# uos/radarays_ros

Hardware: AMD Instinct MI355X
Metric: polar images/sec (400 az x 3424 bins) (higher is better)
Workload: dtype f32 rays / f64 energy+time; 1 GPU; target_10M_400x200_4pass; triangles=10248350, azimuths=400, range_bins=3424, rays_per_beam=200, passes=4, ambient_noise=2, frames_per_batch=8

## Files before the change

### include/radarays_mi355.h

```cpp
#ifndef RADARAYS_MI355_H
#define RADARAYS_MI355_H

#include <stddef.h>
#include <stdint.h>

#ifdef __cplusplus
extern "C" {
#endif

#define RR_ABI_VERSION 7
#define RR_MAX_BATCH 64

typedef struct rr_ctx rr_ctx;

typedef struct rr_material {
    float velocity;
    float ambient;
    float diffuse;
    float specular;
} rr_material;

typedef struct rr_config {
    int32_t n_cells;
    int32_t n_angles;
    int32_t n_reflections;
    int32_t signal_denoising;
    int32_t signal_denoising_triangular_width;
    int32_t signal_denoising_gaussian_width;
    int32_t signal_denoising_mb_width;
    int32_t ambient_noise;
    int32_t scroll_image;
    int32_t record_multi_reflection;
    int32_t record_multi_path;
    int32_t max_waves_per_azimuth;
    int32_t brdf_model;
    int32_t reserved_;
    double  resolution;
    double  energy_max;
    double  signal_max;
    double  signal_denoising_triangular_mode;
    double  signal_denoising_gaussian_mode;
    double  signal_denoising_mb_mode;
    double  ambient_noise_at_signal_0;
    double  ambient_noise_at_signal_1;
    double  ambient_noise_energy_max;
    double  ambient_noise_energy_min;
    double  ambient_noise_energy_loss;
    double  multipath_threshold;
    float   wave_energy_threshold;
    float   theta_min;
    float   theta_inc;
    float   range_max;
} rr_config;

typedef struct rr_stats {
    uint64_t wave_passes;
    uint64_t hits;
    uint64_t signals;
    uint64_t nodes_visited;
    uint64_t tris_tested;
    uint32_t overflow;
    uint32_t pad_;
} rr_stats;

void rr_default_config(rr_config* cfg);

rr_ctx* rr_create(int device);
void    rr_destroy(rr_ctx* ctx);
const char* rr_last_error(const rr_ctx* ctx);
int     rr_abi_version(void);

int rr_set_mesh(rr_ctx* ctx, const float* verts , size_t nv,
                const uint32_t* faces , size_t nf,
                const uint32_t* face_object_id );

int rr_set_mesh_gpu(rr_ctx* ctx, const float* verts , size_t nv,
                    const uint32_t* faces , size_t nf,
                    const uint32_t* face_object_id );

int rr_copy_mesh(rr_ctx* ctx, rr_ctx* src);

int rr_set_object_poses(rr_ctx* ctx, const float* poses , size_t n);
int rr_update_vertices(rr_ctx* ctx, const float* verts , size_t nv);
int rr_get_tree_cost(rr_ctx* ctx, double* cost_now, double* cost_at_build);
int rr_rebuild_tree(rr_ctx* ctx, int builder);

int rr_set_materials(rr_ctx* ctx, const rr_material* materials, size_t n_materials,
                     const int32_t* object_materials, size_t n_objects,
                     int32_t material_id_air);

int rr_set_config(rr_ctx* ctx, const rr_config* cfg);

int rr_set_beam_samples(rr_ctx* ctx, const float* dirs , size_t n);

int rr_set_noise_offsets(rr_ctx* ctx, const float* rnd, size_t n);

int rr_set_motion_poses(rr_ctx* ctx, const float* poses, size_t n);

int rr_simulate(rr_ctx* ctx, const float pose_qxyzw_t[7], int az_begin, int az_end,
                uint8_t* out_u8, float* out_f32, rr_stats* stats);

int rr_simulate_columns_device(rr_ctx* ctx, const float pose_qxyzw_t[7], int az_begin, int az_end,
                               uint8_t* d_cols_u8, float* d_cols_f32, void* stream);

int rr_simulate_batch_columns_device(rr_ctx* ctx, const float* poses, int n_frames, int az_begin, int az_end,
                                     uint8_t* d_cols_u8, void* stream);

int rr_simulate_batch_device(rr_ctx* ctx, const float* poses, int n_frames, uint8_t* d_imgs_u8, void* stream);

int rr_simulate_batch_host_async(rr_ctx* ctx, const float* poses, int n_frames, uint8_t* h_imgs_u8, void* stream);
int rr_wait_host(rr_ctx* ctx, const void* h_imgs_u8);
void* rr_host_alloc(size_t bytes);
void  rr_host_free(void* p);

int rr_copy_to_host_async(rr_ctx* ctx, const void* d_src, void* h_dst, size_t bytes, void* stream);
int rr_deliver_to_host_async(rr_ctx* ctx, const void* d_src, void* h_dst, size_t bytes, void* stream);
int rr_host_delivery_route(rr_ctx* ctx);

int rr_assemble_image_device(rr_ctx* ctx, const uint8_t* d_cols_u8 ,
                             uint8_t* d_img_u8 , void* stream);

int rr_assemble_blocks_device(rr_ctx* ctx, const uint8_t* d_cols_u8, int n_loc, size_t block_stride,
                              uint8_t* d_img_u8, void* stream);

int rr_simulate_material_sets_device(rr_ctx* ctx, const float pose[7], const rr_material* sets, int n_sets,
                                     size_t n_materials ,
                                     uint8_t* d_imgs_u8, void* stream);
int rr_simulate_material_sets(rr_ctx* ctx, const float pose[7], const rr_material* sets, int n_sets,
                              size_t n_materials, uint8_t* out_imgs_u8);

typedef struct rr_param_set {
    const rr_material* materials;
    const float* beam_dirs;
    int32_t n_reflections;
    int32_t reserved_;
} rr_param_set;
int rr_simulate_param_sets_device(rr_ctx* ctx, const float pose[7], const rr_param_set* sets, int n_sets, size_t n_materials,
                                  uint8_t* d_imgs_u8 , void* stream);
int rr_score_images_device(rr_ctx* ctx, const uint8_t* d_imgs_u8, int n_images, const uint8_t* d_ref_u8,
                           double* out_psnr , uint64_t* out_sse , void* stream);
int rr_simulate_param_sets(rr_ctx* ctx, const float pose[7], const rr_param_set* sets, int n_sets, size_t n_materials,
                           uint8_t* out_imgs_u8, const uint8_t* ref_img_u8, double* out_psnr);

int rr_assemble_frames_device(rr_ctx* ctx, const uint8_t* d_cols_u8, int n_loc, size_t block_stride,
                              int n_frames, size_t frame_stride, uint8_t* d_imgs_u8, void* stream);

int rr_simulate_device(rr_ctx* ctx, const float pose_qxyzw_t[7], uint8_t* d_img_u8, void* stream);

int rr_synchronize(rr_ctx* ctx, void* stream);

int rr_peek_error_bits_async(rr_ctx* ctx, uint32_t* h_bits, void* stream);

int rr_get_stats(rr_ctx* ctx, rr_stats* stats);

int rr_set_stats_mode(rr_ctx* ctx, int enable);
int rr_get_traversal_shape(rr_ctx* ctx, uint64_t out[8]);

int rr_debug_trace(rr_ctx* ctx, const float* origs , const float* dirs , size_t n,
                   float* out_t , uint32_t* out_face );
int rr_debug_fresnel(rr_ctx* ctx, size_t n, const float* normals , const float* dirs , const double* energy ,
                     const double* v1 , const float* v2 ,
                     float* out_refl_dir , double* out_refl_energy , float* out_refr_dir , double* out_refr_energy );
int rr_debug_brdf(rr_ctx* ctx, size_t n, const float* in5 , int brdf_model, float* out );
int rr_get_bvh_info(rr_ctx* ctx, uint64_t* n_nodes, uint64_t* n_tris, uint32_t* depth, uint32_t* stack_need);
int rr_get_trace_grid(rr_ctx* ctx, uint32_t out_rows[24], uint32_t out_hist[24], uint64_t* repaired_groups);
int rr_get_graph_stats(rr_ctx* ctx, uint64_t* captures, uint64_t* replays);
int rr_set_timing_mode(rr_ctx* ctx, int enable );
int rr_get_kernel_time(rr_ctx* ctx, const char* kernel ,
                       double* total_ms, uint64_t* launches, int reset);

int rr_get_kernel_samples(rr_ctx* ctx, const char* kernel, float* out_ms, size_t capacity, size_t* n_out);
int rr_reserve_timing_events(rr_ctx* ctx, size_t n);

typedef struct rr_detect_config {
    int32_t method;
    int32_t guard_cells;
    int32_t train_cells;
    int32_t k;
    int32_t min_intensity;
    int32_t min_bin;
    float   cfar_scale;
    int32_t reserved_;
} rr_detect_config;

typedef struct rr_radar_point {
    float    x, y, z;
    float    intensity;
    uint32_t column;
    uint32_t bin;
} rr_radar_point;

typedef struct rr_cartesian_config {
    int32_t width;
    int32_t interpolation;
    float   pixel_size;
    int32_t reserved_;
} rr_cartesian_config;

void rr_default_detect_config(rr_detect_config* cfg);

int rr_detect_device(rr_ctx* ctx, const uint8_t* d_imgs_u8 , int n_frames,
                     const rr_detect_config* cfg, rr_radar_point* d_points ,
                     int max_points, uint32_t* d_offsets , void* stream);
int rr_detect(rr_ctx* ctx, const uint8_t* imgs_u8, int n_frames, const rr_detect_config* cfg,
              rr_radar_point* points, int max_points, uint32_t* offsets);
int rr_polar_to_cartesian_device(rr_ctx* ctx, const uint8_t* d_imgs_u8, int n_frames, const rr_cartesian_config* cfg,
                                 uint8_t* d_cart_u8 , void* stream);
int rr_polar_to_cartesian(rr_ctx* ctx, const uint8_t* imgs_u8, int n_frames, const rr_cartesian_config* cfg,
                          uint8_t* cart_u8);

typedef struct rr_multi rr_multi;
rr_multi* rr_create_multi(const int* devices, int n_devices);
void rr_destroy_multi(rr_multi* m);
const char* rr_multi_last_error(const rr_multi* m);
int rr_multi_device_count(const rr_multi* m);
int rr_multi_rccl_version(const rr_multi* m);
rr_ctx* rr_multi_ctx(rr_multi* m, int i);
void rr_partition(int n_angles, int world, int rank, int* begin, int* end);
int rr_multi_plan(int n_angles, int n_cells, int n_devices, int n_frames, int* equal_blocks, size_t* bytes_per_device,
                  size_t* send_off, size_t* recv_off, size_t* piece_bytes);
int rr_multi_set_mesh(rr_multi* m, const float* verts, size_t nv, const uint32_t* faces, size_t nf, const uint32_t* face_object_id);
int rr_multi_set_mesh_gpu(rr_multi* m, const float* verts, size_t nv, const uint32_t* faces, size_t nf, const uint32_t* face_object_id);
int rr_multi_set_object_poses(rr_multi* m, const float* poses, size_t n);
int rr_multi_update_vertices(rr_multi* m, const float* verts, size_t nv);
int rr_multi_rebuild_tree(rr_multi* m, int builder);
int rr_multi_set_materials(rr_multi* m, const rr_material* materials, size_t n_materials,
                           const int32_t* object_materials, size_t n_objects, int32_t material_id_air);
int rr_multi_set_config(rr_multi* m, const rr_config* cfg);
int rr_multi_set_beam_samples(rr_multi* m, const float* dirs, size_t n);
int rr_multi_set_noise_offsets(rr_multi* m, const float* rnd, size_t n);
int rr_multi_set_motion_poses(rr_multi* m, const float* poses, size_t n);
int rr_multi_simulate(rr_multi* m, const float pose_qxyzw_t[7], uint8_t* out_u8);
int rr_multi_simulate_batch(rr_multi* m, const float* poses, int n_frames, uint8_t* out_imgs_u8);
int rr_multi_simulate_batch_async(rr_multi* m, const float* poses, int n_frames, uint8_t* h_imgs_u8);
int rr_multi_wait(rr_multi* m, const void* h_imgs_u8);

int rr_cone_dirs(float width_rad, int sample_dist, float p_in_cone, const float* u_angle, const float* r_variate, size_t n,
                 float* out_dirs);
int rr_sample_cone_local(uint32_t seed, float width_rad, size_t n, int sample_dist, float p_in_cone, float* out_dirs);

typedef struct rr_mesh {
    float* verts;
    size_t n_verts;
    uint32_t* faces;
    size_t n_faces;
    uint32_t* face_object_id;
    size_t n_objects;
    char** object_names;
} rr_mesh;
int rr_load_mesh_file(const char* path, rr_mesh* out, char* err, size_t err_len);
int rr_mesh_reorder_objects(rr_mesh* m, const char* const* order, size_t n_order, char* err, size_t err_len);
void rr_free_mesh(rr_mesh* m);


#ifdef __cplusplus
}
#endif
#endif
```

### radarays_ros_amd/csrc/rr_api.hip

```cpp
#include "rr_ctx.h"
#include <algorithm>
#include <cmath>
#include <cstring>
#include <cstdlib>
#include <dlfcn.h>

namespace rr {
namespace {

std::string g_create_error;

bool roctx_load()
{
    static int state = 0;
    if (state == 0) {
        state = -1;
        for (const char* n : { "librocprofiler-sdk-roctx.so.1", "librocprofiler-sdk-roctx.so", "libroctx64.so.4", "libroctx64.so" }) {
            void* h = dlopen(n, RTLD_NOW | RTLD_GLOBAL);
            if (!h) continue;
            g_roctx_push = (roctx_push_fn)dlsym(h, "roctxRangePushA");
            g_roctx_pop = (roctx_pop_fn)dlsym(h, "roctxRangePop");
            if (g_roctx_push && g_roctx_pop) { state = 1; break; }
        }
    }
// ... 118 lines not shown
    }
    }

    if (dirty & rr_ctx::D_MAT) {
    std::vector<float4> m4(c->materials.size());
    for (size_t i = 0; i < m4.size(); i++)
        m4[i] = make_float4(c->materials[i].velocity, c->materials[i].ambient, c->materials[i].diffuse, c->materials[i].specular);
    RR_HIP(c, c->d_materials.ensure(m4.size()));
    if (!m4.empty()) RR_HIP(c, upload_table(c, c->d_materials.p, m4.data(), m4.size() * sizeof(float4)));
    RR_HIP(c, c->d_mat_limits.ensure(m4.size()));
    launch_mat_limits(c->d_materials.p, m4.size(), c->d_mat_limits.p, nullptr);
    RR_HIP(c, hipGetLastError());
    RR_HIP(c, hipStreamSynchronize(nullptr));
    RR_HIP(c, c->d_objmat.ensure(c->object_materials.size()));
    if (!c->object_materials.empty())
        RR_HIP(c, upload_table(c, c->d_objmat.p, c->object_materials.data(), c->object_materials.size() * sizeof(int32_t)));
    }

    if (dirty & rr_ctx::D_CFG) {
    make_smear(g, c->smear, c->smear_mode);
    RR_HIP(c, c->d_smear.ensure(c->smear.size()));
    if (!c->smear.empty()) RR_HIP(c, upload_table(c, c->d_smear.p, c->smear.data(), c->smear.size() * sizeof(float)));

    RR_HIP(c, c->d_decay.ensure((size_t)std::max(1, g.n_cells)));
    launch_decay_table(c->d_decay.p, g.n_cells, g.resolution, g.ambient_noise_energy_loss, nullptr);
    RR_HIP(c, hipGetLastError());
    RR_HIP(c, hipDeviceSynchronize());
    }

    if (dirty & (rr_ctx::D_NOISE | rr_ctx::D_CFG)) {
    const size_t A = (size_t)g.n_angles;
    if (!c->noise.empty() && c->noise.size() % A != 0)
        return fail(c, -3, "rr_set_noise_offsets: the number of offsets must be a multiple of n_angles (one row per frame of a batch)");
    c->noise_rows = c->noise.size() >= 2 * A ? (int)(c->noise.size() / A) : 1;
    std::vector<float> nz((size_t)c->noise_rows * A, 0.0f);
    for (size_t i = 0; i < nz.size() && i < c->noise.size(); i++) nz[i] = c->noise[i];
    RR_HIP(c, c->d_noise.ensure(nz.size()));
    RR_HIP(c, upload_table(c, c->d_noise.p, nz.data(), nz.size() * sizeof(float)));
    }
    if ((dirty & (rr_ctx::D_MOTION | rr_ctx::D_CFG)) && !c->motion.empty()) {
        if (c->motion.size() % (7 * (size_t)g.n_angles) != 0)
            return fail(c, -3, "rr_set_motion_poses: the number of poses must be a multiple of n_angles (one table per frame of a batch)");
        c->motion_rows = (int)(c->motion.size() / (7 * (size_t)g.n_angles));
        RR_HIP(c, c->d_motion.ensure(c->motion.size()));
        RR_HIP(c, upload_table(c, c->d_motion.p, c->motion.data(), c->motion.size() * sizeof(float)));
    }
    c->motion_live = !c->motion.empty();
    const void* motion_after = c->motion_live ? (const void*)c->d_motion.p : nullptr;
    if (regen || noise_before != (const void*)c->d_noise.p || noise_rows_before != c->noise_rows ||
        motion_before != motion_after || motion_rows_before != c->motion_rows) c->graph_gen++;
    c->tables_dirty = 0;
    return 0;
}

int read_back(rr_ctx* c, void* dst, const void* d_src, size_t bytes)
{
    if (bytes == 0) return 0;
    if (bytes % 16 != 0 || (uintptr_t)d_src % 16 != 0) { RR_HIP(c, hipMemcpy(dst, d_src, bytes, hipMemcpyDeviceToHost)); return 0; }
    if (c->h_rb_bytes < bytes) {
        if (c->h_rb) (void)hipHostFree(c->h_rb);
        c->h_rb = nullptr; c->h_rb_bytes = 0;
        RR_HIP(c, hipHostMalloc(&c->h_rb, bytes + 4096, hipHostMallocDefault));
        c->h_rb_bytes = bytes + 4096;
    }
    launch_copy_host(d_src, c->h_rb, bytes, 4, -1, c->stream);
    RR_HIP(c, hipGetLastError());
    RR_HIP(c, hipStreamSynchronize(c->stream));
    std::memcpy(dst, c->h_rb, bytes);
    return 0;
}

int overflow_error(rr_ctx* c, uint32_t bits, bool since_sync)
{
    if (bits & 1u)
        return fail(c, -7, std::string("wave/signal queue capacity exceeded") + (since_sync ? " in a frame since the last rr_synchronize" : "") +
                               "; raise rr_config.max_waves_per_azimuth");
    if (bits & 2u)
        return fail(c, -8, std::string("object id or material id out of range of the tables given to rr_set_materials") +
                               (since_sync ? " (a frame since the last rr_synchronize)" : ""));
    return 0;
}

int check_ready(rr_ctx* c)
{
    if (!c) return -1;
    if (!c->have_mesh) return fail(c, -2, "rr_set_mesh has not been called");
    if (!c->have_cfg) return fail(c, -2, "rr_set_config has not been called");
    if (!c->have_materials) return fail(c, -2, "rr_set_materials has not been called");
    if (c->beams.empty() && c->cfg.n_reflections > 0) return fail(c, -2, "rr_set_beam_samples has not been called");
    return 0;
}

}

extern "C" {

int rr_abi_version(void) { return RR_ABI_VERSION; }

void rr_partition(int n_angles, int world, int rank, int* begin, int* end)
{
    if (world < 1) world = 1;
    const int base = n_angles / world, rem = n_angles % world;
    const int b = rank * base + (rank < rem ? rank : rem);
    if (begin) *begin = b;
    if (end) *end = b + base + (rank < rem ? 1 : 0);
}

void rr_default_config(rr_config* cfg)
{
    if (!cfg) return;
    std::memset(cfg, 0, sizeof(*cfg));
    cfg->n_cells = 3424; cfg->n_angles = 400; cfg->n_reflections = 4;
    cfg->signal_denoising = 1;
    cfg->signal_denoising_triangular_width = 50; cfg->signal_denoising_triangular_mode = 0.35;
    cfg->signal_denoising_gaussian_width = 50; cfg->signal_denoising_gaussian_mode = 0.5;
    cfg->signal_denoising_mb_width = 50; cfg->signal_denoising_mb_mode = 0.4;
    cfg->ambient_noise = 2; cfg->scroll_image = 0;
    cfg->record_multi_reflection = 1; cfg->record_multi_path = 0;
    cfg->max_waves_per_azimuth = 0;
    cfg->resolution = 0.0438; cfg->energy_max = 0.5; cfg->signal_max = 120.0;
    cfg->ambient_noise_at_signal_0 = 0.3; cfg->ambient_noise_at_signal_1 = 0.03;
    cfg->ambient_noise_energy_max = 0.5; cfg->ambient_noise_energy_min = 0.1;
    cfg->ambient_noise_energy_loss = 0.05; cfg->multipath_threshold = 0.5;
    cfg->wave_energy_threshold = 0.001f;
    cfg->theta_min = 0.0f; cfg->theta_inc = (float)(-(2 * M_PI) / 400);
    cfg->range_max = 1000.0f;
}

rr_ctx* rr_create(int device)
{
    int n = 0;
    hipError_t e = hipGetDeviceCount(&n);
    if (e != hipSuccess || n <= 0) {
        g_create_error = std::string("rr_create: no HIP device (") + (e != hipSuccess ? hipGetErrorString(e) : "count 0") +
                         "); this library has no CPU fallback";
        return nullptr;
    }
    if (device < 0 || device >= n) { g_create_error = "rr_create: device index out of range"; return nullptr; }
    if (hipSetDevice(device) != hipSuccess) { g_create_error = "rr_create: hipSetDevice failed"; return nullptr; }
    rr_ctx* c = new rr_ctx();
    c->device = device;
    if (hipStreamCreateWithFlags(&c->stream, hipStreamNonBlocking) != hipSuccess) {
        g_create_error = "rr_create: hipStreamCreate failed"; delete c; return nullptr;
    }
    rr_default_config(&c->cfg);
    int n_lanes = getenv("RR_LANES") ? atoi(getenv("RR_LANES")) : 4;
    n_lanes = std::max(1, std::min(n_lanes, 8));
    c->stream_lanes = getenv("RR_STREAM_LANES") ? std::max(1, std::min(atoi(getenv("RR_STREAM_LANES")), n_lanes))
                                                : std::min(3, n_lanes);
    if (getenv("RR_PASS0_AZ")) { const int a = atoi(getenv("RR_PASS0_AZ")); if (a == 1 || a == 2 || a == 4 || a == 8 || a == 16) c->pass0_az = a; }
    if (getenv("RR_STACK_LDS")) c->stack_lds_max = std::max(1, std::min(64, atoi(getenv("RR_STACK_LDS"))));
    if (getenv("RR_ROCTX") && atoi(getenv("RR_ROCTX")) != 0) c->roctx = roctx_load();
    if (getenv("RR_CULL_POP")) c->cull_pop = atoi(getenv("RR_CULL_POP")) != 0;
    if (getenv("RR_STACKLESS")) c->stackless = atoi(getenv("RR_STACKLESS")) != 0;
    if (getenv("RR_TRACE_CHUNK")) c->seg_chunk = std::max(0, std::min(1024, atoi(getenv("RR_TRACE_CHUNK"))));
    if (getenv("RR_GRAPHS")) c->use_graphs = atoi(getenv("RR_GRAPHS")) != 0;
    if (getenv("RR_HOST_SDMA")) c->host_sdma = atoi(getenv("RR_HOST_SDMA")) != 0;
    if (getenv("RR_TIGHT_GRID")) c->tight_grid = atoi(getenv("RR_TIGHT_GRID")) != 0;
    if (getenv("RR_TIGHT_FORCE")) c->tight_force = std::max(0, atoi(getenv("RR_TIGHT_FORCE")));
    {
        const float4 same = make_float4(0.3f, 0.f, 0.f, 0.f);
        DevBuf<float4> m1; DevBuf<double> l1;
        bool ok = m1.ensure(1) == hipSuccess && l1.ensure(2) == hipSuccess &&
                  upload_table(c, m1.p, &same, sizeof(same)) == hipSuccess;
        if (ok) {
            launch_mat_limits(m1.p, 1, l1.p, nullptr);
            double two[2] = {0.0, 0.0};
            ok = hipStreamSynchronize(nullptr) == hipSuccess && read_back(c, two, l1.p, sizeof(two)) == 0;
            c->limit_same = two[0];
        }
        m1.release(); l1.release();
        if (!ok) { g_create_error = "rr_create: device set-up failed"; rr_destroy(c); return nullptr; }
    }
    c->lanes.resize((size_t)n_lanes);
    for (Lane& L : c->lanes) {
        if (hipStreamCreateWithFlags(&L.stream, hipStreamNonBlocking) != hipSuccess ||
            hipEventCreateWithFlags(&L.ev_ready, hipEventDisableTiming) != hipSuccess ||
            hipEventCreateWithFlags(&L.ev_consumed, hipEventDisableTiming) != hipSuccess ||
            hipEventCreateWithFlags(&L.slot[0].ev, hipEventDisableTiming) != hipSuccess ||
            hipEventCreateWithFlags(&L.slot[1].ev, hipEventDisableTiming) != hipSuccess) {
            g_create_error = "rr_create: lane stream/event creation failed"; rr_destroy(c); return nullptr;
        }
    }
    return c;
}

void rr_destroy(rr_ctx* c)
{
    if (!c) return;
    (void)hipSetDevice(c->device);
    (void)hipDeviceSynchronize();
    if (c->sdma) { sdma_destroy(c->sdma); c->sdma = nullptr; }
    for (Delivery& d : c->deliveries) (void)hipEventDestroy(d.ev);
    for (hipEvent_t e : c->delivery_events) (void)hipEventDestroy(e);
    for (auto& kv : c->timers) for (auto& p : kv.second.pending) { (void)hipEventDestroy(p.first); (void)hipEventDestroy(p.second); }
    for (hipEvent_t e : c->event_pool) (void)hipEventDestroy(e);
    c->d_rest_v.release(); c->d_stage_v.release(); c->d_rest_f.release(); c->d_poses.release(); c->d_stage_poses.release();
    c->d_levels.release(); c->d_red.release(); c->d_cost.release(); c->d_built.release(); c->d_moved.release();
    c->d_bvh.release(); c->d_qas.release(); c->d_beams.release(); c->d_materials.release(); c->d_mat_limits.release();
    c->d_objmat.release(); c->d_smear.release(); c->d_noise.release(); c->d_decay.release(); c->d_param_imgs.release(); c->d_sse.release(); c->d_ref_img.release(); c->d_conv_in.release(); c->d_conv_cart.release(); c->d_conv_points.release(); c->d_conv_offs.release(); c->d_beam_order.release(); c->d_beam_order2.release(); c->d_motion.release();
    for (Lane& L : c->lanes) {
        if (L.stream) (void)hipStreamSynchronize(L.stream);
        for (int k = 0; k < 2; k++) { L.d_wA[k].release(); L.d_wB[k].release(); L.d_wC[k].release(); L.d_idx[k].release(); L.d_count[k].release(); L.d_torder[k].release(); }
        L.d_refpos.release();
        L.d_hit.release(); L.d_sig_count.release(); L.d_spill.release(); L.d_cflag.release(); L.d_cols_u8.release();
        L.d_sigtmp.release(); L.d_sig.release(); L.d_cols_f32.release(); L.d_counters.release(); L.d_sticky.release(); L.d_seg_stats.release(); L.d_matsets.release(); L.d_matset_limits.release(); L.d_set_beams.release(); L.d_set_order.release(); L.d_set_order2.release(); L.d_img_f32.release();
        L.d_hint.release(); L.d_ovf_list.release(); if (L.h_hist) { (void)hipHostFree(L.h_hist); L.h_hist = nullptr; }
        drop_graphs(L); L.d_poses.release();
        if (L.ev_ready) (void)hipEventDestroy(L.ev_ready);
        if (L.ev_consumed) (void)hipEventDestroy(L.ev_consumed);
        for (Delivery& d : L.slot) { d.img.release(); if (d.ev) (void)hipEventDestroy(d.ev); }
        if (L.stream) (void)hipStreamDestroy(L.stream);
    }
    if (c->stream) (void)hipStreamDestroy(c->stream);
    if (c->h_frame) (void)hipHostFree(c->h_frame);
    if (c->h_rb) (void)hipHostFree(c->h_rb);
    delete c;
}

const char* rr_last_error(const rr_ctx* c) { return c ? c->err.c_str() : g_create_error.c_str(); }

int rr_set_materials(rr_ctx* c, const rr_material* materials, size_t n_materials,
                     const int32_t* object_materials, size_t n_objects, int32_t material_id_air)
{
    if (!c) return -1;
    if (!materials || n_materials == 0) return fail(c, -3, "rr_set_materials: empty material table");
    if (n_objects && !object_materials) return fail(c, -3, "rr_set_materials: null object_materials");
    if (material_id_air < 0 || (size_t)material_id_air >= n_materials) return fail(c, -3, "rr_set_materials: material_id_air out of range");
    for (size_t i = 0; i < n_objects; i++)
        if (object_materials[i] < 0 || (size_t)object_materials[i] >= n_materials)
            return fail(c, -3, "rr_set_materials: object_materials entry out of range");
    if (c->have_materials && c->materials.size() == n_materials && c->object_materials.size() == n_objects &&
        c->material_id_air == material_id_air &&
        std::memcmp(c->materials.data(), materials, n_materials * sizeof(rr_material)) == 0 &&
        (n_objects == 0 || std::memcmp(c->object_materials.data(), object_materials, n_objects * sizeof(int32_t)) == 0))
        return 0;
    c->materials.assign(materials, materials + n_materials);
    c->object_materials.assign(object_materials, object_materials + n_objects);
    c->material_id_air = material_id_air;
    c->have_materials = true; c->tables_dirty |= rr_ctx::D_MAT;
    return 0;
}

int rr_set_config(rr_ctx* c, const rr_config* cfg)
{
    if (!c) return -1;
    if (!cfg) return fail(c, -3, "rr_set_config: null config");
    if (cfg->n_cells < 1 || cfg->n_cells > 8192) return fail(c, -3, "rr_set_config: n_cells must be in [1, 8192]");
    if (cfg->n_angles < 1 || cfg->n_angles > 65536) return fail(c, -3, "rr_set_config: n_angles must be in [1, 65536]");
    if (cfg->n_reflections < 0 || cfg->n_reflections > 16) return fail(c, -3, "rr_set_config: n_reflections must be in [0, 16]");
    if (cfg->signal_denoising < 0 || cfg->signal_denoising > 3) return fail(c, -3, "rr_set_config: signal_denoising must be 0..3");
    const int w = cfg->signal_denoising == 1 ? cfg->signal_denoising_triangular_width
                : cfg->signal_denoising == 2 ? cfg->signal_denoising_gaussian_width
                : cfg->signal_denoising == 3 ? cfg->signal_denoising_mb_width : 0;
    if (w < 0 || w > 256) return fail(c, -3, "rr_set_config: smear width must be in [0, 256]");
    if (cfg->ambient_noise < 0 || cfg->ambient_noise > 2) return fail(c, -3, "rr_set_config: ambient_noise must be 0..2");
    if (cfg->brdf_model < 0 || cfg->brdf_model > 1) return fail(c, -3, "rr_set_config: brdf_model must be 0 (A + B cos^C) or 1 (Cook-Torrance lobe)");
    if (!(cfg->resolution > 0.0)) return fail(c, -3, "rr_set_config: resolution must be > 0");
    const double mf = cfg->signal_denoising == 1 ? cfg->signal_denoising_triangular_mode
                    : cfg->signal_denoising == 2 ? cfg->signal_denoising_gaussian_mode
                    : cfg->signal_denoising == 3 ? cfg->signal_denoising_mb_mode : 0.0;
    if (!(mf >= 0.0 && mf < 1.0)) return fail(c, -3, "rr_set_config: denoising mode fraction must be in [0, 1)");
    if (!(cfg->range_max > 0.0f && cfg->range_max <= 1.0e30f)) return fail(c, -3, "rr_set_config: range_max must be in (0, 1e30]");
    if (!std::isfinite(cfg->wave_energy_threshold) || !std::isfinite(cfg->theta_min) || !std::isfinite(cfg->theta_inc))
        return fail(c, -3, "rr_set_config: non-finite wave_energy_threshold / theta_min / theta_inc");
    if (c->have_cfg && std::memcmp(&c->cfg, cfg, sizeof(rr_config)) == 0) return 0;
    c->cfg = *cfg;
    c->have_cfg = true; c->tables_dirty |= rr_ctx::D_CFG;
    return 0;
}

int rr_set_beam_samples(rr_ctx* c, const float* dirs, size_t n)
{
    if (!c) return -1;
    if (n && !dirs) return fail(c, -3, "rr_set_beam_samples: null dirs");
    if (n > 65536) return fail(c, -3, "rr_set_beam_samples: more than 65536 samples");
    for (size_t i = 0; i < 3 * n; i++) if (!std::isfinite(dirs[i])) return fail(c, -3, "rr_set_beam_samples: non-finite direction");
    if (c->beams.size() == 3 * n && (n == 0 || std::memcmp(c->beams.data(), dirs, 3 * n * sizeof(float)) == 0)) return 0;
    c->beams.assign(dirs, dirs + 3 * n);
    c->tables_dirty |= rr_ctx::D_BEAMS;
    return 0;
}

int rr_set_noise_offsets(rr_ctx* c, const float* rnd, size_t n)
{
    if (!c) return -1;
    if (n && !rnd) return fail(c, -3, "rr_set_noise_offsets: null pointer");
    for (size_t i = 0; i < n; i++) if (!std::isfinite(rnd[i])) return fail(c, -3, "rr_set_noise_offsets: non-finite offset");
    c->noise.assign(rnd, rnd + n);
    c->tables_dirty |= rr_ctx::D_NOISE;
    return 0;
}

int rr_set_motion_poses(rr_ctx* c, const float* poses, size_t n)
{
    if (!c) return -1;
    if (n && !poses) return fail(c, -3, "rr_set_motion_poses: null pointer");
    for (size_t i = 0; i < 7 * n; i++) if (!std::isfinite(poses[i])) return fail(c, -3, "rr_set_motion_poses: non-finite pose");
    c->motion.assign(poses, poses + 7 * n);
    c->tables_dirty |= rr_ctx::D_MOTION;
    return 0;
}

void* rr_host_alloc(size_t bytes)
{
    void* p = nullptr;
    if (hipHostMalloc(&p, bytes ? bytes : 1, hipHostMallocDefault) != hipSuccess) return nullptr;
    return p;
}

void rr_host_free(void* p) { if (p) (void)hipHostFree(p); }

int rr_score_images_device(rr_ctx* c, const uint8_t* d_imgs_u8, int n_images, const uint8_t* d_ref_u8, double* out_psnr,
                           uint64_t* out_sse, void* stream)
{
    if (!c) return -1;
    if (!c->have_cfg) return fail(c, -2, "rr_set_config has not been called");
    if (!d_imgs_u8 || !d_ref_u8 || (!out_psnr && !out_sse)) return fail(c, -3, "rr_score_images_device: null buffer");
    if (n_images < 1 || n_images > 65535) return fail(c, -3, "rr_score_images_device: n_images must be 1..65535");
    RR_HIP(c, hipSetDevice(c->device));
    hipStream_t s = stream_of(c, stream);
    const size_t npx = (size_t)c->cfg.n_cells * c->cfg.n_angles;
    static_assert(sizeof(unsigned long long) == sizeof(uint64_t), "sse words");
    if (c->d_sse.n < (size_t)n_images) { RR_HIP(c, hipStreamSynchronize(s)); RR_HIP(c, c->d_sse.ensure((size_t)n_images)); }
    RR_HIP(c, hipMemsetAsync(c->d_sse.p, 0, (size_t)n_images * sizeof(uint64_t), s));
    launch_score(d_imgs_u8, d_ref_u8, npx, n_images, c->d_sse.p, s);
    RR_HIP(c, hipGetLastError());
    std::vector<uint64_t> sse((size_t)n_images);
    RR_HIP(c, hipMemcpyAsync(sse.data(), c->d_sse.p, (size_t)n_images * sizeof(uint64_t), hipMemcpyDeviceToHost, s));
    RR_HIP(c, hipStreamSynchronize(s));
    for (int k = 0; k < n_images; k++) {
        if (out_sse) out_sse[k] = sse[(size_t)k];
        if (out_psnr) {
            const double err = (double)sse[(size_t)k] / (double)npx;
            out_psnr[k] = err > 0.0 ? 10.0 * std::log10((255.0 * 255.0) / err) : INFINITY;
        }
    }
    return 0;
}

void rr_default_detect_config(rr_detect_config* cfg)
{
    if (!cfg) return;
    std::memset(cfg, 0, sizeof(*cfg));
    cfg->method = 0; cfg->guard_cells = 2; cfg->train_cells = 16; cfg->k = 12;
    cfg->min_intensity = 1; cfg->min_bin = 0; cfg->cfar_scale = 3.0f;
}

namespace {

int check_frames(rr_ctx* c, const char* who, const void* imgs, int n_frames)
{
    if (!c) return -1;
    if (!c->have_cfg) return fail(c, -2, "rr_set_config has not been called");
    if (!imgs) return fail(c, -3, std::string(who) + ": null images");
    if (n_frames < 1 || n_frames > 65535) return fail(c, -3, std::string(who) + ": n_frames must be 1..65535");
// ... 135 lines not shown
```

### radarays_ros_amd/csrc/rr_ctx.h

```cpp
#pragma once
#include "rr_launch.h"
#include "rr_sdma.h"
#include <map>
#include <string>
#include <vector>

namespace rr {
template <typename T>
struct DevBuf {
    T* p = nullptr;
    size_t n = 0;
    hipError_t ensure(size_t count) {
        if (count <= n && p) return hipSuccess;
        if (p) { (void)hipFree(p); p = nullptr; n = 0; }
        if (count == 0) count = 1;
        hipError_t e = hipMalloc((void**)&p, count * sizeof(T));
        if (e == hipSuccess) n = count;
        return e;
    }
    void release() { if (p) (void)hipFree(p); p = nullptr; n = 0; }
};

struct KernelTimer {
    std::vector<std::pair<hipEvent_t, hipEvent_t>> pending;
    double total_ms = 0.0;
    uint64_t launches = 0;
    std::vector<float> samples_ms;
};

struct Delivery {
    DevBuf<uint8_t> img;
    hipEvent_t ev = nullptr;
    const void* dst = nullptr;
    uint64_t job = 0;
};

struct Lane {
    int buf_seg = 0, buf_cap = 0, buf_sigcap = 0, buf_cells = 0, buf_passes = 0;
    DevBuf<float4> d_wA[2], d_wB[2];
    DevBuf<double2> d_wC[2];
    DevBuf<uint32_t> d_idx[2], d_count[2], d_refpos, d_sig_count, d_spill;
    DevBuf<uint2> d_torder[2];
    DevBuf<uint2> d_hit;
    DevBuf<uint8_t> d_cflag, d_cols_u8;
    DevBuf<SigRec> d_sigtmp, d_sig;
    DevBuf<float> d_cols_f32;
    DevBuf<Counters> d_counters;
    DevBuf<uint32_t> d_sticky;
    DevBuf<float> d_img_f32;
    DevBuf<SegStats> d_seg_stats;
    DevBuf<float4> d_matsets;
    DevBuf<double> d_matset_limits;
    DevBuf<float4> d_set_beams; DevBuf<uint32_t> d_set_order, d_set_order2;
    std::vector<float4> h_set_beams, h_matsets; std::vector<uint32_t> h_set_order, h_set_order2;
    int last_n_seg = 0, last_n_passes = 0;
    int spill_stride = 0, stack_lds = 1;
    DevBuf<GridHint> d_hint; DevBuf<uint32_t> d_ovf_list; int ovf_stride = 0;
    uint32_t* h_hist = nullptr; int hist_gen = 0;
    struct FrameGraph {
        int az_begin = 0, az_end = 0, n_frames = 0; const void* cols = nullptr; unsigned short rows[kMaxPasses] = {};
        hipGraph_t g = nullptr; hipGraphExec_t ge = nullptr; hipGraphNode_t pose_node = nullptr; uint64_t last_use = 0; int hits = 0;
        hipGraphExec_t ge2 = nullptr; hipEvent_t ev[2] = { nullptr, nullptr }; bool ev_pending[2] = { false, false }; int flip = 0;
        hipKernelNodeParams pose_kp{};
        Params pose_P;
    };
    std::vector<FrameGraph> graphs; int graph_gen = 0;
    DevBuf<float> d_poses;
    unsigned short last_rows[kMaxPasses] = {};

    hipStream_t stream = nullptr;
    hipEvent_t ev_ready = nullptr, ev_consumed = nullptr;
    bool pending_consume = false;
    Delivery slot[2]; int next_slot = 0;
};

}
using namespace rr;

struct rr_ctx {
    int device = 0;
    hipStream_t stream = nullptr;
    std::string err;

    bool have_mesh = false;
    DevBuf<float4> d_bvh;
    uint32_t tri_base4 = 0;
    uint64_t n_nodes = 0, n_tris = 0;
    uint32_t depth = 0, stack_need = 0;
    float hit_pad = 0.f;

    DevBuf<float> d_rest_v, d_stage_v;
    DevBuf<uint32_t> d_rest_f;
    size_t rest_nv = 0, rest_nf = 0;
    uint32_t n_objects = 1;
    std::vector<float> poses;
    DevBuf<float> d_poses, d_stage_poses;
    bool dyn_ready = false;
    bool rebuilding = false;
    DevBuf<uint32_t> d_levels;
    std::vector<uint32_t> level_off;
    bool cost_known = false; double cost_at_build = 0.0;
    DevBuf<float4> d_built; bool have_built = false; float built_hit_pad = 0.f;
    std::vector<float> build_poses; bool verts_dirty = false;
    DevBuf<uint8_t> d_moved;
    DevBuf<float> d_red; DevBuf<double> d_cost;

    rr_config cfg;
    bool have_cfg = false;
    std::vector<rr_material> materials;
    std::vector<int32_t> object_materials;
    int32_t material_id_air = 0;
    bool have_materials = false;
    std::vector<float> beams;
    std::vector<float> noise;
    int noise_rows = 1;
    int motion_rows = 1;
    bool motion_live = false;
    std::vector<float> motion;
    std::vector<float> smear;
    int smear_mode = 0;

    DevBuf<float4> d_qas, d_beams, d_materials;
    DevBuf<double> d_mat_limits;
    double limit_same = 0.0;
    DevBuf<uint32_t> d_beam_order, d_beam_order2;
    DevBuf<int32_t> d_objmat;
    DevBuf<float> d_smear, d_noise, d_motion, d_decay;
    DevBuf<uint8_t> d_param_imgs;
    enum : unsigned { D_CFG = 1, D_BEAMS = 2, D_MAT = 4, D_NOISE = 8, D_MOTION = 16, D_ALL = 31 };
    unsigned tables_dirty = D_ALL;

    std::vector<Lane> lanes;
    size_t next_lane = 0, last_lane = 0;
    size_t next_stream_lane = 0;
    int stream_lanes = 3;

    bool stats_mode = false;
    int pass0_az = 16;
    int stack_lds_max = 64;
    int timing = 0;
    std::map<std::string, KernelTimer> timers;
    std::vector<hipEvent_t> event_pool;
    hipEvent_t take_event() {
        if (!event_pool.empty()) { hipEvent_t e = event_pool.back(); event_pool.pop_back(); return e; }
        hipEvent_t e = nullptr; (void)hipEventCreate(&e); return e;
    }

    int passes_override = -1;
    DevBuf<unsigned long long> d_sse; DevBuf<uint8_t> d_ref_img;
    DevBuf<uint8_t> d_conv_in, d_conv_cart; DevBuf<rr_radar_point> d_conv_points; DevBuf<uint32_t> d_conv_offs;
    void* h_rb = nullptr; size_t h_rb_bytes = 0;
    void* h_frame = nullptr; size_t h_frame_bytes = 0;

    bool roctx = false;
    int seg_chunk = 16;
    int stackless = 0;
    int cull_pop = 1;
    int host_sdma = 1; SdmaCopier* sdma = nullptr; bool sdma_tried = false;
    std::vector<Delivery> deliveries;
    std::vector<hipEvent_t> delivery_events;
    int tight_grid = 1;
    int tight_force = 0;
    int hist_gen = 1;
    int use_graphs = 1;
    int graph_gen = 1;
    uint64_t graph_clock = 0, graph_replays = 0, graph_captures = 0;
};

namespace rr {
typedef int (*roctx_push_fn)(const char*);
typedef int (*roctx_pop_fn)(void);
inline roctx_push_fn g_roctx_push = nullptr; inline roctx_pop_fn g_roctx_pop = nullptr;
inline void roctx_push(const char* name) { if (g_roctx_push) g_roctx_push(name); }
inline void roctx_pop() { if (g_roctx_pop) g_roctx_pop(); }
int fail(rr_ctx* c, int code, const std::string& msg);

inline hipStream_t stream_of(const rr_ctx* c, void* stream) { return stream ? (hipStream_t)stream : c->stream; }

#define RR_HIP(c, expr)                                                                        \
    do {                                                                                       \
        hipError_t e_ = (expr);                                                                \
        if (e_ != hipSuccess)                                                                  \
            return fail((c), -100, std::string(#expr) + ": " + hipGetErrorString(e_));         \
    } while (0)

struct TimedScope {
    rr_ctx* c; hipStream_t s; const char* name; hipEvent_t a = nullptr, b = nullptr;
    bool on;
    TimedScope(rr_ctx* c_, hipStream_t s_, const char* n_) : c(c_), s(s_), name(n_) {
        on = c->timing == 1;
        if (on) { a = c->take_event(); b = c->take_event(); (void)hipEventRecord(a, s); }
        if (c->roctx) roctx_push(name);
    }
    ~TimedScope() {
        if (on) { (void)hipEventRecord(b, s); c->timers[name].pending.emplace_back(a, b); }
        if (c->roctx) roctx_pop();
    }
};

struct KernelEvents {
    rr_ctx* c; const char* name; hipEvent_t a = nullptr, b = nullptr;
    KernelEvents(rr_ctx* c_, const char* n_) : c(c_), name(n_) {
        if (c->timing == 1) { a = c->take_event(); b = c->take_event(); }
        if (c->roctx) roctx_push(name);
    }
    ~KernelEvents() {
        if (a) c->timers[name].pending.emplace_back(a, b);
        if (c->roctx) roctx_pop();
    }
};

struct SetPlan {
    int n_groups = 1;
    unsigned char frame_passes[64], frame_beam[64], group_frame[64];
    const float4* d_beams = nullptr; const uint32_t* d_order = nullptr; const uint32_t* d_order2 = nullptr;
};

int check_ready(rr_ctx* c);
int upload_tables(rr_ctx* c);
void beam_trace_orders(const float* beams, size_t nb, std::vector<uint32_t>& order, std::vector<uint32_t>& order2);
int read_back(rr_ctx* c, void* dst, const void* d_src, size_t bytes);
int overflow_error(rr_ctx* c, uint32_t bits, bool since_sync = false);
inline int read_counters(rr_ctx* c, Counters& h) { return read_back(c, &h, c->lanes[c->last_lane].d_counters.p, sizeof(h)); }

void drop_graphs(Lane& L);
int prepare_lane(rr_ctx* c, Lane& L, int n_seg, bool want_f32 = false);
bool host_visible(const void* p);
int settle_lane(rr_ctx* c, Lane& L, int slot = -1, const void* only_dst = nullptr);
int take_lane(rr_ctx* c, size_t li, hipStream_t s, int slot = -1);
hipError_t give_lane(Lane& L, hipStream_t s);
int run_frame(rr_ctx* c, Lane& L, const float* pose, int az_begin, int az_end, uint8_t* d_cols_u8 , float* d_cols_f32,
              hipStream_t s, int n_frames = 1, const float4* d_matsets = nullptr, int mat_stride = 0, bool lane_f32 = false, const SetPlan* plan = nullptr);
int assemble_frames(rr_ctx* c, const Lane& L, uint8_t* dst, int n_frames, hipStream_t s);

}
```

### radarays_ros_amd/csrc/rr_device.h

```cpp
#pragma once
#include <hip/hip_runtime.h>
#include <stdint.h>

#include "rr_bvh.h"

namespace rr {

struct V3 { float x, y, z; };
struct Quat { float x, y, z, w; };

__host__ __device__ inline V3 v_add(V3 a, V3 b) { return { a.x + b.x, a.y + b.y, a.z + b.z }; }
__host__ __device__ inline V3 v_sub(V3 a, V3 b) { return { a.x - b.x, a.y - b.y, a.z - b.z }; }
__host__ __device__ inline V3 v_neg(V3 a) { return { -a.x, -a.y, -a.z }; }
__host__ __device__ inline V3 v_scale(V3 a, float s) { return { a.x * s, a.y * s, a.z * s }; }
__host__ __device__ inline float v_dot(V3 a, V3 b) { return a.x * b.x + a.y * b.y + a.z * b.z; }
__host__ __device__ inline V3 v_cross(V3 a, V3 b)
{
    return { a.y * b.z - a.z * b.y, a.z * b.x - a.x * b.z, a.x * b.y - a.y * b.x };
}
__host__ __device__ inline V3 v_normalize(V3 a)
{
    const float d = sqrtf(a.x * a.x + a.y * a.y + a.z * a.z);
    return { a.x / d, a.y / d, a.z / d };
}
__host__ __device__ inline Quat q_mul(Quat a, Quat b)
{
    Quat r;
    r.x = a.w * b.x + a.x * b.w + a.y * b.z - a.z * b.y;
    r.y = a.w * b.y - a.x * b.z + a.y * b.w + a.z * b.x;
    r.z = a.w * b.z + a.x * b.y - a.y * b.x + a.z * b.w;
    r.w = a.w * b.w - a.x * b.x - a.y * b.y - a.z * b.z;
    return r;
}
__host__ __device__ inline Quat q_conj(Quat a) { return { -a.x, -a.y, -a.z, a.w }; }
__host__ __device__ inline V3 q_rot(Quat q, V3 v)
{
    Quat t;
    t.x = q.w * v.x + q.y * v.z - q.z * v.y;
    t.y = q.w * v.y - q.x * v.z + q.z * v.x;
    t.z = q.w * v.z + q.x * v.y - q.y * v.x;
    t.w = 0.0f - q.x * v.x - q.y * v.y - q.z * v.z;
    const Quat c = q_conj(q);
    V3 r;
    r.x = t.w * c.x + t.x * c.w + t.y * c.z - t.z * c.y;
    r.y = t.w * c.y - t.x * c.z + t.y * c.w + t.z * c.x;
    r.z = t.w * c.z + t.x * c.y - t.y * c.x + t.z * c.w;
    return r;
}

struct WaveBuf {
    float4* A;
    float4* B;
    double2* C;
};

struct SigRec { int32_t cell; float strength; };

struct Counters {
    unsigned long long nodes, tris;
    unsigned long long wave_iters;
    unsigned int max_iters, n_waves;
    unsigned int overflow, pad;
    unsigned long long it_all, it_node, it_leaf, quad_steps;
    unsigned long long pad2;
};

constexpr int kMaxPasses = 24;
struct GridHint { uint32_t hist[kMaxPasses]; uint32_t ovf_n[kMaxPasses]; unsigned long long repaired;  };

struct SegStats { uint32_t wave_passes, hits, signals, pad; };

struct Params {
    const Node4* nodes;
    const TriRec* tris;
    uint32_t tri_base4;
    const float4* q_as;
    const float4* beams;
    const uint32_t* beam_order;
    const uint32_t* beam_order2;
    const float4* materials;
    const double* mat_limits;
    double limit_same;
    const int32_t* object_materials;
    const float* smear;
    const float* noise_rnd;
    int noise_rows;
    int mat_stride;
    int set_mode;
    int n_groups;
    unsigned char frame_passes[64];
    unsigned char frame_beam[64];
    unsigned char group_frame[64];
    const float* decay;
    const float* motion_poses;
    int motion_rows;
    WaveBuf waves[2];
    uint32_t* idx[2];
    uint32_t* count[2];
    uint2* torder[2];
    uint32_t* refpos;
    uint8_t* cflag;
    SigRec* sigtmp;
    uint2* hit;
    SigRec* sig;
    uint32_t* sig_count;
    uint32_t* spill;
    Counters* counters;
    uint32_t* sticky;
    SegStats* seg_stats;
    uint8_t* cols_u8;
    float* cols_f32;
    int az_begin, n_seg;
    int n_loc, n_frames;
    float4* pose_table;
    int n_beam, cap, sigcap;
    int n_cells, n_angles, n_materials, n_objects, material_id_air;
    int n_passes, record_multi_reflection, record_multi_path;
    int brdf_model;
    int signal_denoising, smear_w, smear_mode, ambient_noise, scroll;
    float thr, range_max;
    float hit_pad;
    double resolution, multipath_threshold;
    float energy_max_f;
    double signal_max;
    double noise_at_0, noise_at_1, noise_e_max, noise_e_min, noise_e_loss;
    int spill_stride, stack_lds, spill_depth;
    int pass0_az;
    int trace_row;
    int seg_chunk;
    int stackless;
    int cull_pop;
    GridHint* grid_hint;
    uint32_t* hist_host;
    uint32_t* ovf_list;
    int ovf_stride;
    unsigned short tight_groups[kMaxPasses];
};

struct PoseArgs { float p[64][7]; int n; };
struct NoPoses {};
template <bool FIRST> struct PosesOf { using type = NoPoses; };
template <> struct PosesOf<true> { using type = PoseArgs; };

__host__ __device__ inline int passes_of(const Params& P, int frame) { return P.set_mode ? (int)P.frame_passes[frame] : P.n_passes; }
__host__ __device__ inline int beam_base(const Params& P, int frame) { return P.set_mode ? (int)P.frame_beam[frame] * P.n_beam : 0; }

static_assert(sizeof(Params) <= 4096, "Params is passed by value: HIP kernel arguments are limited to 4 KB");

}
```

### radarays_ros_amd/csrc/rr_frame.hip

```cpp
#include "rr_ctx.h"
#include "rr_hostprof.h"
#include <algorithm>
#include <cmath>
#include <cstdio>
#include <cstring>
#include <cstdlib>

namespace rr {
namespace {

inline int eff_passes(const rr_ctx* c) { return c->passes_override >= 0 ? c->passes_override : c->cfg.n_reflections; }
inline rr_config eff_config(const rr_ctx* c) { rr_config g = c->cfg; g.n_reflections = eff_passes(c); return g; }

int wave_capacity(const rr_config& cfg, int n_beam)
{
    long cap = cfg.max_waves_per_azimuth;
    if (cap <= 0) {
        cap = n_beam;
        for (int p = 1; p < cfg.n_reflections && cap < 65536; p++) cap *= 2;
        cap = std::min<long>(cap, 65536);
    }
    cap = std::max<long>(cap, n_beam);
    return (int)cap;
}

int signal_capacity(const rr_config& cfg, int n_beam, int cap)
{
    long tot = 0, w = n_beam;
    for (int p = 0; p < cfg.n_reflections; p++) { tot += std::min<long>(w, cap); w = std::min<long>(2 * w, cap); }
    if (cfg.record_multi_path) tot *= 2;
    return (int)std::max<long>(tot, 1);
}

void drop_graph(Lane::FrameGraph& fg)
{
    for (int k = 0; k < 2; k++) {
        if (fg.ev[k]) { if (fg.ev_pending[k]) (void)hipEventSynchronize(fg.ev[k]); (void)hipEventDestroy(fg.ev[k]); fg.ev[k] = nullptr; fg.ev_pending[k] = false; }
    }
    if (fg.ge) (void)hipGraphExecDestroy(fg.ge);
    if (fg.ge2) (void)hipGraphExecDestroy(fg.ge2);
    if (fg.g) (void)hipGraphDestroy(fg.g);
    fg.ge = fg.ge2 = nullptr; fg.g = nullptr;
}
int ensure_frame_buffers(rr_ctx* c, Lane& L, int n_seg, bool want_f32)
{
    const rr_config g = eff_config(c);
    const int n_beam = (int)(c->beams.size() / 3);
    const int cap = wave_capacity(g, n_beam);
    const int sigcap = signal_capacity(g, n_beam, cap);
    const size_t S = (size_t)n_seg;
    const size_t per_seg = (size_t)cap * (2 * 2 * 48 + 2 * 4 + 2 * 9 + 8) + (size_t)sigcap * 8 + (size_t)g.n_cells * 5;
    size_t free_b = 0, total_b = 0;
    RR_HIP(c, hipMemGetInfo(&free_b, &total_b));
    if (S * per_seg > total_b / 2)
        return fail(c, -6, "wave queue capacity needs more than half of device memory; lower max_waves_per_azimuth");
    for (int k = 0; k < 2; k++) {
        RR_HIP(c, L.d_wA[k].ensure(S * 2 * cap));
        RR_HIP(c, L.d_wB[k].ensure(S * 2 * cap));
        RR_HIP(c, L.d_wC[k].ensure(S * 2 * cap));
        RR_HIP(c, L.d_idx[k].ensure(S * cap));
        RR_HIP(c, L.d_torder[k].ensure(S * cap));
        RR_HIP(c, L.d_count[k].ensure(S));
    }
    RR_HIP(c, L.d_cflag.ensure(S * 2 * cap));
    RR_HIP(c, L.d_refpos.ensure(S * 2 * cap));
    RR_HIP(c, L.d_sigtmp.ensure(S * 2 * cap));
    RR_HIP(c, L.d_hit.ensure(S * cap));
    RR_HIP(c, L.d_sig.ensure(S * sigcap));
    RR_HIP(c, L.d_sig_count.ensure(S));
    if (!L.d_counters.p) { RR_HIP(c, L.d_counters.ensure(1)); RR_HIP(c, hipMemset(L.d_counters.p, 0, sizeof(Counters))); }
    if (!L.d_sticky.p) { RR_HIP(c, L.d_sticky.ensure(1)); RR_HIP(c, hipMemset(L.d_sticky.p, 0, sizeof(uint32_t))); }
    RR_HIP(c, L.d_seg_stats.ensure(S * (size_t)std::max(1, g.n_reflections)));
    if (!L.d_hint.p) { RR_HIP(c, L.d_hint.ensure(1)); RR_HIP(c, hipMemset(L.d_hint.p, 0, sizeof(GridHint))); L.hist_gen = 0; }
    if (!L.h_hist) { RR_HIP(c, hipHostMalloc((void**)&L.h_hist, kMaxPasses * sizeof(uint32_t), hipHostMallocDefault)); std::memset(L.h_hist, 0, kMaxPasses * sizeof(uint32_t)); }
    RR_HIP(c, L.d_ovf_list.ensure(S * (size_t)kMaxPasses)); L.ovf_stride = (int)S;
    RR_HIP(c, L.d_cols_u8.ensure(S * g.n_cells));
    if (want_f32) RR_HIP(c, L.d_cols_f32.ensure(S * g.n_cells));
    L.stack_lds = (int)std::max<uint32_t>(1, std::min<uint32_t>(c->stack_need, (uint32_t)c->stack_lds_max));
    const int spill_depth = (int)c->stack_need - L.stack_lds;
    const size_t A0 = (size_t)c->pass0_az, Sw0 = 16 / A0;
    const size_t slots0 = ((((S + A0 - 1) / A0) * (((size_t)n_beam + Sw0 - 1) / Sw0) + 1) / 2) * 32;
    const size_t threads = std::max(S * (size_t)((cap + 63) / 64) * 64, slots0);
    L.spill_stride = (int)threads;
    if (spill_depth > 0) RR_HIP(c, L.d_spill.ensure((size_t)spill_depth * threads));
    else RR_HIP(c, L.d_spill.ensure(1));
    L.buf_seg = n_seg; L.buf_cap = cap; L.buf_sigcap = sigcap; L.buf_cells = g.n_cells; L.buf_passes = std::max(1, g.n_reflections);
    RR_HIP(c, L.d_poses.ensure((size_t)RR_MAX_BATCH * 8));
    L.graph_gen = 0;
    return 0;
}

void fill_params(rr_ctx* c, Lane& L, Params& P, const float pose[7], int az_begin, int n_seg,
                 uint8_t* d_cols_u8, float* d_cols_f32)
{
    const rr_config g = eff_config(c);
    std::memset(&P, 0, sizeof(P));
    P.nodes = reinterpret_cast<const Node4*>(c->d_bvh.p); P.tris = reinterpret_cast<const TriRec*>(c->d_bvh.p + c->tri_base4);
    P.tri_base4 = c->tri_base4;
    P.q_as = c->d_qas.p; P.beams = c->d_beams.p; P.beam_order = c->d_beam_order.p; P.beam_order2 = c->d_beam_order2.p; P.materials = c->d_materials.p;
    P.mat_limits = c->d_mat_limits.p; P.limit_same = c->limit_same;
    P.object_materials = c->d_objmat.p; P.smear = c->d_smear.p;
    P.noise_rnd = g.ambient_noise ? c->d_noise.p : nullptr; P.noise_rows = c->noise_rows;
    P.decay = c->d_decay.p;
    P.motion_poses = c->motion.empty() ? nullptr : c->d_motion.p; P.motion_rows = c->motion_rows;
    for (int k = 0; k < 2; k++) {
        P.waves[k].A = L.d_wA[k].p; P.waves[k].B = L.d_wB[k].p; P.waves[k].C = L.d_wC[k].p;
        P.idx[k] = L.d_idx[k].p; P.count[k] = L.d_count[k].p; P.torder[k] = L.d_torder[k].p;
    }
    P.refpos = L.d_refpos.p;
    P.cflag = L.d_cflag.p; P.sigtmp = L.d_sigtmp.p; P.hit = L.d_hit.p;
    P.sig = L.d_sig.p; P.sig_count = L.d_sig_count.p; P.spill = L.d_spill.p; P.counters = L.d_counters.p; P.sticky = L.d_sticky.p; P.seg_stats = L.d_seg_stats.p;
    P.cols_u8 = d_cols_u8; P.cols_f32 = d_cols_f32;
    P.az_begin = az_begin; P.n_seg = n_seg;
    P.n_beam = (int)(c->beams.size() / 3); P.cap = L.buf_cap; P.sigcap = L.buf_sigcap;
    P.n_cells = g.n_cells; P.n_angles = g.n_angles;
    P.n_materials = (int)c->materials.size(); P.n_objects = (int)c->object_materials.size();
    P.material_id_air = c->material_id_air;
    P.n_passes = g.n_reflections;
    P.record_multi_reflection = g.record_multi_reflection; P.record_multi_path = g.record_multi_path;
    P.brdf_model = g.brdf_model;
    P.signal_denoising = c->smear.empty() ? 0 : g.signal_denoising;
    P.smear_w = (int)c->smear.size(); P.smear_mode = c->smear_mode;
    P.ambient_noise = g.ambient_noise; P.scroll = g.scroll_image;
    P.thr = g.wave_energy_threshold; P.range_max = g.range_max; P.hit_pad = c->hit_pad;
    P.resolution = g.resolution; P.multipath_threshold = g.multipath_threshold;
    P.energy_max_f = (float)g.energy_max; P.signal_max = g.signal_max;
    P.noise_at_0 = g.ambient_noise_at_signal_0; P.noise_at_1 = g.ambient_noise_at_signal_1;
    P.noise_e_max = g.ambient_noise_energy_max; P.noise_e_min = g.ambient_noise_energy_min;
    P.noise_e_loss = g.ambient_noise_energy_loss;
    P.spill_stride = L.spill_stride; P.stack_lds = L.stack_lds;
    P.spill_depth = std::max(0, (int)c->stack_need - L.stack_lds);
    P.pass0_az = c->pass0_az;
    P.cull_pop = c->cull_pop; P.seg_chunk = c->seg_chunk; P.stackless = c->stackless;
    P.grid_hint = L.d_hint.p; P.ovf_list = L.d_ovf_list.p; P.ovf_stride = L.ovf_stride;
    P.hist_host = (c->tight_grid && g.n_reflections > 1) ? L.h_hist : nullptr;
}

int copy_out(rr_ctx* c, const void* d_src, void* h_dst, size_t bytes, bool visible, hipStream_t s)
{
    if (bytes == 0) return 0;
    if (visible && bytes % 16 == 0 && ((uintptr_t)h_dst | (uintptr_t)d_src) % 16 == 0) {
        launch_copy_host(d_src, h_dst, bytes, 8, 0, s);
        RR_HIP(c, hipGetLastError());
    } else RR_HIP(c, hipMemcpyAsync(h_dst, d_src, bytes, hipMemcpyDeviceToHost, s));
    return 0;
}

int wait_delivery(rr_ctx* c, Delivery& d)
{
    if (!d.dst) return 0;
    if (d.job) sdma_wait(c->sdma, d.job);
    else RR_HIP(c, hipEventSynchronize(d.ev));
    d.dst = nullptr; d.job = 0;
    return 0;
}

SdmaCopier* sdma_of(rr_ctx* c, const void* any_device_ptr)
{
    if (!c->host_sdma) return nullptr;
    if (!c->sdma && !c->sdma_tried) {
        c->sdma_tried = true;
        std::string why;
        c->sdma = sdma_create(c->device, any_device_ptr, why);
        if (!c->sdma && getenv("RR_HOST_SDMA_VERBOSE")) fprintf(stderr, "[rr] SDMA delivery not available: %s\n", why.c_str());
    }
    if (c->sdma && sdma_failed(c->sdma, nullptr)) {
        if (getenv("RR_HOST_SDMA_VERBOSE")) { std::string why; (void)sdma_failed(c->sdma, &why); fprintf(stderr, "[rr] SDMA delivery switched off: %s\n", why.c_str()); }
        c->host_sdma = 0;
        return nullptr;
    }
    return c->sdma;
}

int choose_trace_rows(rr_ctx* c, Lane& L, Params& P, const rr_config& g, hipStream_t s)
{
    if (L.hist_gen != c->hist_gen) {
        RR_HIP(c, hipMemsetAsync(L.d_hint.p, 0, sizeof(GridHint), s));
        std::memset(L.h_hist, 0, kMaxPasses * sizeof(uint32_t));
        L.hist_gen = c->hist_gen;
    }
    const bool tight = c->tight_grid && !c->stats_mode && !P.set_mode && P.spill_depth == 0 && g.n_reflections <= kMaxPasses;
    if (tight) {
        for (int pass = 1; pass < g.n_reflections; pass++) {
            const long bound = std::min<long>((long)P.cap, pass < 20 ? (long)P.n_beam << pass : (long)P.cap);
            const long full = (bound + 15) / 16;
            uint32_t h = 0;
            for (const Lane& o : c->lanes) if (o.h_hist && o.hist_gen == c->hist_gen) h = std::max(h, o.h_hist[pass]);
            long row = h ? std::min<long>(full, ((long)h + (long)h / 16 + 32 + 15) / 16) : full;
            row |= 1;
            if (c->tight_force) row = std::min<long>(full, c->tight_force);
            P.tight_groups[pass] = (row < full && row < 65535) ? (unsigned short)row : 0;
        }
    }
    std::memcpy(L.last_rows, P.tight_groups, sizeof(L.last_rows));
    return 0;
}

int issue_chain(rr_ctx* c, const Params& Q, const PoseArgs& pa, const rr_config& g, hipStream_t s)
{
    for (int pass = 0; pass < g.n_reflections; pass++) {
        if (c->roctx) roctx_push(pass == 0 ? "trace pass 0" : "trace");
        if (c->timing) {
            hipEvent_t a = c->take_event(), b = c->take_event();
            const bool rep = pass > 0 && pass < kMaxPasses && Q.tight_groups[pass];
            hipEvent_t ra = rep ? c->take_event() : nullptr, rb = rep ? c->take_event() : nullptr;
            bool launched = false;
            launch_trace(Q, pass, &pa, c->stats_mode, s, a, b, ra, rb, &launched);
            c->timers[pass == 0 ? "trace0" : "trace"].pending.emplace_back(a, b);
            if (launched) c->timers["trace_repair"].pending.emplace_back(ra, rb);
            else if (rep) { c->event_pool.push_back(ra); c->event_pool.push_back(rb); }
        } else {
            launch_trace(Q, pass, &pa, c->stats_mode, s);
        }
        if (c->roctx) roctx_pop();
        { KernelEvents t(c, "shade"); launch_shade(Q, pass, s, t.a, t.b); }
        if (pass < g.n_reflections - 1) { KernelEvents t(c, "scan"); launch_scan(Q, pass, s, t.a, t.b); }
    }
    { KernelEvents t(c, "column"); launch_column(Q, s, t.a, t.b); }
    return 0;
}

Lane::FrameGraph* find_graph(Lane& L, int az_begin, int az_end, int n_frames, const uint8_t* d_cols_u8, const Params& P)
{
    Lane::FrameGraph* fg = nullptr;
    for (Lane::FrameGraph& x : L.graphs)
        if (x.az_begin == az_begin && x.az_end == az_end && x.n_frames == n_frames && x.cols == (const void*)d_cols_u8 &&
            std::memcmp(x.rows, P.tight_groups, sizeof(x.rows)) == 0) { fg = &x; break; }
    if (!fg) {
        if (L.graphs.size() >= 12) {
            size_t lru = 0;
            for (size_t k = 1; k < L.graphs.size(); k++) if (L.graphs[k].last_use < L.graphs[lru].last_use) lru = k;
            drop_graph(L.graphs[lru]);
            L.graphs.erase(L.graphs.begin() + (long)lru);
        }
        Lane::FrameGraph n;
        n.az_begin = az_begin; n.az_end = az_end; n.n_frames = n_frames; n.cols = d_cols_u8;
        std::memcpy(n.rows, P.tight_groups, sizeof(n.rows));
        L.graphs.push_back(n);
        fg = &L.graphs.back();
    }
    return fg;
}

void capture_graph(rr_ctx* c, Lane::FrameGraph* fg, const Params& P, const PoseArgs& pa, const rr_config& g, hipStream_t s)
{
    if (c->sdma) sdma_wait_all(c->sdma);
    hipError_t e = hipStreamBeginCapture(s, hipStreamCaptureModeThreadLocal);
    if (e == hipSuccess) {
        const int rcq = issue_chain(c, P, pa, g, s);
        hipGraph_t gph = nullptr;
        e = hipStreamEndCapture(s, &gph);
        if (rcq == 0 && e == hipSuccess && gph) {
            hipGraphExec_t ge = nullptr, ge2 = nullptr;
            if (hipGraphInstantiate(&ge, gph, nullptr, nullptr, 0) == hipSuccess && hipGraphInstantiate(&ge2, gph, nullptr, nullptr, 0) == hipSuccess &&
                hipEventCreateWithFlags(&fg->ev[0], hipEventDisableTiming) == hipSuccess && hipEventCreateWithFlags(&fg->ev[1], hipEventDisableTiming) == hipSuccess) {
                size_t nn = 0; (void)hipGraphGetNodes(gph, nullptr, &nn);
                std::vector<hipGraphNode_t> nodes(nn); (void)hipGraphGetNodes(gph, nodes.data(), &nn);
                for (hipGraphNode_t nd : nodes) {
                    hipGraphNodeType ty; hipKernelNodeParams kp{};
                    if (hipGraphNodeGetType(nd, &ty) == hipSuccess && ty == hipGraphNodeTypeKernel &&
                        hipGraphKernelNodeGetParams(nd, &kp) == hipSuccess && kp.func == trace0_kernel(P.spill_depth > 0, P.stackless != 0)) {
                        fg->pose_node = nd; fg->pose_kp = kp; fg->pose_P = P; break;
                    }
                }
                if (fg->pose_node) { fg->g = gph; fg->ge = ge; fg->ge2 = ge2; c->graph_captures++; }
                else { (void)hipGraphExecDestroy(ge); (void)hipGraphExecDestroy(ge2); (void)hipGraphDestroy(gph); }
            } else { if (ge) (void)hipGraphExecDestroy(ge); if (ge2) (void)hipGraphExecDestroy(ge2); (void)hipGraphDestroy(gph); }
            if (!fg->ge) for (int k = 0; k < 2; k++) if (fg->ev[k]) { (void)hipEventDestroy(fg->ev[k]); fg->ev[k] = nullptr; }
        } else if (gph) (void)hipGraphDestroy(gph);
    }
    (void)hipGetLastError();
    if (!fg->ge) fg->hits = -1000000;
}

int replay_graph(rr_ctx* c, Lane::FrameGraph* fg, const PoseArgs& pa, hipStream_t s)
{
    int pass0 = 0;
    void* args[3] = { (void*)&fg->pose_P, (void*)&pass0, (void*)&pa };
    hipKernelNodeParams kp = fg->pose_kp;
    kp.kernelParams = args; kp.extra = nullptr;
    hipError_t e = hipSuccess;
    const int w = fg->flip; fg->flip ^= 1;
    hipGraphExec_t ex = w ? fg->ge2 : fg->ge;
    if (fg->ev_pending[w]) { HostProfScope hp(6, "ctx:   graph: wait for the exec's previous launch"); e = hipEventSynchronize(fg->ev[w]); fg->ev_pending[w] = false; }
    { HostProfScope hp(3, "ctx:   graph: set the poses"); if (e == hipSuccess) e = hipGraphExecKernelNodeSetParams(ex, fg->pose_node, &kp); }
    { HostProfScope hp(4, "ctx:   graph: launch"); if (e == hipSuccess) e = hipGraphLaunch(ex, s); }
// ... 420 lines not shown
```

### radarays_ros_amd/csrc/rr_kernels.hip

```cpp
#include "rr_device.h"
#include "rr_launch.h"
#include <hip/hip_ext.h>

#include <algorithm>

namespace rr {

__device__ inline Quat ld_quat(const float4* p) { const float4 v = *p; return { v.x, v.y, v.z, v.w }; }

template <bool ARGS>
__device__ __forceinline__ void azimuth_frame(const Params& P, const PoseArgs* pa, int seg, Quat& q_am, V3& t_am)
{
    const int frame = seg / P.n_loc, az = P.az_begin + seg % P.n_loc;
    const Quat q_as = ld_quat(P.q_as + az);
    const int row = P.set_mode ? 0 : frame;
    Quat q_sm; V3 t_sm;
    if constexpr (ARGS) {
        const float* ps = pa->p[row];
        q_sm = { ps[0], ps[1], ps[2], ps[3] }; t_sm = { ps[4], ps[5], ps[6] };
    } else {
        const float4 a = P.pose_table[2 * row], b = P.pose_table[2 * row + 1];
        q_sm = { a.x, a.y, a.z, a.w }; t_sm = { b.x, b.y, b.z };
    }
    if (P.motion_poses) {
        const float* ps = P.motion_poses + 7 * ((size_t)(frame % P.motion_rows) * P.n_angles + az);
        q_sm = { ps[0], ps[1], ps[2], ps[3] }; t_sm = { ps[4], ps[5], ps[6] };
    }
    q_am = q_mul(q_sm, q_as);
    t_am = t_sm;
}

struct Hit { float t; uint32_t tri; uint32_t face; };

constexpr int kRaysPerWave = 16;
constexpr int kTraceThreads = 64;
constexpr int kRaysPerBlock = kTraceThreads / 4;
#ifndef RR_CULL_POP
#define RR_CULL_POP 1
#endif
constexpr bool kCullPop = RR_CULL_POP != 0;

#define RR_DPP_I(x, ctrl) __builtin_amdgcn_update_dpp(0, (int)(x), (ctrl), 0xF, 0xF, true)
#define RR_DPP_F(x, ctrl) __int_as_float(__builtin_amdgcn_update_dpp(0, __float_as_int(x), (ctrl), 0xF, 0xF, true))
#define RR_QBCAST0 0x00
#define RR_QBCAST1 0x55
#define RR_QBCAST2 0xAA
#define RR_QBCAST3 0xFF
#define RR_QROT1 0x39
#define RR_QROT2 0x4E
#define RR_QROT3 0x93
#define RR_QXOR1 0xB1
#define RR_QXOR2 0x4E

struct RaySetup { V3 o, d; float idx, idy, idz, oox, ooy, ooz; };
__device__ inline RaySetup ray_setup(V3 o, V3 d)
{
    RaySetup R; R.o = o; R.d = d;
    const float eps = 1e-20f;
    const float dx = fabsf(d.x) < eps ? copysignf(eps, d.x) : d.x;
    const float dy = fabsf(d.y) < eps ? copysignf(eps, d.y) : d.y;
    const float dz = fabsf(d.z) < eps ? copysignf(eps, d.z) : d.z;
    R.idx = __builtin_amdgcn_rcpf(dx); R.idy = __builtin_amdgcn_rcpf(dy); R.idz = __builtin_amdgcn_rcpf(dz);
    R.oox = -o.x * R.idx; R.ooy = -o.y * R.idy; R.ooz = -o.z * R.idz;
    return R;
}

template <bool STATS, bool SPILL, bool CULL>
__device__ inline Hit traverse(const float4* __restrict__ base4, const uint32_t tri_base4,
                               const RaySetup& R, float range_max, float hit_pad,
                               uint32_t* lds_stack, int stack_lds, uint32_t* spill, int spill_stride, int gray,
                               unsigned& n_nodes, unsigned& n_tris, unsigned* wstat = nullptr)
{
    const int q = threadIdx.x & 3;
    const int wave = threadIdx.x >> 6;
    const int rw = (threadIdx.x & 63) >> 2;
    uint32_t* my = lds_stack + (size_t)wave * stack_lds * kRaysPerWave + rw;
    uint16_t* myk = reinterpret_cast<uint16_t*>(lds_stack + (size_t)(kTraceThreads / 64) * stack_lds * kRaysPerWave) +
                    (size_t)wave * stack_lds * kRaysPerWave + rw;
    const V3 o = R.o, d = R.d;
    const float idx = R.idx, idy = R.idy, idz = R.idz, oox = R.oox, ooy = R.ooy, ooz = R.ooz;

    unsigned long long bestkey = 0x7F80000000000000ull;
    uint32_t best_first = 0;
    float tcull = range_max * 1.0001f + 1e-3f;
    int sp = 0;
    uint32_t cur = 0;

    const uint32_t q2 = 2u * (uint32_t)q, q3 = 3u * (uint32_t)q;
    const int qsh = (threadIdx.x & 63) & ~3;
    uint32_t misskey = 0x7F800000u | (uint32_t)q;
    asm volatile("" : "+v"(misskey));
    while (true) {
        const bool leaf = (cur & kLeafFlag) != 0;
        if (STATS) n_tris += 0x10000u;
        if (STATS && wstat) {
            wstat[0]++; wstat[1] += __ballot(!leaf) != 0ull; wstat[2] += __ballot(leaf) != 0ull;
            wstat[3] += (unsigned)__builtin_popcountll(__ballot(true)) >> 2;
        }
        const uint32_t first = cur & 0x0FFFFFFFu;
        const uint32_t cnt = ((cur >> 28) & 7u) + 1u;
        const float4* p = base4 + (first + (leaf ? q3 : q2));
        const float4 A = p[0], B = p[1];
        float4 C = make_float4(0.f, 0.f, 0.f, 0.f);
        if (leaf) C = p[2];
        if (!leaf) {
            if (STATS) { n_nodes += (q == 0); }
            const float ax = __builtin_fmaf(A.x, idx, oox), bx = __builtin_fmaf(A.w, idx, oox);
            const float ay = __builtin_fmaf(A.y, idy, ooy), by = __builtin_fmaf(B.x, idy, ooy);
            const float az = __builtin_fmaf(A.z, idz, ooz), bz = __builtin_fmaf(B.y, idz, ooz);
            const float tmin = fmaxf(fmaxf(fminf(ax, bx), fminf(ay, by)), fmaxf(fminf(az, bz), 0.0f));
            const float tmax = fminf(fminf(fmaxf(ax, bx), fmaxf(ay, by)), fmaxf(az, bz));
            const float lim = __int_as_float(min(__float_as_int(tmax), __float_as_int(tcull)));
            const bool h = tmin <= lim;
            const uint32_t mykey = h ? ((__float_as_uint(tmin) & ~3u) | (uint32_t)q) : misskey;
            const uint32_t myref = __float_as_uint(B.z);
            const uint32_t d1 = (uint32_t)RR_DPP_I(mykey, RR_QROT1) - mykey;
            const uint32_t d2 = (uint32_t)RR_DPP_I(mykey, RR_QROT2) - mykey;
            const uint32_t d3 = (uint32_t)RR_DPP_I(mykey, RR_QROT3) - mykey;
            const int rank = (int)((d1 >> 31) + (d2 >> 31) + (d3 >> 31));
            const int nhit = __builtin_popcount((unsigned)(__builtin_amdgcn_ballot_w64(h) >> qsh) & 0xFu);
            uint32_t nxt = (h && rank == 0) ? myref : 0u;
            nxt |= (uint32_t)RR_DPP_I(nxt, RR_QXOR1);
            nxt |= (uint32_t)RR_DPP_I(nxt, RR_QXOR2);
            if (h && rank > 0) {
                const int e = sp + (nhit - 1 - rank);
                if (SPILL && e >= stack_lds) spill[(size_t)(e - stack_lds) * spill_stride + gray] = myref;
                else { my[e * kRaysPerWave] = myref; if (CULL) myk[e * kRaysPerWave] = (uint16_t)(__float_as_uint(tmin) >> 16); }
            }
            if (nhit > 0) { sp += nhit - 1; cur = nxt; continue; }
        } else {
            if (STATS) n_tris += ((uint32_t)q < cnt);
            const V3 v0 = { A.x, A.y, A.z }, e1 = { B.x, B.y, B.z }, e2 = { C.x, C.y, C.z };
            const V3 pvec = v_cross(d, e2);
            const float det = v_dot(e1, pvec);
            const float inv = 1.0f / det;
            const V3 tvec = v_sub(o, v0);
            const float u = v_dot(tvec, pvec) * inv;
            const V3 qvec = v_cross(tvec, e1);
            const float v = v_dot(d, qvec) * inv;
            const float tt = v_dot(e2, qvec) * inv;
            bool ok = ((uint32_t)q < cnt) && (det != 0.0f) && (u >= 0.0f && u <= 1.0f) && (v >= 0.0f && u + v <= 1.0f) &&
                      (tt > 0.0f && tt <= range_max);
            const bool graze = ok && (det * det < C.w);
            if (__builtin_amdgcn_ballot_w64(graze) != 0ull) {
                const V3 ph = v_add(o, v_scale(d, tt));
                const V3 v1 = v_add(v0, e1), v2 = v_add(v0, e2);
                const bool inside =
                    ph.x >= fminf(v0.x, fminf(v1.x, v2.x)) - hit_pad && ph.x <= fmaxf(v0.x, fmaxf(v1.x, v2.x)) + hit_pad &&
                    ph.y >= fminf(v0.y, fminf(v1.y, v2.y)) - hit_pad && ph.y <= fmaxf(v0.y, fmaxf(v1.y, v2.y)) + hit_pad &&
                    ph.z >= fminf(v0.z, fminf(v1.z, v2.z)) - hit_pad && ph.z <= fmaxf(v0.z, fmaxf(v1.z, v2.z)) + hit_pad;
                if (graze && !inside) ok = false;
            }
            const uint32_t tb = ok ? __float_as_uint(tt) : 0x7F800000u;
            uint32_t tm = min(tb, (uint32_t)RR_DPP_I(tb, RR_QXOR1));
            tm = min(tm, (uint32_t)RR_DPP_I(tm, RR_QXOR2));
            const uint32_t fk = (tb == tm) ? ((__float_as_uint(A.w) << 2) | (uint32_t)q) : 0xFFFFFFFFu;
            uint32_t fm = min(fk, (uint32_t)RR_DPP_I(fk, RR_QXOR1));
            fm = min(fm, (uint32_t)RR_DPP_I(fm, RR_QXOR2));
            const unsigned long long key = ((unsigned long long)tm << 32) | fm;
            if (key < bestkey) {
                bestkey = key; best_first = first;
                tcull = __builtin_fmaf(__uint_as_float(tm), 1.0001f, 1e-3f);
            }
        }
        if (!CULL) {
            if (sp == 0) break;
            sp--;
            cur = (SPILL && sp >= stack_lds) ? spill[(size_t)(sp - stack_lds) * spill_stride + gray] : my[sp * kRaysPerWave];
        } else {
            const uint32_t ck = __float_as_uint(tcull) >> 16;
            bool more = false;
            while (sp > 0) {
                sp--;
                uint32_t k = 0;
                if (SPILL && sp >= stack_lds) cur = spill[(size_t)(sp - stack_lds) * spill_stride + gray];
                else { cur = my[sp * kRaysPerWave]; k = myk[sp * kRaysPerWave]; }
                asm volatile("" : "+v"(cur), "+v"(k));
                if (k <= ck) { more = true; break; }
            }
            if (!more) break;
        }
    }
    Hit best;
    best.t = __uint_as_float((uint32_t)(bestkey >> 32));
    const bool hit = (uint32_t)(bestkey >> 32) < 0x7F800000u;
    best.face = hit ? ((uint32_t)bestkey >> 2) : 0xFFFFFFFFu;
    best.tri = hit ? (best_first - tri_base4) / 3u + ((uint32_t)bestkey & 3u) : 0xFFFFFFFFu;
    return best;
}

__device__ inline Hit traverse_stackless(const float4* __restrict__ base4, const uint32_t tri_base4,
                                         const RaySetup& R, float range_max, float hit_pad)
{
    const int q = threadIdx.x & 3;
    const V3 o = R.o, d = R.d;
    const float idx = R.idx, idy = R.idy, idz = R.idz, oox = R.oox, ooy = R.ooy, ooz = R.ooz;
    unsigned long long bestkey = 0x7F80000000000000ull;
    uint32_t best_first = 0;
    float tcull = range_max * 1.0001f + 1e-3f;
    const uint32_t q2 = 2u * (uint32_t)q, q3 = 3u * (uint32_t)q;
    uint32_t cur = 0;
    int from = -1;
    float tmin = 0.0f, tmax = -1.0f;
    uint32_t mykey = 0x7FFFFFFFu, myref = 0u, plink = 0xFFFFFFFFu, leafkey = 0u;
    while (true) {
        const bool leaf = (cur & kLeafFlag) != 0;
        const uint32_t first = cur & 0x0FFFFFFFu;
        const uint32_t cnt = ((cur >> 28) & 7u) + 1u;
        const float4* p = base4 + (first + (leaf ? q3 : q2));
        const float4 A = p[0], B = p[1];
        float4 C = make_float4(0.f, 0.f, 0.f, 0.f);
        if (leaf) C = p[2];
        int prev;
        if (!leaf) {
            const float ax = __builtin_fmaf(A.x, idx, oox), bx = __builtin_fmaf(A.w, idx, oox);
            const float ay = __builtin_fmaf(A.y, idy, ooy), by = __builtin_fmaf(B.x, idy, ooy);
            const float az = __builtin_fmaf(A.z, idz, ooz), bz = __builtin_fmaf(B.y, idz, ooz);
            tmin = fmaxf(fmaxf(fminf(ax, bx), fminf(ay, by)), fmaxf(fminf(az, bz), 0.0f));
            tmax = fminf(fminf(fmaxf(ax, bx), fmaxf(ay, by)), fmaxf(az, bz));
            mykey = (__float_as_uint(tmin) & ~3u) | (uint32_t)q;
            myref = __float_as_uint(B.z);
            plink = (uint32_t)RR_DPP_I(__float_as_uint(B.w), RR_QBCAST0);
            uint32_t pk = (q == from) ? mykey : 0u;
            pk |= (uint32_t)RR_DPP_I(pk, RR_QXOR1);
            pk |= (uint32_t)RR_DPP_I(pk, RR_QXOR2);
            prev = from >= 0 ? (int)pk : -1;
        } else {
            const V3 v0 = { A.x, A.y, A.z }, e1 = { B.x, B.y, B.z }, e2 = { C.x, C.y, C.z };
            const V3 pvec = v_cross(d, e2);
            const float det = v_dot(e1, pvec);
            const float inv = 1.0f / det;
            const V3 tvec = v_sub(o, v0);
            const float u = v_dot(tvec, pvec) * inv;
            const V3 qvec = v_cross(tvec, e1);
            const float v = v_dot(d, qvec) * inv;
            const float tt = v_dot(e2, qvec) * inv;
            bool ok = ((uint32_t)q < cnt) && (det != 0.0f) && (u >= 0.0f && u <= 1.0f) && (v >= 0.0f && u + v <= 1.0f) &&
                      (tt > 0.0f && tt <= range_max);
            const bool graze = ok && (det * det < C.w);
            if (__builtin_amdgcn_ballot_w64(graze) != 0ull) {
                const V3 ph = v_add(o, v_scale(d, tt));
                const V3 v1 = v_add(v0, e1), v2 = v_add(v0, e2);
                const bool inside =
                    ph.x >= fminf(v0.x, fminf(v1.x, v2.x)) - hit_pad && ph.x <= fmaxf(v0.x, fmaxf(v1.x, v2.x)) + hit_pad &&
                    ph.y >= fminf(v0.y, fminf(v1.y, v2.y)) - hit_pad && ph.y <= fmaxf(v0.y, fmaxf(v1.y, v2.y)) + hit_pad &&
                    ph.z >= fminf(v0.z, fminf(v1.z, v2.z)) - hit_pad && ph.z <= fmaxf(v0.z, fmaxf(v1.z, v2.z)) + hit_pad;
                if (graze && !inside) ok = false;
            }
            const uint32_t tb = ok ? __float_as_uint(tt) : 0x7F800000u;
            uint32_t tm = min(tb, (uint32_t)RR_DPP_I(tb, RR_QXOR1));
            tm = min(tm, (uint32_t)RR_DPP_I(tm, RR_QXOR2));
            const uint32_t fk = (tb == tm) ? ((__float_as_uint(A.w) << 2) | (uint32_t)q) : 0xFFFFFFFFu;
            uint32_t fm = min(fk, (uint32_t)RR_DPP_I(fk, RR_QXOR1));
            fm = min(fm, (uint32_t)RR_DPP_I(fm, RR_QXOR2));
            const unsigned long long key = ((unsigned long long)tm << 32) | fm;
            if (key < bestkey) {
                bestkey = key; best_first = first;
                tcull = __builtin_fmaf(__uint_as_float(tm), 1.0001f, 1e-3f);
            }
            prev = (int)leafkey;
        }
        const float lim = __int_as_float(min(__float_as_int(tmax), __float_as_int(tcull)));
        const bool h = (tmin <= lim) && ((int)mykey > prev);
        const uint32_t cand = h ? mykey : 0x7FFFFFFFu;
        uint32_t m = min(cand, (uint32_t)RR_DPP_I(cand, RR_QXOR1));
        m = min(m, (uint32_t)RR_DPP_I(m, RR_QXOR2));
        if (m != 0x7FFFFFFFu) {
            uint32_t nxt = (cand == m) ? myref : 0u;
            nxt |= (uint32_t)RR_DPP_I(nxt, RR_QXOR1);
            nxt |= (uint32_t)RR_DPP_I(nxt, RR_QXOR2);
            cur = nxt; leafkey = m; from = -1;
        } else {
            if (plink == 0xFFFFFFFFu) break;
            cur = plink & ~7u; from = (int)(plink & 7u);
        }
    }
    Hit best;
    best.t = __uint_as_float((uint32_t)(bestkey >> 32));
    const bool hit = (uint32_t)(bestkey >> 32) < 0x7F800000u;
    best.face = hit ? ((uint32_t)bestkey >> 2) : 0xFFFFFFFFu;
    best.tri = hit ? (best_first - tri_base4) / 3u + ((uint32_t)bestkey & 3u) : 0xFFFFFFFFu;
    return best;
}

template <bool FIRST, bool STATS, bool SPILL, bool CULL, bool SL = false>
__device__ __forceinline__ void trace_group(const Params& P, const int pass, const int seg_y, const int gx, const int count,
                                            uint32_t* lds_stack, const int gdim_x, const PoseArgs* poses = nullptr)
{
    const int r = threadIdx.x >> 2, q = threadIdx.x & 3;
    const int cur = pass & 1;
    RaySetup R; int j, seg;
    {
        const int rr = r;
        int k = gx * kRaysPerBlock + rr;
        seg = seg_y;
        bool live = k < count;
        if (FIRST) {
            const int ns = P.set_mode ? P.n_groups * P.n_loc : P.n_seg;
            const int A = P.pass0_az, lgA = 31 - __builtin_clz(A), Sw = kRaysPerWave >> lgA;
            const int n_ab = (ns + A - 1) >> lgA;
            const int w = gx * (kRaysPerBlock / kRaysPerWave) + (rr >> 4), r16 = rr & 15;
            const int sb = w / n_ab, ab = w - sb * n_ab;
            k = sb * Sw + (r16 >> lgA); seg = (ab << lgA) + (r16 & (A - 1));
            live = k < P.n_beam && seg < ns;
            if (!live) { seg = 0; k = 0; }
            else if (P.set_mode) { const int g = seg / P.n_loc; seg = (int)P.group_frame[g] * P.n_loc + (seg - g * P.n_loc); }
        }
        j = -1;
        V3 orig = { 0.0f, 0.0f, 0.0f }, dir = { 1.0f, 0.0f, 0.0f };
        if (live) {
            const int bb = FIRST ? beam_base(P, seg / P.n_loc) : 0;
            uint2 tj = make_uint2(0u, 0u);
            if (!FIRST) tj = P.torder[cur][(size_t)seg * P.cap + k];
            j = FIRST ? (int)P.beam_order[bb + k] : (int)tj.x;
            if (FIRST) {
                const float4 b = P.beams[bb + j];
                dir = { b.x, b.y, b.z };
            } else {
                const uint32_t slot = tj.y;
                const size_t w = (size_t)seg * 2 * P.cap + slot;
                const float4 A = P.waves[cur].A[w], B = P.waves[cur].B[w];
                orig = { A.x, A.y, A.z };
                dir = { A.w, B.x, B.y };
            }
        }
        Quat q_am; V3 t_am;
        azimuth_frame<FIRST>(P, poses, seg, q_am, t_am);
        R = ray_setup(FIRST ? t_am : v_add(q_rot(q_am, orig), t_am), q_rot(q_am, dir));
    }
    const bool active = j >= 0;

    unsigned nn = 0, nt = 0;
    unsigned ws[4] = { 0, 0, 0, 0 };
    if (active) {
        const int gray = ((FIRST ? 0 : seg_y) * gdim_x + (int)gx) * kRaysPerBlock + r;
        Hit h;
        if constexpr (SL) h = traverse_stackless(reinterpret_cast<const float4*>(P.nodes), P.tri_base4, R, P.range_max, P.hit_pad);
        else h = traverse<STATS, SPILL, CULL>(reinterpret_cast<const float4*>(P.nodes), P.tri_base4, R, P.range_max, P.hit_pad, lds_stack, P.stack_lds,
                                              P.spill, P.spill_stride, gray, nn, nt, STATS ? ws : nullptr);
        if (q == 0) {
            const size_t hk = (size_t)seg * P.cap + j;
            P.hit[hk] = make_uint2(__float_as_uint((h.tri != 0xFFFFFFFFu) ? h.t : -1.0f), h.tri);
        }
    }
    if (STATS) {
        unsigned it = nt >> 16; nt &= 0xFFFFu;
        for (int off = 32; off > 0; off >>= 1) { nn += __shfl_down(nn, off); nt += __shfl_down(nt, off); it = max(it, (unsigned)__shfl_down(it, off)); }
        if ((threadIdx.x & 63) == 0) {
            atomicAdd(&P.counters->nodes, (unsigned long long)nn);
            atomicAdd(&P.counters->tris, (unsigned long long)nt);
            atomicAdd(&P.counters->wave_iters, (unsigned long long)it);
            atomicMax(&P.counters->max_iters, it);
            atomicAdd(&P.counters->n_waves, 1u);
        }
        unsigned a = ws[0], b = ws[1], c2 = ws[2], d2 = ws[3];
        for (int off = 32; off > 0; off >>= 1) {
            const unsigned a2 = __shfl_down(a, off), b2 = __shfl_down(b, off), c3 = __shfl_down(c2, off), d3 = __shfl_down(d2, off);
            if (a2 > a) { a = a2; b = b2; c2 = c3; d2 = d3; }
        }
        if ((threadIdx.x & 63) == 0) {
            atomicAdd(&P.counters->it_all, (unsigned long long)a);
            atomicAdd(&P.counters->it_node, (unsigned long long)b);
            atomicAdd(&P.counters->it_leaf, (unsigned long long)c2);
            atomicAdd(&P.counters->quad_steps, (unsigned long long)d2);
        }
    }
}

template <bool FIRST, bool STATS, bool SPILL, bool CULL, bool SL = false>
__global__ __launch_bounds__(kTraceThreads) void k_trace(const Params P, const int pass, const typename PosesOf<FIRST>::type poses)
{
    __builtin_amdgcn_s_setprio(2);
    extern __shared__ uint32_t lds_stack[];
    const int cur = pass & 1;
    if (FIRST && blockIdx.x == 0 && blockIdx.y == 0) {
        if (threadIdx.x == 0) P.counters->overflow = 0;
        if (P.grid_hint && threadIdx.x < kMaxPasses) P.grid_hint->ovf_n[threadIdx.x] = 0;
        if constexpr (FIRST) {
            float* table = reinterpret_cast<float*>(P.pose_table);
            for (int i = threadIdx.x; i < 8 * poses.n; i += kTraceThreads) table[i] = (i & 7) < 7 ? poses.p[i >> 3][i & 7] : 0.0f;
        }
    }
    int seg_y = (int)blockIdx.y, gx = (int)blockIdx.x, gdim = (int)gridDim.x;
    if (!FIRST && P.seg_chunk > 0) {
        gdim = P.trace_row;
        const int yy = (int)blockIdx.y, ch = yy / gdim;
        gx = yy - ch * gdim;
        seg_y = ch * P.seg_chunk + (int)blockIdx.x;
        if (seg_y >= P.n_seg) return;
    }
    const int count = FIRST ? 0 : (int)P.count[cur][seg_y];
    if (!FIRST && gx * kRaysPerBlock >= count) return;
    const PoseArgs* pa = nullptr;
    if constexpr (FIRST) pa = &poses;
    trace_group<FIRST, STATS, SPILL, CULL, SL>(P, pass, seg_y, gx, count, lds_stack, gdim, pa);
}

template <bool CULL>
__global__ __launch_bounds__(kTraceThreads) void k_trace_repair(const Params P, const int pass)
{
    extern __shared__ uint32_t lds_stack[];
    const uint32_t n = P.grid_hint->ovf_n[pass];
    if (n == 0) return;
    __builtin_amdgcn_s_setprio(2);
    const int tight = (int)P.tight_groups[pass];
    for (uint32_t i = 0; i < n; i++) {
        const int seg = (int)P.ovf_list[(size_t)pass * P.ovf_stride + i];
        const int count = (int)P.count[pass & 1][seg];
        for (int g = tight + (int)blockIdx.x; g * kRaysPerBlock < count; g += (int)gridDim.x) {
            trace_group<false, false, false, CULL>(P, pass, seg, g, count, lds_stack, 0);
            if (threadIdx.x == 0) atomicAdd(&P.grid_hint->repaired, 1ull);
        }
    }
}

template <bool CULL, bool STATS>
__global__ __launch_bounds__(kTraceThreads) void k_debug_trace(const Params P, const float* origs, const float* dirs, int n,
                                                               float* out_t, uint32_t* out_face, unsigned long long* steps)
{
    extern __shared__ uint32_t lds_stack[];
    const int i = blockIdx.x * kRaysPerBlock + (threadIdx.x >> 2);
    if (i >= n) return;
    const V3 o = { origs[3 * i], origs[3 * i + 1], origs[3 * i + 2] };
    const V3 d = { dirs[3 * i], dirs[3 * i + 1], dirs[3 * i + 2] };
    unsigned nn = 0, nt = 0;
    const RaySetup R = ray_setup(o, d);
    const Hit h = traverse<STATS, true, CULL>(reinterpret_cast<const float4*>(P.nodes), P.tri_base4, R, P.range_max, P.hit_pad, lds_stack, P.stack_lds,
                                  P.spill, P.spill_stride, i, nn, nt);
    if ((threadIdx.x & 3) == 0) {
        if (out_t) out_t[i] = (h.tri != 0xFFFFFFFFu) ? h.t : -1.0f;
        if (out_face) out_face[i] = h.face;
        if (STATS) atomicAdd(steps, (unsigned long long)(nt >> 16));
    }
}

__device__ inline float acosf_ref(float x) { return (float)acos((double)x); }

__device__ inline double fresnel_angle_limit(double v1, double v2)
{
    const double n1 = v2, n2 = v1;
    double angle_limit = 100.0;
    if (n1 > 0.0) { const double n21 = n2 / n1; if (fabs(n21) <= 1.0) angle_limit = asin(n21); }
    return angle_limit;
}
__global__ void k_mat_limits(const float4* materials, size_t n, double* limits)
{
    const size_t i = (size_t)blockIdx.x * blockDim.x + threadIdx.x;
    if (i < n) limits[i] = fresnel_angle_limit(0.3, (double)materials[i].x);
}
void launch_mat_limits(const float4* materials, size_t n, double* limits, hipStream_t s)
{
    if (n) hipLaunchKernelGGL(k_mat_limits, dim3((unsigned)((n + 63) / 64)), dim3(64), 0, s, materials, n, limits);
}

__device__ inline void fresnel_split(V3 n, const V3 d, const float incidence_f, const double energy, const double v1, const double v2,
                                     const double angle_limit, V3& rdir, double& renergy, V3& tdir, double& tenergy)
{
    const double polarization = 0.5;
    const double n1 = v2, n2 = v1;
    const double incidence_angle = (double)incidence_f;
    rdir = v_add(d, v_scale(v_scale(n, 2.0f), v_dot(v_neg(n), d)));
    tdir = { 0.0f, 0.0f, 0.0f };
    bool transmitted = false;
    if (n1 > 0.0) {
        if (incidence_angle <= angle_limit) {
            if (v_dot(n, d) > 0.0f) n = v_neg(n);
            if (n2 > 0.0) {
                const double n12 = n1 / n2;
                const double c = cos(incidence_angle);
                tdir = v_add(v_scale(d, (float)n12),
                             v_scale(n, (float)(n12 * c - sqrt(1 - n12 * n12 * (1 - c * c)))));
                transmitted = true;
            }
        }
    }
    double rs, rp;
    const double eps = 0.0001;
    if (!transmitted) {
        const double h = (double)1.57079637050628662109375f;
        const double ch = -0x1.777a5cf72ceccp-25, sh = 0x1.ffffffffffff7p-1;
        const double s = incidence_angle + h;
        if (s > M_PI - eps) { rs = 1.0; rp = 1.0; }
        else {
            double si, ci;
            sincos(incidence_angle, &si, &ci);
            const double a = si * ch, b = ci * sh, e = ci * ch, f = si * sh;
            const double sd = a - b, ss = a + b, cd = e + f, cs = e - f;
            rs = -sd / ss;
            rp = (sd / cd) / (ss / cs);
        }
    } else {
        const double refraction_angle = (double)acosf_ref(v_dot(tdir, v_neg(n)));
        const double s = incidence_angle + refraction_angle;
        if (s < eps) {
            rs = (n1 - n2) / (n1 + n2);
            rp = rs;
        } else if (s > M_PI - eps) {
            rs = 1.0; rp = 1.0;
        } else {
            const double df = incidence_angle - refraction_angle;
            double sd, cd, ss, cs;
            sincos(df, &sd, &cd);
            sincos(s, &ss, &cs);
            rs = -sd / ss;
            rp = (sd / cd) / (ss / cs);
        }
    }
    const double Rs = rs * rs, Rp = rp * rp;
    const double Reff = polarization * Rs + (1.0 - polarization) * Rp;
    const double Teff = 1.0 - Reff;
    renergy = Reff * energy;
    tenergy = Teff * energy;
}

__global__ void k_debug_fresnel(size_t n, const float* normals, const float* dirs, const double* energy, const double* v1, const float* v2,
                                float* out_rdir, double* out_re, float* out_tdir, double* out_te)
{
    const size_t i = (size_t)blockIdx.x * blockDim.x + threadIdx.x;
    if (i >= n) return;
    const V3 nrm = { normals[3 * i], normals[3 * i + 1], normals[3 * i + 2] }, d = { dirs[3 * i], dirs[3 * i + 1], dirs[3 * i + 2] };
    const float inc = acosf_ref(v_dot(v_neg(d), nrm));
    const double v2d = (double)v2[i];
    V3 rdir, tdir; double re, te;
    fresnel_split(nrm, d, inc, energy[i], v1[i], v2d, fresnel_angle_limit(v1[i], v2d), rdir, re, tdir, te);
    out_rdir[3 * i] = rdir.x; out_rdir[3 * i + 1] = rdir.y; out_rdir[3 * i + 2] = rdir.z;
    out_tdir[3 * i] = tdir.x; out_tdir[3 * i + 1] = tdir.y; out_tdir[3 * i + 2] = tdir.z;
    out_re[i] = re; out_te[i] = te;
}
void launch_debug_fresnel(size_t n, const float* normals, const float* dirs, const double* energy, const double* v1, const float* v2,
                          float* out_rdir, double* out_re, float* out_tdir, double* out_te, hipStream_t s)
{
    if (n) hipLaunchKernelGGL(k_debug_fresnel, dim3((unsigned)((n + 63) / 64)), dim3(64), 0, s, n, normals, dirs, energy, v1, v2, out_rdir, out_re, out_tdir, out_te);
}

__device__ inline float ct_lobe(float angle, float specular_exp)
{
    float sn, c;
    sincosf(angle, &sn, &c);
    if (!(c > 0.0f)) return 0.0f;
    float a2 = 2.0f / (specular_exp + 2.0f);
    a2 = fminf(fmaxf(a2, 1e-4f), 1.0f);
    const float cc = c * c;
    const float d = a2 * cc + sn * sn;
    const float D = a2 / (d * d);
    const float g1 = (2.0f * c) / (c + sqrtf(a2 + (1.0f - a2) * cc));
    return a2 * D * (g1 * g1);
}

__device__ inline float back_reflection_shader(float incidence_angle, float energy,
                                               float diffuse, float specular_fac, float specular_exp, int model)
{
    float I_specular;
    if (model == 1) I_specular = ct_lobe(incidence_angle, specular_exp);
    else {
        const float IdotR = cosf(incidence_angle);
        I_specular = powf(IdotR, specular_exp);
    }
    const float I_total = diffuse * 1.0f + specular_fac * I_specular;
    return I_total * energy;
}

__global__ void k_debug_brdf(size_t n, const float* __restrict__ in, int model, float* __restrict__ out)
{
    const size_t i = (size_t)blockIdx.x * blockDim.x + threadIdx.x;
    if (i < n) out[i] = back_reflection_shader(in[5 * i], in[5 * i + 1], in[5 * i + 2], in[5 * i + 3], in[5 * i + 4], model);
}
void launch_debug_brdf(size_t n, const float* in, int model, float* out, hipStream_t s)
{
    if (n) hipLaunchKernelGGL(k_debug_brdf, dim3((unsigned)((n + 63) / 64)), dim3(64), 0, s, n, in, model, out);
}

__device__ inline int signal_cell(double time, double resolution)
{
    const float half_time = (float)(time / 2.0);
    const float signal_dist = (float)(0.3 * (double)half_time);
    return (int)((double)signal_dist / resolution);
}

template <bool FIRST>
__global__ __launch_bounds__(64) void k_shade(const Params P, const int pass)
{
    const int seg = blockIdx.y;
    const int j = blockIdx.x * 64 + threadIdx.x;
    const int cur = pass & 1, nxt = cur ^ 1;
    const int count = FIRST ? P.n_beam : (int)P.count[cur][seg];
    if (j >= count) return;
    const int frame = seg / P.n_loc;
    const int np_f = passes_of(P, frame);
    const bool last = (pass == np_f - 1);

    const size_t base2 = (size_t)seg * 2 * P.cap;
    const size_t s0 = base2 + 2 * (size_t)j, s1 = s0 + 1;
    if (FIRST && pass >= np_f) {
        P.cflag[s0] = 0; P.cflag[s1] = 0;
        const SigRec none = { -1, 0.0f };
        P.sigtmp[s0] = none; P.sigtmp[s1] = none;
        return;
    }

    V3 orig = { 0.0f, 0.0f, 0.0f }, dir;
    double energy = 1.0, time = 0.0;
    uint32_t mat = 0;
    if (FIRST) {
        const float4 b = P.beams[beam_base(P, frame) + j];
        dir = { b.x, b.y, b.z };
    } else {
        const uint32_t slot = P.idx[cur][(size_t)seg * P.cap + j];
        const size_t w = base2 + slot;
        const float4 A = P.waves[cur].A[w], B = P.waves[cur].B[w];
        const double2 C = P.waves[cur].C[w];
        orig = { A.x, A.y, A.z };
        dir = { A.w, B.x, B.y };
        mat = __float_as_uint(B.z);
        energy = C.x; time = C.y;
    }

    uint8_t f0 = 0, f1 = 0;
    SigRec sg0 = { -1, 0.0f }, sg1 = { -1, 0.0f };

    const size_t hk = (size_t)((FIRST && P.set_mode) ? (int)P.group_frame[P.frame_beam[frame]] * P.n_loc + (seg - frame * P.n_loc) : seg) * P.cap + j;
    const uint2 hitrec = P.hit[hk];
    const float range = __uint_as_float(hitrec.x);
    if (range >= 0.0f)
    {
        f0 |= 4;
        const uint32_t tri = hitrec.y;
        const float4* tp = reinterpret_cast<const float4*>(P.tris + tri);
        const float4 tb = tp[1], tc = tp[2];
        const uint32_t obj_id = __float_as_uint(tb.w);
        const V3 e1 = { tb.x, tb.y, tb.z }, e2 = { tc.x, tc.y, tc.z };

        Quat q_am; V3 t_am;
        azimuth_frame<false>(P, nullptr, seg, q_am, t_am);
        V3 nint = v_normalize(v_cross(e1, e2));
        nint = q_rot(q_conj(q_am), nint);
        if (v_dot(dir, nint) > 0.0f) nint = v_neg(nint);
        const V3 normal = v_normalize(nint);

        const V3 dir_in = dir;
        orig = v_add(orig, v_scale(dir, range));
        time += (double)range / 0.3;

        bool ok = true;
        uint32_t mat_refr;
        if ((int)mat == P.material_id_air) {
            if (obj_id >= (uint32_t)P.n_objects) { ok = false; mat_refr = 0; }
            else mat_refr = (uint32_t)P.object_materials[obj_id];
        } else {
            mat_refr = (uint32_t)P.material_id_air;
        }
        if (ok && mat_refr >= (uint32_t)P.n_materials) ok = false;
        if (!ok) {
            atomicOr(&P.counters->overflow, 2u); atomicOr(P.sticky, 2u);
        } else {
            const float4 m = P.materials[(size_t)frame * P.mat_stride + mat_refr];
            const float v_refraction = (mat != mat_refr) ? m.x : (float)0.3;
            const double angle_limit = (mat != mat_refr) ? P.mat_limits[(size_t)frame * P.mat_stride + mat_refr] : P.limit_same;

            V3 rdir, tdir; double renergy, tenergy;
            const float incidence_angle = acosf_ref(v_dot(v_neg(dir_in), normal));
            fresnel_split(normal, dir_in, incidence_angle, energy, 0.3, (double)v_refraction, angle_limit, rdir, renergy, tdir, tenergy);

            const float skip_dist = 0.001f;
            if (renergy > (double)P.thr)
            {
                if (!last) {
                    f0 |= 1;
                    const V3 o2 = v_add(orig, v_scale(rdir, skip_dist));
                    const double t2 = time + (double)skip_dist / 0.3;
                    P.waves[nxt].A[s0] = make_float4(o2.x, o2.y, o2.z, rdir.x);
                    P.waves[nxt].B[s0] = make_float4(rdir.y, rdir.z, __uint_as_float(mat), 0.0f);
                    P.waves[nxt].C[s0] = make_double2(renergy, t2);
                }
                if ((int)mat == P.material_id_air)
                {
                    const float ret = back_reflection_shader(incidence_angle, (float)renergy, m.y, m.z, m.w, P.brdf_model);
                    if (pass == 0 || P.record_multi_reflection) {
                        const float time_back = (float)(time * 2.0);
                        sg0.cell = signal_cell((double)time_back, P.resolution);
                        sg0.strength = ret;
                        if (sg0.cell < 0) sg0.cell = -1;
                    }
                    if (pass > 0 && P.record_multi_path) {
                        const float dist = sqrtf(orig.x * orig.x + orig.y * orig.y + orig.z * orig.z);
                        const V3 dsh = { orig.x / dist, orig.y / dist, orig.z / dist };
                        const double time_to_sensor = (double)dist / 0.3;
                        const double sensor_view_scalar = (double)v_dot(dir_in, dsh);
                        const float ang = acosf_ref(v_dot(v_neg(rdir), dsh));
                        if (sensor_view_scalar > P.multipath_threshold) {
                            sg1.strength = back_reflection_shader(ang, (float)renergy, m.y, m.z, m.w, P.brdf_model);
                            sg1.cell = signal_cell(time + time_to_sensor, P.resolution);
                            if (sg1.cell < 0) sg1.cell = -1;
                        }
                    }
                }
            }
            if (!last && tenergy > (double)P.thr)
            {
                f1 |= 1;
                const V3 o2 = v_add(orig, v_scale(tdir, skip_dist));
                const double t2 = time + (double)skip_dist / 0.3;
                P.waves[nxt].A[s1] = make_float4(o2.x, o2.y, o2.z, tdir.x);
                P.waves[nxt].B[s1] = make_float4(tdir.y, tdir.z, __uint_as_float(mat_refr), 0.0f);
                P.waves[nxt].C[s1] = make_double2(tenergy, t2);
            }
        }
    }
    P.cflag[s0] = f0; P.cflag[s1] = f1;
    P.sigtmp[s0] = sg0; P.sigtmp[s1] = sg1;
}

__device__ inline int block_excl_scan(int v, int& total, int* lds )
{
    const int lane = threadIdx.x & 63, wid = threadIdx.x >> 6;
    int x = v;
    for (int off = 1; off < 64; off <<= 1) { const int y = __shfl_up(x, off); if (lane >= off) x += y; }
    if (lane == 63) lds[wid] = x;
    __syncthreads();
    int pre = 0, tot = 0;
    for (int w = 0; w < 4; w++) { const int s = lds[w]; if (w < wid) pre += s; tot += s; }
    __syncthreads();
    total = tot;
    return pre + x - v;
}

template <bool FIRST>
__global__ __launch_bounds__(256) void k_scan(const Params P, const int pass)
{
    __shared__ int lds[8];
    const int seg = blockIdx.x;
    const int cur = pass & 1, nxt = cur ^ 1;
    const int count = FIRST ? P.n_beam : (int)P.count[cur][seg];
    const int n_slots = 2 * count;
    const size_t base2 = (size_t)seg * 2 * P.cap;

    int n_child = 0;
    int n_sig = FIRST ? 0 : (int)P.sig_count[seg];
    const int sig_before = n_sig;
    int n_hit = 0, n_refl = 0, my_hits = 0;
    unsigned ovf = 0;
    uint8_t f_nx = 0; SigRec sr_nx = { -1, 0.0f };
    if ((int)threadIdx.x < n_slots) { f_nx = P.cflag[base2 + threadIdx.x]; sr_nx = P.sigtmp[base2 + threadIdx.x]; }
    for (int b = 0; b < n_slots; b += 256) {
        const int s = b + threadIdx.x;
        const uint8_t f = f_nx; const SigRec sr = sr_nx;
        f_nx = 0; sr_nx = { -1, 0.0f };
        if (s + 256 < n_slots) { f_nx = P.cflag[base2 + s + 256]; sr_nx = P.sigtmp[base2 + s + 256]; }
        const int hit = (f >> 2) & 1;
        const int c = f & 1;
        const int g = sr.cell >= 0 ? 1 : 0;
        int tot;
        const int pre = block_excl_scan(((s & 1) ? (c << 10) : c) | (g << 20), tot, lds);
        const int pos = n_child + (pre & 1023) + ((pre >> 10) & 1023);
        if (c) { if (pos < P.cap) { P.idx[nxt][(size_t)seg * P.cap + pos] = (uint32_t)s; P.refpos[base2 + s] = (uint32_t)pos; } else { ovf = 1; P.refpos[base2 + s] = 0xFFFFFFFFu; } }
        n_child += (tot & 1023) + ((tot >> 10) & 1023);
        n_refl += tot & 1023;
        const int spos = n_sig + ((pre >> 20) & 1023);
        if (g) { if (spos < P.sigcap) P.sig[(size_t)seg * P.sigcap + spos] = sr; else ovf = 1; }
        n_sig += (tot >> 20) & 1023;
        my_hits += hit;
    }
    {
        int tot;
        block_excl_scan(my_hits, tot, lds);
        n_hit = tot;
    }
    __syncthreads();
    {
        int n_refl_placed = 0;
        {
            n_refl_placed = n_refl;
            if (n_child > P.cap) {
                int mine = 0;
                for (int k = threadIdx.x; k < count; k += 256) {
                    const size_t sl = base2 + 2 * (size_t)k;
                    if ((P.cflag[sl] & 1) && P.refpos[sl] != 0xFFFFFFFFu) mine++;
                }
                int tot; block_excl_scan(mine, tot, lds); n_refl_placed = tot;
            }
        }
        int placed0 = 0, placed1 = 0;
        auto fetch = [&](int k, int& c0, int& c1, uint32_t& rp0, uint32_t& rp1, uint32_t& jp) {
            c0 = c1 = 0; rp0 = rp1 = 0xFFFFFFFFu; jp = 0;
            if (k < count) {
                const uint32_t j = FIRST ? P.beam_order2[beam_base(P, seg / P.n_loc) + k] : P.torder[cur][(size_t)seg * P.cap + k].x;
                const size_t sl = base2 + 2 * (size_t)j;
                const uint2 rp = *reinterpret_cast<const uint2*>(P.refpos + sl);
                const uint8_t f0 = P.cflag[sl], f1 = P.cflag[sl + 1];
                if (f0 & 1) { rp0 = rp.x; c0 = rp0 != 0xFFFFFFFFu; }
                if (f1 & 1) { rp1 = rp.y; c1 = rp1 != 0xFFFFFFFFu; }
                jp = j;
            }
        };
        int c0n, c1n; uint32_t rp0n, rp1n, jpn;
        fetch((int)threadIdx.x, c0n, c1n, rp0n, rp1n, jpn);
        for (int b = 0; b < count; b += 256) {
            const int c0 = c0n, c1 = c1n; const uint32_t rp0 = rp0n, rp1 = rp1n, jp = jpn;
            fetch(b + 256 + (int)threadIdx.x, c0n, c1n, rp0n, rp1n, jpn);
            int tot;
            const int pre = block_excl_scan(c0 | (c1 << 10), tot, lds);
            if (c0) P.torder[nxt][(size_t)seg * P.cap + placed0 + (pre & 1023)] = make_uint2(rp0, 2u * jp);
            if (c1) P.torder[nxt][(size_t)seg * P.cap + n_refl_placed + placed1 + ((pre >> 10) & 1023)] = make_uint2(rp1, 2u * jp + 1u);
            placed0 += tot & 1023; placed1 += (tot >> 10) & 1023;
        }
    }
    if (__syncthreads_or((int)ovf) && threadIdx.x == 0) { atomicOr(&P.counters->overflow, 1u); atomicOr(P.sticky, 1u); }
    if (threadIdx.x == 0) {
        P.count[nxt][seg] = (uint32_t)min(n_child, P.cap);
        if (P.grid_hint && pass + 1 < kMaxPasses) {
            const uint32_t cn = (uint32_t)min(n_child, P.cap);
            if (cn > P.grid_hint->hist[pass + 1]) atomicMax(&P.grid_hint->hist[pass + 1], cn);
            const uint32_t tg = P.tight_groups[pass + 1];
            if (tg && cn > tg * (uint32_t)kRaysPerBlock) {
                const uint32_t at = atomicAdd(&P.grid_hint->ovf_n[pass + 1], 1u);
                P.ovf_list[(size_t)(pass + 1) * P.ovf_stride + at] = (uint32_t)seg;
            }
        }
        P.sig_count[seg] = (uint32_t)min(n_sig, P.sigcap);
        SegStats st; st.wave_passes = (uint32_t)count; st.hits = (uint32_t)n_hit;
        st.signals = (uint32_t)(n_sig - sig_before); st.pad = 0;
        P.seg_stats[(size_t)pass * P.n_seg + seg] = st;
    }
}

__constant__ unsigned char c_perm[256] = {
    151, 160, 137, 91, 90, 15, 131, 13, 201, 95, 96, 53, 194, 233, 7, 225, 140, 36, 103, 30,
    69, 142, 8, 99, 37, 240, 21, 10, 23, 190, 6, 148, 247, 120, 234, 75, 0, 26, 197, 62,
    94, 252, 219, 203, 117, 35, 11, 32, 57, 177, 33, 88, 237, 149, 56, 87, 174, 20, 125, 136,
    171, 168, 68, 175, 74, 165, 71, 134, 139, 48, 27, 166, 77, 146, 158, 231, 83, 111, 229, 122,
    60, 211, 133, 230, 220, 105, 92, 41, 55, 46, 245, 40, 244, 102, 143, 54, 65, 25, 63, 161,
    1, 216, 80, 73, 209, 76, 132, 187, 208, 89, 18, 169, 200, 196, 135, 130, 116, 188, 159, 86,
    164, 100, 109, 198, 173, 186, 3, 64, 52, 217, 226, 250, 124, 123, 5, 202, 38, 147, 118, 126,
    255, 82, 85, 212, 207, 206, 59, 227, 47, 16, 58, 17, 182, 189, 28, 42, 223, 183, 170, 213,
    119, 248, 152, 2, 44, 154, 163, 70, 221, 153, 101, 155, 167, 43, 172, 9, 129, 22, 39, 253,
    19, 98, 108, 110, 79, 113, 224, 232, 178, 185, 112, 104, 218, 246, 97, 228, 251, 34, 242, 193,
    238, 210, 144, 12, 191, 179, 162, 241, 81, 51, 145, 235, 249, 14, 239, 107, 49, 192, 214, 31,
    181, 199, 106, 157, 184, 84, 204, 176, 115, 121, 50, 45, 127, 4, 150, 254, 138, 236, 205, 93,
    222, 114, 67, 29, 24, 72, 243, 141, 128, 195, 78, 66, 215, 61, 156, 180
};
__device__ inline double p_fade(double t) { return t * t * t * (t * (t * 6 - 15) + 10); }
__device__ inline double p_lerp(double t, double a, double b) { return a + t * (b - a); }
__device__ inline double2 p_grad_coef(int hash)
{
    const int h = hash & 15;
    const double su = (h & 1) == 0 ? 1.0 : -1.0, sv = (h & 2) == 0 ? 1.0 : -1.0;
    double a = 0.0, b = 0.0;
    if (h < 8) a = su; else b = su;
    if (h < 4) b = sv;
    else if (h == 12 || h == 14) a = sv;
    return make_double2(a, b);
}
__device__ inline double p_grad2(const double2 g, double x, double y) { return g.x * x + g.y * y; }
constexpr int kPerlinRow = 257;
struct PerlinCol { double v; const double2* t0; const double2* t1; };
__device__ inline void perlin_col_table(const unsigned char* pt, double sy, double2* t0, double2* t1,
                                        int tid, int n_threads)
{
    const int Y = (int)floor(sy) & 255;
    const double y = sy - floor(sy);
    for (int e = tid; e < 2 * kPerlinRow; e += n_threads) {
        const int row = e >= kPerlinRow ? 1 : 0;
        const int X = (e - row * kPerlinRow) & 255;
        const double2 g = p_grad_coef(pt[pt[(pt[X] + Y + row) & 255]]);
        (row ? t1 : t0)[e - row * kPerlinRow] = make_double2(g.x, g.y * (row ? y - 1 : y));
    }
}
__device__ inline double perlin_col(const PerlinCol& pc, double sx)
{
    const double fl = floor(sx);
    const int X = (int)fl & 255;
    const double x = sx - fl, x1 = x - 1;
    const double u = p_fade(x);
    const double2 e00 = pc.t0[X], e10 = pc.t0[X + 1], e01 = pc.t1[X], e11 = pc.t1[X + 1];
    return p_lerp(pc.v, p_lerp(u, e00.x * x + e00.y, e10.x * x1 + e10.y),
                        p_lerp(u, e01.x * x + e01.y, e11.x * x1 + e11.y));
}

__device__ inline float uniform01(uint32_t seed, uint32_t col, uint32_t i)
{
    unsigned long long z = ((unsigned long long)seed << 40) ^ ((unsigned long long)col << 20) ^ (unsigned long long)i;
    z += 0x9E3779B97F4A7C15ull;
    z = (z ^ (z >> 30)) * 0xBF58476D1CE4E5B9ull;
    z = (z ^ (z >> 27)) * 0x94D049BB133111EBull;
    z = z ^ (z >> 31);
    return (float)(z >> 40) * (1.0f / 16777216.0f);
}

__device__ inline uint8_t saturate_u8(float x)
{
    const float r = __builtin_amdgcn_fmed3f(__builtin_rintf(x), 0.0f, 255.0f);
    return (__builtin_fabsf(x) < 2147483648.0f) ? (uint8_t)(int)r : (uint8_t)0;
}

__global__ void k_decay_table(float* decay, int n_cells, double resolution, double energy_loss_d)
{
    const int i = blockIdx.x * blockDim.x + threadIdx.x;
    if (i >= n_cells) return;
    const float energy_loss = (float)energy_loss_d;
    const float x = (float)(((double)(float)i + 0.5) * resolution);
    decay[i] = expf(-energy_loss * x);
}
void launch_decay_table(float* decay, int n_cells, double resolution, double energy_loss, hipStream_t s)
{
    hipLaunchKernelGGL(k_decay_table, dim3((n_cells + 255) / 256), dim3(256), 0, s, decay, n_cells, resolution, energy_loss);
}

#ifndef RR_SIG_CHUNK
#define RR_SIG_CHUNK 1024
#endif
constexpr int kSigChunk = RR_SIG_CHUNK;

template <int kColThreads>
__global__ __launch_bounds__(kColThreads) void k_column(const Params P)
{
    constexpr int kColWaves = kColThreads / 64;
    extern __shared__ float lds_col[];
    constexpr int kWPad = 64;
    constexpr size_t kReplayBytes = kSigChunk * sizeof(SigRec) + (256 + 2 * kWPad) * sizeof(double) + kColWaves * 64 * sizeof(int2);
    constexpr size_t kNoiseBytes = 4 * kPerlinRow * sizeof(double2) + 256;
    constexpr size_t kUnionBytes = kReplayBytes > kNoiseBytes ? kReplayBytes : kNoiseBytes;
    __shared__ __align__(16) unsigned char s_union[kUnionBytes];
    SigRec* s_sig = reinterpret_cast<SigRec*>(s_union);
    double* s_w = reinterpret_cast<double*>(s_union + kSigChunk * sizeof(SigRec));
    int2 (*s_list)[64] = reinterpret_cast<int2 (*)[64]>(s_union + kSigChunk * sizeof(SigRec) + (256 + 2 * kWPad) * sizeof(double));
    double2* s_tab = reinterpret_cast<double2*>(s_union);
    unsigned char* s_perm = reinterpret_cast<unsigned char*>(s_tab + 4 * kPerlinRow);
    __shared__ unsigned long long s_tiles[2];
    __shared__ int s_odd;
    __shared__ float s_red[kColWaves];
    __shared__ int s_wcnt[kColWaves];

    const int seg = blockIdx.x;
    const int tid = threadIdx.x, lane = tid & 63, wid = tid >> 6;
    const int n_cells = P.n_cells;
    const int W = P.signal_denoising > 0 ? P.smear_w : 1;
    const int mode = P.signal_denoising > 0 ? P.smear_mode : 0;
    const int n_tiles = (n_cells + 63) >> 6;

    const int n_list = (P.n_passes > 1) ? (int)P.sig_count[seg] : 0;
    int count_last = 0;
    if (P.n_passes == 1) count_last = P.n_beam;
    else if (P.n_passes > 1) count_last = (int)P.count[(P.n_passes - 1) & 1][seg];
    const int n_slots = 2 * count_last;
    const int S = n_list + n_slots;
    const size_t base2 = (size_t)seg * 2 * P.cap;

    for (int i = tid; i < n_cells; i += kColThreads) lds_col[i] = 0.0f;
    for (int i = tid; i < 256 + 2 * kWPad; i += kColThreads) {
        const int k = i - kWPad;
        s_w[i] = (P.signal_denoising > 0 && k >= 0 && k < W) ? (double)P.smear[k] : 0.0;
    }
    __syncthreads();

    int n_valid_last = 0, n_hit_last = 0;
    float rmax = 0.0f;
    for (int c0 = 0; c0 < S; c0 += kSigChunk) {
        const int n_in = min(kSigChunk, S - c0);
        if (tid < 2) s_tiles[tid] = 0ull;
        if (tid == 2) s_odd = 0;
        int n = 0;
        unsigned long long tm0 = 0ull, tm1 = 0ull;
        bool odd = false;
        for (int r0 = 0; r0 < n_in; r0 += kColThreads) {
// ... 217 lines not shown
        const int w = t & 15, c = c0 + 4 * w;
#pragma unroll
        for (int k = 0; k < 4; k++) {
            const int r = (t >> 4) + 16 * k, a = a0 + r;
            uint32_t v = 0;
            if (a < n_angles && c < n_cells) {
                const uint32_t blk = __umulhi((uint32_t)a, magic);
                const uint32_t loc = (uint32_t)a - blk * (uint32_t)n_loc;
                v = *reinterpret_cast<const uint32_t*>(cols + (size_t)blk * block_stride + (size_t)loc * n_cells + c);
            }
            tile[r][w] = v;
        }
    }
    __syncthreads();
    {
        const int g = t & 15, a = a0 + 4 * g;
        int col = scroll + a;
        if (col >= n_angles) col -= n_angles;
#pragma unroll
        for (int k = 0; k < 4; k++) {
            const int r = (t >> 4) + 16 * k, c = c0 + r;
            if (a < n_angles && c < n_cells) {
                const int w = r >> 2, sh = 8 * (r & 3);
                const uint32_t b0 = (tile[4 * g + 0][w] >> sh) & 0xFFu, b1 = (tile[4 * g + 1][w] >> sh) & 0xFFu;
                const uint32_t b2 = (tile[4 * g + 2][w] >> sh) & 0xFFu, b3 = (tile[4 * g + 3][w] >> sh) & 0xFFu;
                *reinterpret_cast<uint32_t*>(img + (size_t)c * n_angles + col) = b0 | (b1 << 8) | (b2 << 16) | (b3 << 24);
            }
        }
    }
}

__global__ __launch_bounds__(256) void k_score(const uint8_t* __restrict__ imgs, const uint8_t* __restrict__ ref, size_t npx,
                                               unsigned long long* sse)
{
    const uint8_t* img = imgs + (size_t)blockIdx.y * npx;
    unsigned long long acc = 0;
    const size_t n16 = npx / 16, stride = (size_t)gridDim.x * blockDim.x;
    const bool aligned = ((reinterpret_cast<uintptr_t>(img) | reinterpret_cast<uintptr_t>(ref)) & 15u) == 0;
    size_t done = 0;
    if (aligned) {
        for (size_t i = (size_t)blockIdx.x * blockDim.x + threadIdx.x; i < n16; i += stride) {
            const uint4 a = reinterpret_cast<const uint4*>(img)[i], b = reinterpret_cast<const uint4*>(ref)[i];
            const uint32_t aw[4] = { a.x, a.y, a.z, a.w }, bw[4] = { b.x, b.y, b.z, b.w };
            uint32_t part = 0;
#pragma unroll
            for (int w = 0; w < 4; w++)
#pragma unroll
                for (int k = 0; k < 4; k++) {
                    const int d = (int)((aw[w] >> (8 * k)) & 0xFFu) - (int)((bw[w] >> (8 * k)) & 0xFFu);
                    part += (uint32_t)(d * d);
                }
            acc += part;
        }
        done = n16 * 16;
    }
    for (size_t i = done + (size_t)blockIdx.x * blockDim.x + threadIdx.x; i < npx; i += stride) {
        const int d = (int)img[i] - (int)ref[i];
        acc += (unsigned long long)(d * d);
    }
    for (int off = 32; off > 0; off >>= 1) acc += __shfl_down(acc, off);
    __shared__ unsigned long long s_part[4];
    if ((threadIdx.x & 63) == 0) s_part[threadIdx.x >> 6] = acc;
    __syncthreads();
    if (threadIdx.x == 0) atomicAdd(&sse[blockIdx.y], s_part[0] + s_part[1] + s_part[2] + s_part[3]);
}
constexpr int kCopyThreads = 256;
__global__ __launch_bounds__(kCopyThreads) void k_copy_host(const uint4* __restrict__ src, uint4* __restrict__ dst, size_t n16, int xcd)
{
    unsigned b = blockIdx.x, nb = gridDim.x;
    if (xcd >= 0) {
        if ((int)(b & 7u) != xcd) return;
        b >>= 3; nb >>= 3;
    }
    const size_t nthreads = (size_t)nb * kCopyThreads;
    for (size_t i = (size_t)b * kCopyThreads + threadIdx.x; i < n16; i += nthreads) {
        const uint4 v = src[i];
        dst[i] = v;
    }
}
void launch_copy_host(const void* src, void* dst, size_t bytes, int blocks, int xcd, hipStream_t s)
{
    const size_t n16 = bytes / 16;
    if (n16 == 0) return;
    unsigned g = (unsigned)std::max<size_t>(1, std::min<size_t>((size_t)blocks, (n16 + kCopyThreads - 1) / kCopyThreads));
    if (xcd >= 0) g *= 8u;
    hipLaunchKernelGGL(k_copy_host, dim3(g), dim3(kCopyThreads), 0, s, reinterpret_cast<const uint4*>(src), reinterpret_cast<uint4*>(dst), n16, xcd);
}

__global__ void k_store_u32(const uint32_t* __restrict__ src, uint32_t* __restrict__ dst) { *dst = *src; }
void launch_store_u32(const uint32_t* src, uint32_t* h_dst, hipStream_t s) { hipLaunchKernelGGL(k_store_u32, dim3(1), dim3(1), 0, s, src, h_dst); }

__global__ __launch_bounds__(256) void k_copy_words(const uint32_t* __restrict__ src, uint32_t* __restrict__ dst, size_t n)
{
    for (size_t i = (size_t)blockIdx.x * blockDim.x + threadIdx.x; i < n; i += (size_t)gridDim.x * blockDim.x) dst[i] = src[i];
}
void launch_copy_words(const void* src, void* dst, size_t bytes, hipStream_t s)
{
    const size_t n = bytes / 4;
    if (!n) return;
    const int g = (int)std::min<size_t>(256, (n + 255) / 256);
    hipLaunchKernelGGL(k_copy_words, dim3(g), dim3(256), 0, s, reinterpret_cast<const uint32_t*>(src), reinterpret_cast<uint32_t*>(dst), n);
}

void launch_score(const uint8_t* imgs, const uint8_t* ref, size_t npx, int n_images, unsigned long long* sse, hipStream_t s)
{
    const unsigned blocks = (unsigned)std::max<size_t>(1, std::min<size_t>(64, (npx / 16 + 255) / 256));
    hipLaunchKernelGGL(k_score, dim3(blocks, (unsigned)n_images), dim3(256), 0, s, imgs, ref, npx, sse);
}

__global__ void k_encode_refs(Node4* nodes, size_t n_children, uint32_t tri_base4)
{
    const size_t i = (size_t)blockIdx.x * blockDim.x + threadIdx.x;
    if (i >= n_children) return;
    uint32_t& ref = nodes[i >> 2].c[i & 3].ref;
    const uint32_t r = ref;
    if (r == kEmptyRef) return;
    if (r & kLeafFlag) ref = (r & 0xF0000000u) | (tri_base4 + 3u * (r & 0x0FFFFFFFu));
    else ref = r * 8u;
}
__global__ void k_tri_graze(TriRec* tris, size_t n)
{
    const size_t i = (size_t)blockIdx.x * blockDim.x + threadIdx.x;
    if (i >= n) return;
    const V3 e1 = { tris[i].e1[0], tris[i].e1[1], tris[i].e1[2] }, e2 = { tris[i].e2[0], tris[i].e2[1], tris[i].e2[2] };
    const V3 c = v_cross(e1, e2);
    tris[i].pad = __float_as_uint(2.5e-5f * v_dot(c, c));
}
__global__ void k_parent_links(Node4* nodes, size_t n_children)
{
    const size_t i = (size_t)blockIdx.x * blockDim.x + threadIdx.x;
    if (i == 0) nodes[0].c[0].pad = 0xFFFFFFFFu;
    if (i >= n_children) return;
    const uint32_t r = nodes[i >> 2].c[i & 3].ref;
    if (r == kEmptyRef || (r & kLeafFlag)) return;
    nodes[r >> 3].c[0].pad = (uint32_t)((i >> 2) << 3) | (uint32_t)(i & 3);
}
void launch_encode_refs(Node4* nodes, size_t n_nodes, uint32_t tri_base4, hipStream_t s, size_t n_tris)
{
    const size_t n = n_nodes * 4;
    if (n == 0) return;
    hipLaunchKernelGGL(k_encode_refs, dim3((unsigned)((n + 255) / 256)), dim3(256), 0, s, nodes, n, tri_base4);
    hipLaunchKernelGGL(k_parent_links, dim3((unsigned)((n + 255) / 256)), dim3(256), 0, s, nodes, n);
    if (n_tris) hipLaunchKernelGGL(k_tri_graze, dim3((unsigned)((n_tris + 255) / 256)), dim3(256), 0, s,
                                   reinterpret_cast<TriRec*>(reinterpret_cast<float4*>(nodes) + tri_base4), n_tris);
}

void launch_trace(const Params& P, int pass, const PoseArgs* poses, bool stats, hipStream_t s, hipEvent_t ev_start, hipEvent_t ev_stop,
                  hipEvent_t ev_rep_start, hipEvent_t ev_rep_stop, bool* repair_launched)
{
    if (repair_launched) *repair_launched = false;
    const int n_seg = (pass == 0 && P.set_mode) ? P.n_groups * P.n_loc : P.n_seg;
    const int A0 = P.pass0_az, Sw0 = kRaysPerWave / A0;
    const size_t waves0 = (size_t)((n_seg + A0 - 1) / A0) * (size_t)((P.n_beam + Sw0 - 1) / Sw0);
    const long bound = std::min<long>((long)P.cap, pass < 20 ? (long)P.n_beam << pass : (long)P.cap);
    const unsigned row = (pass > 0 && pass < kMaxPasses && P.tight_groups[pass]) ? (unsigned)P.tight_groups[pass]
                                                                               : (unsigned)((bound + kRaysPerBlock - 1) / kRaysPerBlock);
    const bool tightened = pass > 0 && pass < kMaxPasses && P.tight_groups[pass];
    const unsigned row_odd = (pass > 0 && P.spill_depth == 0 && !tightened) ? (row | 1u) : row;
    dim3 grid = pass == 0 ? dim3((unsigned)((waves0 + (kTraceThreads / 64) - 1) / (kTraceThreads / 64)))
                          : dim3(row_odd, n_seg);
    Params Pl = P;
    if (pass > 0 && P.seg_chunk > 0) {
        const unsigned S = (unsigned)P.seg_chunk, n_chunks = ((unsigned)n_seg + S - 1) / S;
        if ((size_t)n_chunks * row < 65535) { grid = dim3(S, n_chunks * row); Pl.trace_row = (int)row; }
        else Pl.seg_chunk = 0;
    }
    dim3 block(kTraceThreads);
    const bool cull = kCullPop && P.cull_pop && pass > 0 && (size_t)P.stack_lds * kRaysPerBlock * 6 <= 10240 / (128 / kTraceThreads);
    const size_t lds = (size_t)P.stack_lds * kRaysPerBlock * (cull ? 6 : 4);
    const bool spill = P.spill_depth > 0;
#define RR_LAUNCH_TRACE0(S, X) hipExtLaunchKernelGGL((k_trace<true, S, X, false>), grid, block, lds, s, ev_start, ev_stop, 0, Pl, pass, *poses)
#define RR_LAUNCH_TRACE(F, S, X, C) hipExtLaunchKernelGGL((k_trace<F, S, X, C>), grid, block, lds, s, ev_start, ev_stop, 0, Pl, pass, NoPoses{})
    if (P.stackless && !stats) {
        if (pass == 0) hipExtLaunchKernelGGL((k_trace<true, false, false, false, true>), grid, block, 0, s, ev_start, ev_stop, 0, Pl, pass, *poses);
        else hipExtLaunchKernelGGL((k_trace<false, false, false, false, true>), grid, block, 0, s, ev_start, ev_stop, 0, Pl, pass, NoPoses{});
    } else if (pass == 0) {
        if (stats) { if (spill) RR_LAUNCH_TRACE0(true, true); else RR_LAUNCH_TRACE0(true, false); }
        else       { if (spill) RR_LAUNCH_TRACE0(false, true); else RR_LAUNCH_TRACE0(false, false); }
    } else if (cull) {
        if (stats) { if (spill) RR_LAUNCH_TRACE(false, true, true, true); else RR_LAUNCH_TRACE(false, true, false, true); }
        else       { if (spill) RR_LAUNCH_TRACE(false, false, true, true); else RR_LAUNCH_TRACE(false, false, false, true); }
    } else {
        if (stats) { if (spill) RR_LAUNCH_TRACE(false, true, true, false); else RR_LAUNCH_TRACE(false, true, false, false); }
        else       { if (spill) RR_LAUNCH_TRACE(false, false, true, false); else RR_LAUNCH_TRACE(false, false, false, false); }
    }
#undef RR_LAUNCH_TRACE
#undef RR_LAUNCH_TRACE0
    if (pass > 0 && pass < kMaxPasses && P.tight_groups[pass]) {
        const dim3 rgrid(128);
        if (!ev_rep_start) {
            if (cull) hipLaunchKernelGGL((k_trace_repair<true>), rgrid, block, lds, s, Pl, pass);
            else      hipLaunchKernelGGL((k_trace_repair<false>), rgrid, block, lds, s, Pl, pass);
        } else if (cull) hipExtLaunchKernelGGL((k_trace_repair<true>), rgrid, block, lds, s, ev_rep_start, ev_rep_stop, 0, Pl, pass);
        else             hipExtLaunchKernelGGL((k_trace_repair<false>), rgrid, block, lds, s, ev_rep_start, ev_rep_stop, 0, Pl, pass);
        if (repair_launched) *repair_launched = true;
    }
}

void* trace0_kernel(bool spill, bool stackless)
{
    if (stackless) return (void*)k_trace<true, false, false, false, true>;
    return spill ? (void*)k_trace<true, false, true, false> : (void*)k_trace<true, false, false, false>;
}

void launch_shade(const Params& P, int pass, hipStream_t s, hipEvent_t ev_start, hipEvent_t ev_stop)
{
    const int cap_p = (int)std::min<long>((long)P.cap, pass < 20 ? (long)P.n_beam << pass : (long)P.cap);
    dim3 grid((cap_p + 63) / 64, P.n_seg), block(64);
    if (!ev_start) {
        if (pass == 0) hipLaunchKernelGGL((k_shade<true>), grid, block, 0, s, P, pass);
        else           hipLaunchKernelGGL((k_shade<false>), grid, block, 0, s, P, pass);
    } else if (pass == 0) hipExtLaunchKernelGGL((k_shade<true>), grid, block, 0, s, ev_start, ev_stop, 0, P, pass);
    else                  hipExtLaunchKernelGGL((k_shade<false>), grid, block, 0, s, ev_start, ev_stop, 0, P, pass);
}

void launch_scan(const Params& P, int pass, hipStream_t s, hipEvent_t ev_start, hipEvent_t ev_stop)
{
    dim3 grid(P.n_seg), block(256);
    if (!ev_start) {
        if (pass == 0) hipLaunchKernelGGL((k_scan<true>), grid, block, 0, s, P, pass);
        else           hipLaunchKernelGGL((k_scan<false>), grid, block, 0, s, P, pass);
    } else if (pass == 0) hipExtLaunchKernelGGL((k_scan<true>), grid, block, 0, s, ev_start, ev_stop, 0, P, pass);
    else                  hipExtLaunchKernelGGL((k_scan<false>), grid, block, 0, s, ev_start, ev_stop, 0, P, pass);
}

void launch_column(const Params& P, hipStream_t s, hipEvent_t ev_start, hipEvent_t ev_stop)
{
    dim3 grid(P.n_seg);
    const size_t lds = (((size_t)P.n_cells * sizeof(float)) + 15) & ~(size_t)15;
    if (!ev_start) {
        if (P.n_seg >= 1024) hipLaunchKernelGGL(k_column<256>, grid, dim3(256), lds, s, P);
        else hipLaunchKernelGGL(k_column<512>, grid, dim3(512), lds, s, P);
    } else if (P.n_seg >= 1024) hipExtLaunchKernelGGL(k_column<256>, grid, dim3(256), lds, s, ev_start, ev_stop, 0, P);
    else hipExtLaunchKernelGGL(k_column<512>, grid, dim3(512), lds, s, ev_start, ev_stop, 0, P);
}

void launch_assemble_u8(const uint8_t* cols, uint8_t* img, int n_angles, int n_cells, int scroll, hipStream_t s,
                        int n_loc, size_t block_stride, int n_frames, size_t frame_stride)
{
    dim3 grid((n_cells + 63) / 64, (n_angles + 63) / 64, n_frames > 0 ? n_frames : 1), block(256);
    if (n_loc <= 0) { n_loc = n_angles; block_stride = (size_t)n_angles * n_cells; }
    const int sc = ((scroll % n_angles) + n_angles) % n_angles;
    const bool aligned = ((reinterpret_cast<uintptr_t>(cols) | reinterpret_cast<uintptr_t>(img) | block_stride | frame_stride) & 3u) == 0;
    if (aligned && n_cells % 4 == 0 && n_angles % 4 == 0 && sc % 4 == 0 && n_angles < 65536 && n_loc > 1) {
        const uint32_t magic = (uint32_t)((1ull << 32) / (uint32_t)n_loc) + 1u;
        hipLaunchKernelGGL(k_assemble_u8x4, grid, block, 0, s, cols, img, n_angles, n_cells, sc, n_loc, magic,
                           block_stride, frame_stride);
        return;
    }
    hipLaunchKernelGGL((k_assemble<uint8_t>), grid, block, 0, s, cols, img, n_angles, n_cells, scroll, n_loc, block_stride,
                       frame_stride);
}

void launch_assemble_f32(const float* cols, float* img, int n_angles, int n_cells, int scroll, hipStream_t s)
{
    dim3 grid((n_cells + 63) / 64, (n_angles + 63) / 64), block(256);
    hipLaunchKernelGGL((k_assemble<float>), grid, block, 0, s, cols, img, n_angles, n_cells, scroll, n_angles, (size_t)n_angles * n_cells, (size_t)0);
}

void launch_debug_trace(const Params& P, const float* origs, const float* dirs, int n,
                        float* out_t, uint32_t* out_face, hipStream_t s, unsigned long long* steps)
{
    dim3 grid((n + kRaysPerBlock - 1) / kRaysPerBlock), block(kTraceThreads);
    const bool cull = kCullPop && P.cull_pop;
    const size_t lds = (size_t)P.stack_lds * kRaysPerBlock * (cull ? 6 : 4);
    if (steps) {
        if (cull) hipLaunchKernelGGL((k_debug_trace<true, true>), grid, block, lds, s, P, origs, dirs, n, out_t, out_face, steps);
        else hipLaunchKernelGGL((k_debug_trace<false, true>), grid, block, lds, s, P, origs, dirs, n, out_t, out_face, steps);
    } else {
        if (cull) hipLaunchKernelGGL((k_debug_trace<true, false>), grid, block, lds, s, P, origs, dirs, n, out_t, out_face, steps);
        else hipLaunchKernelGGL((k_debug_trace<false, false>), grid, block, lds, s, P, origs, dirs, n, out_t, out_face, steps);
    }
}

}
```

### radarays_ros_amd/csrc/rr_probe.hip

```cpp
#include "rr_ctx.h"
#include <algorithm>
#include <cstdio>
#include <cstring>
#include <cstdlib>

extern "C" {

int rr_get_stats(rr_ctx* c, rr_stats* st)
{
    if (!c || !st) return -1;
    RR_HIP(c, hipSetDevice(c->device));
    RR_HIP(c, hipDeviceSynchronize());
    std::memset(st, 0, sizeof(*st));
    Lane& L = c->lanes[c->last_lane];
    if (!L.d_counters.p) return 0;
    Counters h;
    { const int rcb = read_counters(c, h); if (rcb) return rcb; }
    st->nodes_visited = h.nodes; st->tris_tested = h.tris; st->overflow = h.overflow;
    if (getenv("RR_TRACE_STATS")) fprintf(stderr, "[rr stats] waves %u wave_iters %llu (avg %.1f) max_iters %u\n", h.n_waves, h.wave_iters, h.n_waves ? (double)h.wave_iters / h.n_waves : 0.0, h.max_iters);
    if (getenv("RR_TRACE_STATS") && h.n_waves)
        fprintf(stderr, "[rr stats] per wave: iterations %.2f, issuing node path %.2f, leaf path %.2f, live quad-steps %.1f (of 16 x iterations = %.1f)\n",
                (double)h.it_all / h.n_waves, (double)h.it_node / h.n_waves, (double)h.it_leaf / h.n_waves,
                (double)h.quad_steps / h.n_waves, 16.0 * h.it_all / h.n_waves);
    const size_t n = (size_t)L.last_n_seg * (size_t)L.last_n_passes;
    if (n && L.d_seg_stats.p) {
        std::vector<SegStats> ss(n);
        { const int rcb = read_back(c, ss.data(), L.d_seg_stats.p, n * sizeof(SegStats)); if (rcb) return rcb; }
        for (const SegStats& x : ss) { st->wave_passes += x.wave_passes; st->hits += x.hits; st->signals += x.signals; }
    }
    return 0;
}

int rr_set_stats_mode(rr_ctx* c, int enable) { if (!c) return -1; c->stats_mode = enable != 0; return 0; }

int rr_get_traversal_shape(rr_ctx* c, uint64_t out[8])
{
    if (!c || !out) return -1;
    RR_HIP(c, hipSetDevice(c->device));
    RR_HIP(c, hipDeviceSynchronize());
    std::memset(out, 0, 8 * sizeof(uint64_t));
    Lane& L = c->lanes[c->last_lane];
    if (!L.d_counters.p) return 0;
    Counters h;
    { const int rcb = read_counters(c, h); if (rcb) return rcb; }
    out[0] = h.n_waves; out[1] = h.it_all; out[2] = h.it_node; out[3] = h.it_leaf; out[4] = h.quad_steps; out[5] = h.max_iters;
    out[6] = h.nodes; out[7] = h.quad_steps > h.nodes ? h.quad_steps - h.nodes : 0;
    return 0;
}
int rr_set_timing_mode(rr_ctx* c, int enable) { if (!c) return -1; c->timing = enable; return 0; }

int rr_get_kernel_time(rr_ctx* c, const char* kernel, double* total_ms, uint64_t* launches, int reset)
{
    if (!c || !kernel) return -1;
    RR_HIP(c, hipSetDevice(c->device));
    RR_HIP(c, hipDeviceSynchronize());
    KernelTimer& t = c->timers[kernel];
    for (auto& p : t.pending) {
        float ms = 0.0f;
        if (hipEventElapsedTime(&ms, p.first, p.second) == hipSuccess) { t.total_ms += ms; t.launches++; t.samples_ms.push_back(ms); }
        c->event_pool.push_back(p.first); c->event_pool.push_back(p.second);
    }
    t.pending.clear();
    if (total_ms) *total_ms = t.total_ms;
    if (launches) *launches = t.launches;
    if (reset) { t.total_ms = 0.0; t.launches = 0; t.samples_ms.clear(); }
    return 0;
}

int rr_get_kernel_samples(rr_ctx* c, const char* kernel, float* out_ms, size_t capacity, size_t* n_out)
{
    if (!c || !kernel || !n_out) return -1;
    int rc = rr_get_kernel_time(c, kernel, nullptr, nullptr, 0); if (rc) return rc;
    const KernelTimer& t = c->timers[kernel];
    *n_out = t.samples_ms.size();
    if (out_ms) for (size_t i = 0; i < t.samples_ms.size() && i < capacity; i++) out_ms[i] = t.samples_ms[i];
    return 0;
}

int rr_reserve_timing_events(rr_ctx* c, size_t n)
{
    if (!c) return -1;
    RR_HIP(c, hipSetDevice(c->device));
    while (c->event_pool.size() < n) { hipEvent_t e = nullptr; RR_HIP(c, hipEventCreate(&e)); c->event_pool.push_back(e); }
    return 0;
}

int rr_get_trace_grid(rr_ctx* c, uint32_t out_rows[24], uint32_t out_hist[24], uint64_t* repaired_groups)
{
    if (!c) return -1;
    static_assert(kMaxPasses == 24, "rr_get_trace_grid's arrays");
    RR_HIP(c, hipSetDevice(c->device));
    RR_HIP(c, hipDeviceSynchronize());
    const Lane& L = c->lanes[c->last_lane];
    uint64_t rep = 0;
    for (int k = 0; k < kMaxPasses; k++) { if (out_rows) out_rows[k] = L.last_rows[k]; if (out_hist) out_hist[k] = 0; }
    for (const Lane& o : c->lanes) {
        if (!o.d_hint.p || o.hist_gen != c->hist_gen) continue;
        GridHint h;
        RR_HIP(c, hipMemcpy(&h, o.d_hint.p, sizeof(h), hipMemcpyDeviceToHost));
        rep += h.repaired;
        for (int k = 0; k < kMaxPasses && out_hist; k++) out_hist[k] = std::max(out_hist[k], h.hist[k]);
    }
    if (repaired_groups) *repaired_groups = rep;
    return 0;
}

int rr_get_graph_stats(rr_ctx* c, uint64_t* captures, uint64_t* replays)
{
    if (!c) return -1;
    if (captures) *captures = c->graph_captures;
    if (replays) *replays = c->graph_replays;
    return 0;
}

int rr_debug_fresnel(rr_ctx* c, size_t n, const float* normals, const float* dirs, const double* energy, const double* v1, const float* v2,
                     float* out_refl_dir, double* out_refl_energy, float* out_refr_dir, double* out_refr_energy)
{
    if (!c) return -1;
    if (n == 0) return 0;
    if (!normals || !dirs || !energy || !v1 || !v2 || !out_refl_dir || !out_refl_energy || !out_refr_dir || !out_refr_energy)
        return fail(c, -3, "rr_debug_fresnel: null pointer");
    RR_HIP(c, hipSetDevice(c->device));
    DevBuf<float> d_n, d_d, d_v2, d_rd, d_td; DevBuf<double> d_e, d_v1, d_re, d_te;
    hipError_t e = d_n.ensure(3 * n);
    if (e == hipSuccess) e = d_d.ensure(3 * n);
    if (e == hipSuccess) e = d_v2.ensure(n);
    if (e == hipSuccess) e = d_rd.ensure(3 * n);
    if (e == hipSuccess) e = d_td.ensure(3 * n);
    if (e == hipSuccess) e = d_e.ensure(n);
    if (e == hipSuccess) e = d_v1.ensure(n);
    if (e == hipSuccess) e = d_re.ensure(n);
    if (e == hipSuccess) e = d_te.ensure(n);
    if (e == hipSuccess) e = hipMemcpy(d_n.p, normals, 3 * n * sizeof(float), hipMemcpyHostToDevice);
    if (e == hipSuccess) e = hipMemcpy(d_d.p, dirs, 3 * n * sizeof(float), hipMemcpyHostToDevice);
    if (e == hipSuccess) e = hipMemcpy(d_v2.p, v2, n * sizeof(float), hipMemcpyHostToDevice);
    if (e == hipSuccess) e = hipMemcpy(d_e.p, energy, n * sizeof(double), hipMemcpyHostToDevice);
    if (e == hipSuccess) e = hipMemcpy(d_v1.p, v1, n * sizeof(double), hipMemcpyHostToDevice);
    if (e == hipSuccess) {
        launch_debug_fresnel(n, d_n.p, d_d.p, d_e.p, d_v1.p, d_v2.p, d_rd.p, d_re.p, d_td.p, d_te.p, c->stream);
        e = hipGetLastError();
        if (e == hipSuccess) e = hipStreamSynchronize(c->stream);
    }
    if (e == hipSuccess) e = hipMemcpy(out_refl_dir, d_rd.p, 3 * n * sizeof(float), hipMemcpyDeviceToHost);
    if (e == hipSuccess) e = hipMemcpy(out_refr_dir, d_td.p, 3 * n * sizeof(float), hipMemcpyDeviceToHost);
    if (e == hipSuccess) e = hipMemcpy(out_refl_energy, d_re.p, n * sizeof(double), hipMemcpyDeviceToHost);
    if (e == hipSuccess) e = hipMemcpy(out_refr_energy, d_te.p, n * sizeof(double), hipMemcpyDeviceToHost);
    d_n.release(); d_d.release(); d_v2.release(); d_rd.release(); d_td.release(); d_e.release(); d_v1.release(); d_re.release(); d_te.release();
    if (e != hipSuccess) return fail(c, -100, std::string("rr_debug_fresnel: ") + hipGetErrorString(e));
    return 0;
}

int rr_debug_brdf(rr_ctx* c, size_t n, const float* in5, int brdf_model, float* out)
{
    if (!c) return -1;
    if (n == 0) return 0;
    if (!in5 || !out) return fail(c, -3, "rr_debug_brdf: null pointer");
    if (brdf_model != 0 && brdf_model != 1) return fail(c, -3, "rr_debug_brdf: brdf_model must be 0 or 1");
    RR_HIP(c, hipSetDevice(c->device));
    DevBuf<float> d_in, d_out;
    hipError_t e = d_in.ensure(5 * n);
    if (e == hipSuccess) e = d_out.ensure(n);
    if (e == hipSuccess) e = hipMemcpy(d_in.p, in5, 5 * n * sizeof(float), hipMemcpyHostToDevice);
    if (e == hipSuccess) {
        launch_debug_brdf(n, d_in.p, brdf_model, d_out.p, c->stream);
        e = hipGetLastError();
        if (e == hipSuccess) e = hipStreamSynchronize(c->stream);
    }
    if (e == hipSuccess) e = hipMemcpy(out, d_out.p, n * sizeof(float), hipMemcpyDeviceToHost);
    d_in.release(); d_out.release();
    if (e != hipSuccess) return fail(c, -100, std::string("rr_debug_brdf: ") + hipGetErrorString(e));
    return 0;
}

int rr_debug_trace(rr_ctx* c, const float* origs, const float* dirs, size_t n, float* out_t, uint32_t* out_face)
{
    if (!c) return -1;
    if (!c->have_mesh) return fail(c, -2, "rr_set_mesh has not been called");
    if (n == 0) return 0;
    if (!origs || !dirs || !out_t || !out_face) return fail(c, -3, "rr_debug_trace: null pointer");
    RR_HIP(c, hipSetDevice(c->device));
    const size_t chunk = 1u << 16;
    const int stack_lds = (int)std::max<uint32_t>(1, std::min<uint32_t>(c->stack_need, (uint32_t)c->stack_lds_max));
    const int spill_depth = (int)c->stack_need - stack_lds;
    DevBuf<float> d_o, d_d, d_t; DevBuf<uint32_t> d_f, d_spill;
    RR_HIP(c, d_o.ensure(3 * chunk)); RR_HIP(c, d_d.ensure(3 * chunk)); RR_HIP(c, d_t.ensure(chunk));
    RR_HIP(c, d_f.ensure(chunk)); RR_HIP(c, d_spill.ensure(spill_depth > 0 ? (size_t)spill_depth * chunk : 1));
    Params P; std::memset(&P, 0, sizeof(P));
    P.nodes = reinterpret_cast<const Node4*>(c->d_bvh.p); P.tris = reinterpret_cast<const TriRec*>(c->d_bvh.p + c->tri_base4);
    P.tri_base4 = c->tri_base4; P.range_max = c->have_cfg ? c->cfg.range_max : 1000.0f; P.hit_pad = c->hit_pad;
    P.spill = d_spill.p; P.spill_stride = (int)chunk; P.stack_lds = stack_lds; P.spill_depth = std::max(0, spill_depth);
    P.cull_pop = c->cull_pop;
    int rc = 0;
    for (size_t b = 0; b < n && !rc; b += chunk) {
        const size_t m = std::min(chunk, n - b);
        hipError_t e = hipMemcpy(d_o.p, origs + 3 * b, 3 * m * sizeof(float), hipMemcpyHostToDevice);
        if (e == hipSuccess) e = hipMemcpy(d_d.p, dirs + 3 * b, 3 * m * sizeof(float), hipMemcpyHostToDevice);
        if (e == hipSuccess) { launch_debug_trace(P, d_o.p, d_d.p, (int)m, d_t.p, d_f.p, c->stream); e = hipStreamSynchronize(c->stream); }
        if (e == hipSuccess) e = hipMemcpy(out_t + b, d_t.p, m * sizeof(float), hipMemcpyDeviceToHost);
        if (e == hipSuccess) e = hipMemcpy(out_face + b, d_f.p, m * sizeof(uint32_t), hipMemcpyDeviceToHost);
// ... 8 lines not shown
```

### radarays_ros_amd/native.py

```python
import ctypes as C
import os
import subprocess

import numpy as np

_HERE = os.path.dirname(os.path.abspath(__file__))
LIB_PATH = os.environ.get("RADARAYS_MI355_LIB") or os.path.join(_HERE, "libradarays_mi355.so")
_LIB = None

SYMBOLS = [
    "rr_abi_version", "rr_default_config", "rr_create", "rr_destroy", "rr_last_error",
    "rr_set_mesh", "rr_set_mesh_gpu", "rr_copy_mesh", "rr_set_materials", "rr_set_config", "rr_set_beam_samples",
    "rr_set_noise_offsets", "rr_set_motion_poses", "rr_simulate", "rr_simulate_columns_device", "rr_simulate_batch_columns_device",
    "rr_assemble_image_device", "rr_assemble_blocks_device", "rr_assemble_frames_device", "rr_simulate_device",
    "rr_simulate_material_sets_device", "rr_simulate_material_sets", "rr_simulate_batch_device", "rr_synchronize", "rr_get_stats",
    "rr_set_stats_mode", "rr_debug_trace", "rr_debug_fresnel", "rr_debug_brdf", "rr_get_bvh_info", "rr_get_trace_grid", "rr_get_graph_stats", "rr_set_timing_mode",
    "rr_get_kernel_time", "rr_get_kernel_samples", "rr_reserve_timing_events",
    "rr_simulate_batch_host_async", "rr_wait_host", "rr_host_alloc", "rr_host_free", "rr_copy_to_host_async", "rr_deliver_to_host_async", "rr_host_delivery_route", "rr_partition", "rr_multi_plan",
    "rr_create_multi", "rr_destroy_multi", "rr_multi_last_error", "rr_multi_device_count", "rr_multi_rccl_version", "rr_multi_ctx",
    "rr_multi_set_mesh", "rr_multi_set_mesh_gpu", "rr_multi_set_materials", "rr_multi_set_config", "rr_multi_set_beam_samples",
    "rr_multi_set_noise_offsets", "rr_multi_set_motion_poses", "rr_multi_simulate", "rr_multi_simulate_batch",
    "rr_multi_simulate_batch_async", "rr_multi_wait", "rr_peek_error_bits_async", "rr_get_traversal_shape",
    "rr_cone_dirs", "rr_sample_cone_local", "rr_load_mesh_file", "rr_mesh_reorder_objects", "rr_free_mesh",
    "rr_simulate_param_sets_device", "rr_simulate_param_sets", "rr_score_images_device",
    "rr_set_object_poses", "rr_update_vertices", "rr_get_tree_cost", "rr_rebuild_tree",
    "rr_multi_set_object_poses", "rr_multi_update_vertices", "rr_multi_rebuild_tree",
    "rr_default_detect_config", "rr_detect_device", "rr_detect", "rr_polar_to_cartesian_device", "rr_polar_to_cartesian",
]


class RRMaterial(C.Structure):
    _fields_ = [("velocity", C.c_float), ("ambient", C.c_float),
                ("diffuse", C.c_float), ("specular", C.c_float)]


class RRConfig(C.Structure):
    _fields_ = [
        ("n_cells", C.c_int32), ("n_angles", C.c_int32), ("n_reflections", C.c_int32),
        ("signal_denoising", C.c_int32),
        ("signal_denoising_triangular_width", C.c_int32),
        ("signal_denoising_gaussian_width", C.c_int32),
        ("signal_denoising_mb_width", C.c_int32),
        ("ambient_noise", C.c_int32), ("scroll_image", C.c_int32),
        ("record_multi_reflection", C.c_int32), ("record_multi_path", C.c_int32),
        ("max_waves_per_azimuth", C.c_int32), ("brdf_model", C.c_int32), ("reserved_", C.c_int32),
        ("resolution", C.c_double), ("energy_max", C.c_double), ("signal_max", C.c_double),
        ("signal_denoising_triangular_mode", C.c_double),
        ("signal_denoising_gaussian_mode", C.c_double),
        ("signal_denoising_mb_mode", C.c_double),
        ("ambient_noise_at_signal_0", C.c_double), ("ambient_noise_at_signal_1", C.c_double),
        ("ambient_noise_energy_max", C.c_double), ("ambient_noise_energy_min", C.c_double),
        ("ambient_noise_energy_loss", C.c_double), ("multipath_threshold", C.c_double),
        ("wave_energy_threshold", C.c_float), ("theta_min", C.c_float),
        ("theta_inc", C.c_float), ("range_max", C.c_float),
    ]


class RRParamSet(C.Structure):
    _fields_ = [("materials", C.c_void_p), ("beam_dirs", C.c_void_p), ("n_reflections", C.c_int32), ("reserved_", C.c_int32)]


class RRMesh(C.Structure):
    _fields_ = [("verts", C.POINTER(C.c_float)), ("n_verts", C.c_size_t), ("faces", C.POINTER(C.c_uint32)), ("n_faces", C.c_size_t),
                ("face_object_id", C.POINTER(C.c_uint32)), ("n_objects", C.c_size_t), ("object_names", C.POINTER(C.c_char_p))]


class RRDetectConfig(C.Structure):
    _fields_ = [("method", C.c_int32), ("guard_cells", C.c_int32), ("train_cells", C.c_int32), ("k", C.c_int32),
                ("min_intensity", C.c_int32), ("min_bin", C.c_int32), ("cfar_scale", C.c_float), ("reserved_", C.c_int32)]


class RRRadarPoint(C.Structure):
    _fields_ = [("x", C.c_float), ("y", C.c_float), ("z", C.c_float), ("intensity", C.c_float),
                ("column", C.c_uint32), ("bin", C.c_uint32)]


class RRCartesianConfig(C.Structure):
    _fields_ = [("width", C.c_int32), ("interpolation", C.c_int32), ("pixel_size", C.c_float), ("reserved_", C.c_int32)]


POINT_DTYPE = np.dtype([("x", "<f4"), ("y", "<f4"), ("z", "<f4"), ("intensity", "<f4"), ("column", "<u4"), ("bin", "<u4")])

DETECT_DEFAULTS = {"method": 0, "guard_cells": 2, "train_cells": 16, "k": 12, "min_intensity": 1, "min_bin": 0, "cfar_scale": 3.0}
DETECT_METHODS = {"cfar": 0, "ca-cfar": 0, "kstrongest": 1, "k-strongest": 1, 0: 0, 1: 1}


class RRStats(C.Structure):
    _fields_ = [("wave_passes", C.c_uint64), ("hits", C.c_uint64), ("signals", C.c_uint64),
                ("nodes_visited", C.c_uint64), ("tris_tested", C.c_uint64),
                ("overflow", C.c_uint32), ("pad_", C.c_uint32)]

    def asdict(self):
        return {k: getattr(self, k) for k, _ in self._fields_ if k != "pad_"}


def build(force=False):
    src = os.path.join(_HERE, "csrc")
    srcs = [os.path.join(src, f) for f in os.listdir(src)] + [os.path.join(_HERE, "..", "include", "radarays_mi355.h")]
    stale = (not os.path.exists(LIB_PATH)) or any(os.path.getmtime(f) > os.path.getmtime(LIB_PATH) for f in srcs)
    if force or stale:
        subprocess.run(["make", "-C", src], check=True, stdout=subprocess.DEVNULL)
    return LIB_PATH


def lib():
    global _LIB
    if _LIB is not None:
        return _LIB
    if not os.path.exists(LIB_PATH):
        raise RuntimeError(
            "radarays_ros_amd: %s is missing -- build it with __graft_entry__.build() "
            "(hipcc --offload-arch=gfx950). There is no CPU fallback." % LIB_PATH)
    try:
        import torch
    except Exception:
        pass
    L = C.CDLL(LIB_PATH)
    vp = C.c_void_p
    L.rr_abi_version.restype = C.c_int
    L.rr_default_config.argtypes = [C.POINTER(RRConfig)]
    L.rr_create.restype = vp
    L.rr_create.argtypes = [C.c_int]
    L.rr_destroy.argtypes = [vp]
    L.rr_last_error.restype = C.c_char_p
    L.rr_last_error.argtypes = [vp]
    L.rr_set_mesh.argtypes = [vp, vp, C.c_size_t, vp, C.c_size_t, vp]
    L.rr_set_mesh_gpu.argtypes = [vp, vp, C.c_size_t, vp, C.c_size_t, vp]
    L.rr_copy_mesh.argtypes = [vp, vp]
    L.rr_set_materials.argtypes = [vp, vp, C.c_size_t, vp, C.c_size_t, C.c_int32]
    L.rr_set_config.argtypes = [vp, C.POINTER(RRConfig)]
    L.rr_set_beam_samples.argtypes = [vp, vp, C.c_size_t]
    L.rr_set_noise_offsets.argtypes = [vp, vp, C.c_size_t]
    L.rr_set_motion_poses.argtypes = [vp, vp, C.c_size_t]
    L.rr_simulate.argtypes = [vp, vp, C.c_int, C.c_int, vp, vp, C.POINTER(RRStats)]
    L.rr_simulate_columns_device.argtypes = [vp, vp, C.c_int, C.c_int, vp, vp, vp]
    L.rr_simulate_batch_columns_device.argtypes = [vp, vp, C.c_int, C.c_int, C.c_int, vp, vp]
    L.rr_assemble_image_device.argtypes = [vp, vp, vp, vp]
    L.rr_assemble_blocks_device.argtypes = [vp, vp, C.c_int, C.c_size_t, vp, vp]
    L.rr_assemble_frames_device.argtypes = [vp, vp, C.c_int, C.c_size_t, C.c_int, C.c_size_t, vp, vp]
    L.rr_simulate_device.argtypes = [vp, vp, vp, vp]
    L.rr_simulate_material_sets_device.argtypes = [vp, vp, vp, C.c_int, C.c_size_t, vp, vp]
    L.rr_simulate_material_sets.argtypes = [vp, vp, vp, C.c_int, C.c_size_t, vp]
    L.rr_simulate_batch_device.argtypes = [vp, vp, C.c_int, vp, vp]
    L.rr_synchronize.argtypes = [vp, vp]
    L.rr_get_stats.argtypes = [vp, C.POINTER(RRStats)]
    L.rr_set_stats_mode.argtypes = [vp, C.c_int]
    L.rr_set_timing_mode.argtypes = [vp, C.c_int]
    L.rr_get_kernel_time.argtypes = [vp, C.c_char_p, C.POINTER(C.c_double), C.POINTER(C.c_uint64), C.c_int]
    L.rr_debug_trace.argtypes = [vp, vp, vp, C.c_size_t, vp, vp]
    L.rr_debug_fresnel.argtypes = [vp, C.c_size_t, vp, vp, vp, vp, vp, vp, vp, vp, vp]
    L.rr_debug_brdf.argtypes = [vp, C.c_size_t, vp, C.c_int, vp]
    L.rr_get_trace_grid.argtypes = [vp, vp, vp, C.POINTER(C.c_uint64)]
    L.rr_get_graph_stats.argtypes = [vp, C.POINTER(C.c_uint64), C.POINTER(C.c_uint64)]
    L.rr_get_bvh_info.argtypes = [vp, C.POINTER(C.c_uint64), C.POINTER(C.c_uint64),
                                  C.POINTER(C.c_uint32), C.POINTER(C.c_uint32)]
    L.rr_get_kernel_samples.argtypes = [vp, C.c_char_p, vp, C.c_size_t, C.POINTER(C.c_size_t)]
    L.rr_reserve_timing_events.argtypes = [vp, C.c_size_t]
    L.rr_simulate_batch_host_async.argtypes = [vp, vp, C.c_int, vp, vp]
    L.rr_wait_host.argtypes = [vp, vp]
    L.rr_copy_to_host_async.argtypes = [vp, vp, vp, C.c_size_t, vp]
    L.rr_deliver_to_host_async.argtypes = [vp, vp, vp, C.c_size_t, vp]
    L.rr_host_delivery_route.argtypes = [vp]
    L.rr_host_alloc.restype = vp
    L.rr_host_alloc.argtypes = [C.c_size_t]
    L.rr_host_free.argtypes = [vp]
    L.rr_host_free.restype = None
    L.rr_partition.argtypes = [C.c_int, C.c_int, C.c_int, C.POINTER(C.c_int), C.POINTER(C.c_int)]
    L.rr_partition.restype = None
    L.rr_multi_plan.argtypes = [C.c_int, C.c_int, C.c_int, C.c_int, C.POINTER(C.c_int), C.POINTER(C.c_size_t), vp, vp, vp]
    L.rr_create_multi.restype = vp
    L.rr_create_multi.argtypes = [C.POINTER(C.c_int), C.c_int]
    L.rr_destroy_multi.argtypes = [vp]
    L.rr_destroy_multi.restype = None
    L.rr_multi_last_error.restype = C.c_char_p
    L.rr_multi_last_error.argtypes = [vp]
    L.rr_multi_device_count.argtypes = [vp]
    L.rr_multi_rccl_version.argtypes = [vp]
    L.rr_multi_ctx.restype = vp
    L.rr_multi_ctx.argtypes = [vp, C.c_int]
    L.rr_multi_set_mesh.argtypes = [vp, vp, C.c_size_t, vp, C.c_size_t, vp]
    L.rr_multi_set_mesh_gpu.argtypes = [vp, vp, C.c_size_t, vp, C.c_size_t, vp]
    L.rr_multi_set_materials.argtypes = [vp, vp, C.c_size_t, vp, C.c_size_t, C.c_int32]
    L.rr_multi_set_config.argtypes = [vp, C.POINTER(RRConfig)]
    L.rr_multi_set_beam_samples.argtypes = [vp, vp, C.c_size_t]
    L.rr_multi_set_noise_offsets.argtypes = [vp, vp, C.c_size_t]
    L.rr_multi_set_motion_poses.argtypes = [vp, vp, C.c_size_t]
    L.rr_multi_simulate.argtypes = [vp, vp, vp]
    L.rr_multi_simulate_batch.argtypes = [vp, vp, C.c_int, vp]
    L.rr_multi_simulate_batch_async.argtypes = [vp, vp, C.c_int, vp]
    L.rr_multi_wait.argtypes = [vp, vp]
    L.rr_peek_error_bits_async.argtypes = [vp, vp, vp]
    L.rr_get_traversal_shape.argtypes = [vp, vp]
    L.rr_simulate_param_sets_device.argtypes = [vp, vp, C.POINTER(RRParamSet), C.c_int, C.c_size_t, vp, vp]
    L.rr_simulate_param_sets.argtypes = [vp, vp, C.POINTER(RRParamSet), C.c_int, C.c_size_t, vp, vp, vp]
    L.rr_score_images_device.argtypes = [vp, vp, C.c_int, vp, vp, vp, vp]
    L.rr_cone_dirs.argtypes = [C.c_float, C.c_int, C.c_float, vp, vp, C.c_size_t, vp]
    L.rr_sample_cone_local.argtypes = [C.c_uint32, C.c_float, C.c_size_t, C.c_int, C.c_float, vp]
    L.rr_load_mesh_file.argtypes = [C.c_char_p, C.POINTER(RRMesh), C.c_char_p, C.c_size_t]
    L.rr_free_mesh.argtypes = [C.POINTER(RRMesh)]
    L.rr_mesh_reorder_objects.argtypes = [C.POINTER(RRMesh), C.POINTER(C.c_char_p), C.c_size_t, C.c_char_p, C.c_size_t]
    L.rr_free_mesh.restype = None
    L.rr_set_object_poses.argtypes = [vp, vp, C.c_size_t]
    L.rr_update_vertices.argtypes = [vp, vp, C.c_size_t]
    L.rr_get_tree_cost.argtypes = [vp, C.POINTER(C.c_double), C.POINTER(C.c_double)]
    L.rr_rebuild_tree.argtypes = [vp, C.c_int]
    L.rr_multi_set_object_poses.argtypes = [vp, vp, C.c_size_t]
    L.rr_multi_update_vertices.argtypes = [vp, vp, C.c_size_t]
    L.rr_multi_rebuild_tree.argtypes = [vp, C.c_int]
    L.rr_default_detect_config.argtypes = [C.POINTER(RRDetectConfig)]
    L.rr_default_detect_config.restype = None
    L.rr_detect_device.argtypes = [vp, vp, C.c_int, C.POINTER(RRDetectConfig), vp, C.c_int, vp, vp]
    L.rr_detect.argtypes = [vp, vp, C.c_int, C.POINTER(RRDetectConfig), vp, C.c_int, vp]
    L.rr_polar_to_cartesian_device.argtypes = [vp, vp, C.c_int, C.POINTER(RRCartesianConfig), vp, vp]
    L.rr_polar_to_cartesian.argtypes = [vp, vp, C.c_int, C.POINTER(RRCartesianConfig), vp]
    for n in SYMBOLS:
        getattr(L, n)
    _LIB = L
    return L


def _rows(a, width, what):
    x = np.asarray(a)
    if x.dtype.kind not in "fiu":
        raise ValueError("%s must be real numbers, got dtype %s" % (what, x.dtype))
    if not ((x.ndim == 2 and x.shape[1] == width) or (x.ndim == 1 and x.size % width == 0)):
        raise ValueError("%s must have shape [n][%d], got %s" % (what, width, x.shape))
    return np.ascontiguousarray(x, np.float32).reshape(-1, width)


def object_poses_array(poses):
    return _rows(poses, 7, "object poses")


def vertex_array(verts):
    return _rows(verts, 3, "vertices")


def builder_id(builder):
    b = {"host": 0, "gpu": 1, 0: 0, 1: 1}.get(builder) if isinstance(builder, (str, int)) else None
    if b is None:
        raise ValueError("builder must be 'host' or 'gpu', got %r" % (builder,))
    return b


def make_config(cfg, n_angles=400, max_waves_per_azimuth=0, wave_energy_threshold=0.001,
                ray_range_max=1000.0, brdf_model=0):
    c = RRConfig()
    lib().rr_default_config(C.byref(c))
    c.n_cells = int(cfg.n_cells)
    c.n_angles = int(n_angles)
    c.n_reflections = int(cfg.n_reflections)
    c.signal_denoising = int(cfg.signal_denoising)
    c.signal_denoising_triangular_width = int(cfg.signal_denoising_triangular_width)
    c.signal_denoising_gaussian_width = int(cfg.signal_denoising_gaussian_width)
    c.signal_denoising_mb_width = int(cfg.signal_denoising_mb_width)
    c.ambient_noise = int(cfg.ambient_noise)
    c.scroll_image = int(cfg.scroll_image)
    c.record_multi_reflection = int(bool(cfg.record_multi_reflection))
    c.record_multi_path = int(bool(cfg.record_multi_path))
    c.max_waves_per_azimuth = int(max_waves_per_azimuth)
    c.brdf_model = int(brdf_model)
    for k in ("resolution", "energy_max", "signal_max", "signal_denoising_triangular_mode",
              "signal_denoising_gaussian_mode", "signal_denoising_mb_mode",
              "ambient_noise_at_signal_0", "ambient_noise_at_signal_1",
              "ambient_noise_energy_max", "ambient_noise_energy_min",
              "ambient_noise_energy_loss", "multipath_threshold"):
        setattr(c, k, float(getattr(cfg, k)))
    c.wave_energy_threshold = float(np.float32(wave_energy_threshold))
    c.theta_min = 0.0
    c.theta_inc = float(np.float32(-(2.0 * np.pi) / n_angles))
    c.range_max = float(ray_range_max)
    return c


class RRError(RuntimeError):
    pass


def _int_in(v, lo, hi, what):
    if isinstance(v, bool) or not isinstance(v, (int, np.integer)) or not lo <= int(v) <= hi:
        raise ValueError("%s must be an integer in [%d, %d], got %r" % (what, lo, hi, v))
    return int(v)


def detect_config(cfg=None, n_cells=None, **kw):
    d = dict(DETECT_DEFAULTS)
    if isinstance(cfg, RRDetectConfig):
        d.update({k: getattr(cfg, k) for k in DETECT_DEFAULTS})
    elif isinstance(cfg, dict):
        d.update(cfg)
    elif cfg is not None:
        raise ValueError("detection config must be an RRDetectConfig or a dict, got %r" % (cfg,))
    d.update(kw)
    unknown = set(d) - set(DETECT_DEFAULTS)
    if unknown:
        raise ValueError("unknown detection config fields: %s" % sorted(unknown))
    m = DETECT_METHODS.get(d["method"]) if isinstance(d["method"], (str, int)) and not isinstance(d["method"], bool) else None
    if m is None:
        raise ValueError("method must be 0 / 'cfar' or 1 / 'kstrongest', got %r" % (d["method"],))
    top = int(n_cells) if n_cells is not None else 8192
    c = RRDetectConfig()
    c.method = m
    c.guard_cells = _int_in(d["guard_cells"], 0, 1024, "guard_cells")
    c.train_cells = _int_in(d["train_cells"], 1, 1024, "train_cells")
    c.k = _int_in(d["k"], 1, top, "k")
    c.min_intensity = _int_in(d["min_intensity"], 0, 255, "min_intensity")
    c.min_bin = _int_in(d["min_bin"], 0, top - 1, "min_bin")
    try:
        scale = float(d["cfar_scale"])
    except (TypeError, ValueError):
        raise ValueError("cfar_scale must be a number, got %r" % (d["cfar_scale"],))
    with np.errstate(over="ignore"):
        finite = bool(np.isfinite(np.float32(scale)))
    if not (finite and scale >= 0.0):
        raise ValueError("cfar_scale must be finite and >= 0, got %r" % (scale,))
    c.cfar_scale = scale
    return c


def cartesian_config(width, pixel_size, bilinear=True):
    c = RRCartesianConfig()
    c.width = _int_in(width, 1, 8192, "width")
    try:
        ps = float(pixel_size)
    except (TypeError, ValueError):
        raise ValueError("pixel_size must be a number, got %r" % (pixel_size,))
    with np.errstate(over="ignore", under="ignore"):
        ok = bool(np.isfinite(np.float32(ps)) and ps > 0.0 and np.float32(ps) > 0.0)
    if not ok:
        raise ValueError("pixel_size must be finite and > 0, got %r" % (pixel_size,))
    c.pixel_size = ps
    c.interpolation = 1 if bilinear else 0
    return c


def _frames_arg(n_frames):
    return _int_in(n_frames, 1, 65535, "n_frames")


class Context:

    def __init__(self, device=0):
        self._L = lib()
        self._h = self._L.rr_create(int(device))
        if not self._h:
            raise RRError(self._L.rr_last_error(None).decode())
        self.device = int(device)
        self.cfg = None
        self.n_angles = 400

    def close(self):
        if getattr(self, "_h", None):
            self._L.rr_destroy(self._h)
            self._h = None

    def __del__(self):
        try:
            self.close()
        except Exception:
            pass

    def _ck(self, rc):
        if rc != 0:
            raise RRError("%s (rc=%d)" % (self._L.rr_last_error(self._h).decode(), rc))

    def set_mesh(self, verts, faces, face_object_id=None, builder="host"):
        v = np.ascontiguousarray(verts, np.float32).reshape(-1, 3)
        f = np.ascontiguousarray(faces, np.uint32).reshape(-1, 3)
        o = None if face_object_id is None else np.ascontiguousarray(face_object_id, np.uint32)
        if o is not None and len(o) != len(f):
            raise ValueError("face_object_id must have one entry per face")
        fn = {"host": self._L.rr_set_mesh, "gpu": self._L.rr_set_mesh_gpu}[builder]
        self._ck(fn(self._h, v.ctypes.data, len(v), f.ctypes.data, len(f), None if o is None else o.ctypes.data))

    def copy_mesh(self, src):
        self._ck(self._L.rr_copy_mesh(self._h, src._h))

    def set_object_poses(self, poses):
        p = object_poses_array(poses)
        self._ck(self._L.rr_set_object_poses(self._h, p.ctypes.data, len(p)))

    def update_vertices(self, verts):
        v = vertex_array(verts)
        self._ck(self._L.rr_update_vertices(self._h, v.ctypes.data, len(v)))

    def tree_cost(self):
        a, b = C.c_double(), C.c_double()
        self._ck(self._L.rr_get_tree_cost(self._h, C.byref(a), C.byref(b)))
        return a.value, b.value

    def rebuild_tree(self, builder="host"):
        b = builder_id(builder)
        self._ck(self._L.rr_rebuild_tree(self._h, b))

    def set_materials(self, materials, object_materials, material_id_air=0):
        m = (RRMaterial * len(materials))(*[RRMaterial(*[float(x) for x in (t.astuple() if hasattr(t, "astuple") else t)])
                                            for t in materials])
        om = np.ascontiguousarray(object_materials, np.int32)
        self._ck(self._L.rr_set_materials(self._h, m, len(materials), om.ctypes.data, len(om), int(material_id_air)))

    def set_config(self, cfg, n_angles=400, **kw):
        self.cfg = cfg
        self.n_angles = n_angles
        self._rrcfg = make_config(cfg, n_angles, **kw)
        self._ck(self._L.rr_set_config(self._h, C.byref(self._rrcfg)))

    def set_beam_samples(self, dirs):
        d = np.ascontiguousarray(dirs, np.float32).reshape(-1, 3)
        self._ck(self._L.rr_set_beam_samples(self._h, d.ctypes.data, len(d)))

    def set_noise_offsets(self, rnd):
        r = np.ascontiguousarray(rnd, np.float32).ravel()
        self._ck(self._L.rr_set_noise_offsets(self._h, r.ctypes.data, r.size))

    def set_motion_poses(self, poses):
        if poses is None or len(poses) == 0:
            self._ck(self._L.rr_set_motion_poses(self._h, None, 0))
            return
        p = np.ascontiguousarray(poses, np.float32).reshape(-1, 7)
        self._ck(self._L.rr_set_motion_poses(self._h, p.ctypes.data, len(p)))

    def simulate(self, pose, az_begin=0, az_end=None, want_f32=False):
        p = np.ascontiguousarray(pose, np.float32)
        assert p.shape == (7,)
        if az_end is None:
            az_end = self.n_angles
        n_cells = self.cfg.n_cells if self.cfg is not None else 1
        u8 = np.zeros((n_cells, self.n_angles), np.uint8)
        f32 = np.zeros((n_cells, self.n_angles), np.float32) if want_f32 else None
        st = RRStats()
        self._ck(self._L.rr_simulate(self._h, p.ctypes.data, az_begin, az_end, u8.ctypes.data,
                                     None if f32 is None else f32.ctypes.data, C.byref(st)))
        return u8, f32, st.asdict()

    def simulate_into(self, pose, out_u8):
        p = np.ascontiguousarray(pose, np.float32)
        self._ck(self._L.rr_simulate(self._h, p.ctypes.data, 0, self.n_angles, out_u8.ctypes.data, None, None))

    def traversal_shape(self):
        a = np.zeros(8, np.uint64)
        self._ck(self._L.rr_get_traversal_shape(self._h, a.ctypes.data))
        return dict(zip(("waves", "iterations", "node_path_issues", "leaf_path_issues", "live_quad_steps", "max_iterations",
                         "node_steps", "leaf_steps"), (int(x) for x in a)))

    def simulate_columns_device(self, pose, az_begin, az_end, d_cols_u8_ptr, d_cols_f32_ptr=None, stream=None):
        p = np.ascontiguousarray(pose, np.float32)
        self._ck(self._L.rr_simulate_columns_device(self._h, p.ctypes.data, az_begin, az_end,
                                                    d_cols_u8_ptr, d_cols_f32_ptr, stream))

    def simulate_batch_device(self, poses, d_imgs_ptr, stream=None):
        p = np.ascontiguousarray(poses, np.float32).reshape(-1, 7)
        self._ck(self._L.rr_simulate_batch_device(self._h, p.ctypes.data, len(p), d_imgs_ptr, stream))

    def simulate_batch_host_async(self, poses, h_imgs_ptr, stream=None):
        p = np.ascontiguousarray(poses, np.float32).reshape(-1, 7)
        self._ck(self._L.rr_simulate_batch_host_async(self._h, p.ctypes.data, len(p), h_imgs_ptr, stream))

    def wait_host(self, h_imgs_ptr=None):
        self._ck(self._L.rr_wait_host(self._h, h_imgs_ptr))

    def copy_to_host_async(self, d_src_ptr, h_dst_ptr, nbytes, stream=None):
        self._ck(lib().rr_copy_to_host_async(self._h, C.c_void_p(d_src_ptr), C.c_void_p(h_dst_ptr), C.c_size_t(nbytes), C.c_void_p(stream)))

    def host_delivery_route(self):
        return {2: "sdma", 1: "sdma (untried)", 0: "stream copies"}.get(int(lib().rr_host_delivery_route(self._h)), "?")

    def deliver_to_host_async(self, d_src_ptr, h_dst_ptr, nbytes, stream=None):
        self._ck(lib().rr_deliver_to_host_async(self._h, C.c_void_p(d_src_ptr), C.c_void_p(h_dst_ptr), C.c_size_t(nbytes), C.c_void_p(stream)))

    def simulate_batch_columns_device(self, poses, az_begin, az_end, d_cols_u8_ptr, stream=None):
        p = np.ascontiguousarray(poses, np.float32).reshape(-1, 7)
        self._ck(self._L.rr_simulate_batch_columns_device(self._h, p.ctypes.data, len(p), az_begin, az_end,
                                                          d_cols_u8_ptr, stream))

    def assemble_image_device(self, d_cols_u8_ptr, d_img_ptr, stream=None):
        self._ck(self._L.rr_assemble_image_device(self._h, d_cols_u8_ptr, d_img_ptr, stream))

    def assemble_blocks_device(self, d_cols_u8_ptr, n_loc, block_stride, d_img_ptr, stream=None):
        self._ck(self._L.rr_assemble_blocks_device(self._h, d_cols_u8_ptr, int(n_loc), int(block_stride), d_img_ptr, stream))

    def assemble_frames_device(self, d_cols_u8_ptr, n_loc, block_stride, n_frames, frame_stride, d_imgs_ptr, stream=None):
        self._ck(self._L.rr_assemble_frames_device(self._h, d_cols_u8_ptr, int(n_loc), int(block_stride), int(n_frames),
                                                   int(frame_stride), d_imgs_ptr, stream))

    @staticmethod
    def _material_sets(sets):
        a = np.ascontiguousarray(np.asarray(sets, dtype=np.float32))
        if a.ndim != 3 or a.shape[2] != 4:
            raise ValueError("material sets must have shape [n_sets][n_materials][4] (velocity, ambient, diffuse, specular)")
        return a

    def simulate_material_sets_device(self, pose, sets, d_imgs_ptr, stream=None):
        a = self._material_sets(sets)
        p = np.ascontiguousarray(pose, dtype=np.float32)
        self._ck(self._L.rr_simulate_material_sets_device(self._h, p.ctypes.data, a.ctypes.data, a.shape[0], a.shape[1], d_imgs_ptr, stream))

    def simulate_material_sets(self, pose, sets):
        a = self._material_sets(sets)
        p = np.ascontiguousarray(pose, dtype=np.float32)
        n_cells = self.cfg.n_cells if self.cfg is not None else 1
        out = np.zeros((a.shape[0], n_cells, self.n_angles), dtype=np.uint8)
        self._ck(self._L.rr_simulate_material_sets(self._h, p.ctypes.data, a.ctypes.data, a.shape[0], a.shape[1], out.ctypes.data))
        return out

    @staticmethod
    def _param_sets(sets):
        keep, n_mat = [], None
        arr = (RRParamSet * len(sets))()
        for k, st in enumerate(sets):
            m = st.get("materials")
            if m is not None:
                m = np.ascontiguousarray(np.asarray([(t.astuple() if hasattr(t, "astuple") else t) for t in m], dtype=np.float32))
                if m.ndim != 2 or m.shape[1] != 4:
                    raise ValueError("materials of a set must have shape [n_materials][4]")
                n_mat = m.shape[0] if n_mat is None else n_mat
                keep.append(m)
                arr[k].materials = m.ctypes.data
            b = st.get("beam_dirs")
            if b is not None:
                b = np.ascontiguousarray(b, np.float32).reshape(-1, 3)
                keep.append(b)
                arr[k].beam_dirs = b.ctypes.data
            nr = st.get("n_reflections")
            arr[k].n_reflections = -1 if nr is None else int(nr)
        return arr, keep, n_mat

    def simulate_param_sets(self, pose, sets, n_materials, ref_u8=None, want_images=True):
        arr, keep, n_mat = self._param_sets(sets)
        p = np.ascontiguousarray(pose, dtype=np.float32)
        n_cells = self.cfg.n_cells if self.cfg is not None else 1
        out = np.zeros((len(sets), n_cells, self.n_angles), dtype=np.uint8) if want_images else None
        psnr = ref = None
        if ref_u8 is not None:
            ref = np.ascontiguousarray(ref_u8, np.uint8)
            if ref.shape != (n_cells, self.n_angles):
                raise ValueError("reference image must be [n_cells][n_angles] uint8")
            psnr = np.zeros(len(sets), np.float64)
        self._ck(self._L.rr_simulate_param_sets(self._h, p.ctypes.data, arr, len(sets), int(n_materials),
                                                None if out is None else out.ctypes.data,
                                                None if ref is None else ref.ctypes.data, None if psnr is None else psnr.ctypes.data))
        return out, psnr

    def simulate_param_sets_device(self, pose, sets, n_materials, d_imgs_ptr, stream=None):
        arr, keep, _ = self._param_sets(sets)
        p = np.ascontiguousarray(pose, dtype=np.float32)
        self._ck(self._L.rr_simulate_param_sets_device(self._h, p.ctypes.data, arr, len(sets), int(n_materials), d_imgs_ptr, stream))

    def score_images_device(self, d_imgs_ptr, n_images, d_ref_ptr, stream=None, want_sse=False):
        psnr = np.zeros(n_images, np.float64); sse = np.zeros(n_images, np.uint64)
        self._ck(self._L.rr_score_images_device(self._h, d_imgs_ptr, int(n_images), d_ref_ptr, psnr.ctypes.data, sse.ctypes.data, stream))
        return (psnr, sse) if want_sse else psnr

    def simulate_device(self, pose, d_img_ptr, stream=None):
        p = np.ascontiguousarray(pose, np.float32)
        self._ck(self._L.rr_simulate_device(self._h, p.ctypes.data, d_img_ptr, stream))

    def _polar_shape(self):
        if self.cfg is None:
            raise RRError("rr_set_config has not been called")
        return int(self.cfg.n_cells), int(self.n_angles)

    def _polar_images(self, imgs):
        n_cells, n_angles = self._polar_shape()
        x = np.asarray(imgs)
        if x.dtype != np.uint8:
            raise ValueError("polar images must be uint8, got dtype %s" % x.dtype)
        if x.ndim == 2:
            x = x[None]
        if x.ndim != 3 or x.shape[1:] != (n_cells, n_angles) or not 1 <= x.shape[0] <= 65535:
            raise ValueError("polar images must have shape [n][%d][%d] (n in 1..65535), got %s" % (n_cells, n_angles, np.asarray(imgs).shape))
        return np.ascontiguousarray(x)

    def detect_device(self, d_imgs_ptr, n_frames, cfg=None, d_points_ptr=None, max_points=0, d_offsets_ptr=None, stream=None, **kw):
        n_cells, _ = self._polar_shape()
        c = detect_config(cfg, n_cells=n_cells, **kw)
        n = _frames_arg(n_frames)
        mp = _int_in(max_points, 0, 2**31 - 1, "max_points")
        if not d_imgs_ptr or not d_offsets_ptr or (mp > 0 and not d_points_ptr):
            raise ValueError("detect_device needs image and offset buffers (and a point buffer when max_points > 0)")
        self._ck(self._L.rr_detect_device(self._h, d_imgs_ptr, n, C.byref(c), d_points_ptr, mp, d_offsets_ptr, stream))

    def detect(self, imgs, cfg=None, max_points=None, allow_truncation=False, **kw):
        x = self._polar_images(imgs)
        n_cells, n_angles = self._polar_shape()
        c = detect_config(cfg, n_cells=n_cells, **kw)
        n = len(x)
        offs = np.zeros((n, n_angles + 1), np.uint32)
        if max_points is None:
            self._ck(self._L.rr_detect(self._h, x.ctypes.data, n, C.byref(c), None, 0, offs.ctypes.data))
            max_points = int(offs[:, -1].max())
        mp = _int_in(max_points, 0, 2**31 - 1, "max_points")
        pts = np.zeros((n, max(mp, 1)), POINT_DTYPE)
        self._ck(self._L.rr_detect(self._h, x.ctypes.data, n, C.byref(c), pts.ctypes.data if mp else None, mp, offs.ctypes.data))
        totals = offs[:, -1]
        over = np.nonzero(totals > mp)[0]
        if len(over) and not allow_truncation:
            f = int(over[0])
# ... 272 lines not shown
```

Before: 4647 images/s.

## Use any-hit traversal for final-pass rays whose output only needs hit existence

On the last pass, rays that do not travel in air (or when multi-reflection and multi-path recording are off) are marked dead: shading only records whether they hit anything. Traversal breaks at the first intersection for them instead of searching for the closest one. The sort stage splits the next-pass trace order into a live region and a 16-aligned dead region, so whole blocks run the cheaper any-hit path. This adds a per-segment live count buffer, extra scans in the sort kernel, padding of the grid bound, and a stats counter with an API to query any-hit ray counts.

```diff
diff --git a/include/radarays_mi355.h b/include/radarays_mi355.h
--- a/include/radarays_mi355.h
+++ b/include/radarays_mi355.h
@@ -155,6 +155,7 @@
 
 int rr_set_stats_mode(rr_ctx* ctx, int enable);
 int rr_get_traversal_shape(rr_ctx* ctx, uint64_t out[8]);
+int rr_get_anyhit_rays(rr_ctx* ctx, uint64_t* rays);
 
 int rr_debug_trace(rr_ctx* ctx, const float* origs , const float* dirs , size_t n,
                    float* out_t , uint32_t* out_face );
diff --git a/radarays_ros_amd/csrc/rr_api.hip b/radarays_ros_amd/csrc/rr_api.hip
--- a/radarays_ros_amd/csrc/rr_api.hip
+++ b/radarays_ros_amd/csrc/rr_api.hip
@@ -294,6 +294,7 @@
     if (getenv("RR_STACK_LDS")) c->stack_lds_max = std::max(1, std::min(64, atoi(getenv("RR_STACK_LDS"))));
     if (getenv("RR_ROCTX") && atoi(getenv("RR_ROCTX")) != 0) c->roctx = roctx_load();
     if (getenv("RR_CULL_POP")) c->cull_pop = atoi(getenv("RR_CULL_POP")) != 0;
+    if (getenv("RR_LASTPASS_ANYHIT")) c->lastpass_anyhit = atoi(getenv("RR_LASTPASS_ANYHIT")) != 0;
     if (getenv("RR_STACKLESS")) c->stackless = atoi(getenv("RR_STACKLESS")) != 0;
     if (getenv("RR_TRACE_CHUNK")) c->seg_chunk = std::max(0, std::min(1024, atoi(getenv("RR_TRACE_CHUNK"))));
     if (getenv("RR_GRAPHS")) c->use_graphs = atoi(getenv("RR_GRAPHS")) != 0;
@@ -344,6 +345,7 @@
     for (Lane& L : c->lanes) {
         if (L.stream) (void)hipStreamSynchronize(L.stream);
         for (int k = 0; k < 2; k++) { L.d_wA[k].release(); L.d_wB[k].release(); L.d_wC[k].release(); L.d_idx[k].release(); L.d_count[k].release(); L.d_torder[k].release(); }
+        L.d_live.release();
         L.d_refpos.release();
         L.d_hit.release(); L.d_sig_count.release(); L.d_spill.release(); L.d_cflag.release(); L.d_cols_u8.release();
         L.d_sigtmp.release(); L.d_sig.release(); L.d_cols_f32.release(); L.d_counters.release(); L.d_sticky.release(); L.d_seg_stats.release(); L.d_matsets.release(); L.d_matset_limits.release(); L.d_set_beams.release(); L.d_set_order.release(); L.d_set_order2.release(); L.d_img_f32.release();
diff --git a/radarays_ros_amd/csrc/rr_ctx.h b/radarays_ros_amd/csrc/rr_ctx.h
--- a/radarays_ros_amd/csrc/rr_ctx.h
+++ b/radarays_ros_amd/csrc/rr_ctx.h
@@ -39,7 +39,7 @@
     int buf_seg = 0, buf_cap = 0, buf_sigcap = 0, buf_cells = 0, buf_passes = 0;
     DevBuf<float4> d_wA[2], d_wB[2];
     DevBuf<double2> d_wC[2];
-    DevBuf<uint32_t> d_idx[2], d_count[2], d_refpos, d_sig_count, d_spill;
+    DevBuf<uint32_t> d_idx[2], d_count[2], d_live, d_refpos, d_sig_count, d_spill;
     DevBuf<uint2> d_torder[2];
     DevBuf<uint2> d_hit;
     DevBuf<uint8_t> d_cflag, d_cols_u8;
@@ -155,6 +155,7 @@
     bool roctx = false;
     int seg_chunk = 16;
     int stackless = 0;
+    int lastpass_anyhit = 1;
     int cull_pop = 1;
     int host_sdma = 1; SdmaCopier* sdma = nullptr; bool sdma_tried = false;
     std::vector<Delivery> deliveries;
diff --git a/radarays_ros_amd/csrc/rr_device.h b/radarays_ros_amd/csrc/rr_device.h
--- a/radarays_ros_amd/csrc/rr_device.h
+++ b/radarays_ros_amd/csrc/rr_device.h
@@ -62,7 +62,7 @@
     unsigned int max_iters, n_waves;
     unsigned int overflow, pad;
     unsigned long long it_all, it_node, it_leaf, quad_steps;
-    unsigned long long pad2;
+    unsigned long long anyhit_rays;
 };
 
 constexpr int kMaxPasses = 24;
@@ -100,6 +100,7 @@
     uint2* torder[2];
     uint32_t* refpos;
     uint8_t* cflag;
+    uint32_t* live;
     SigRec* sigtmp;
     uint2* hit;
     SigRec* sig;
@@ -129,6 +130,7 @@
     int trace_row;
     int seg_chunk;
     int stackless;
+    int lastpass_anyhit;
     int cull_pop;
     GridHint* grid_hint;
     uint32_t* hist_host;
@@ -145,6 +147,13 @@
 __host__ __device__ inline int passes_of(const Params& P, int frame) { return P.set_mode ? (int)P.frame_passes[frame] : P.n_passes; }
 __host__ __device__ inline int beam_base(const Params& P, int frame) { return P.set_mode ? (int)P.frame_beam[frame] * P.n_beam : 0; }
 
+__host__ __device__ inline bool dead_wave(const Params& P, int pass, int np_f, bool in_air)
+{
+    return P.lastpass_anyhit && pass > 0 && pass == np_f - 1 && (!in_air || !(P.record_multi_reflection || P.record_multi_path));
+}
+__host__ __device__ inline int trace_dead_begin(int nlive) { return (nlive + 15) & ~15; }
+__host__ __device__ inline int trace_len(int count, int nlive) { return nlive == count ? count : trace_dead_begin(nlive) + (count - nlive); }
+
 static_assert(sizeof(Params) <= 4096, "Params is passed by value: HIP kernel arguments are limited to 4 KB");
 
 }
diff --git a/radarays_ros_amd/csrc/rr_frame.hip b/radarays_ros_amd/csrc/rr_frame.hip
--- a/radarays_ros_amd/csrc/rr_frame.hip
+++ b/radarays_ros_amd/csrc/rr_frame.hip
@@ -62,6 +62,7 @@
         RR_HIP(c, L.d_torder[k].ensure(S * cap));
         RR_HIP(c, L.d_count[k].ensure(S));
     }
+    RR_HIP(c, L.d_live.ensure(S));
     RR_HIP(c, L.d_cflag.ensure(S * 2 * cap));
     RR_HIP(c, L.d_refpos.ensure(S * 2 * cap));
     RR_HIP(c, L.d_sigtmp.ensure(S * 2 * cap));
@@ -107,7 +108,7 @@
         P.waves[k].A = L.d_wA[k].p; P.waves[k].B = L.d_wB[k].p; P.waves[k].C = L.d_wC[k].p;
         P.idx[k] = L.d_idx[k].p; P.count[k] = L.d_count[k].p; P.torder[k] = L.d_torder[k].p;
     }
-    P.refpos = L.d_refpos.p;
+    P.refpos = L.d_refpos.p; P.live = L.d_live.p;
     P.cflag = L.d_cflag.p; P.sigtmp = L.d_sigtmp.p; P.hit = L.d_hit.p;
     P.sig = L.d_sig.p; P.sig_count = L.d_sig_count.p; P.spill = L.d_spill.p; P.counters = L.d_counters.p; P.sticky = L.d_sticky.p; P.seg_stats = L.d_seg_stats.p;
     P.cols_u8 = d_cols_u8; P.cols_f32 = d_cols_f32;
@@ -131,7 +132,7 @@
     P.spill_stride = L.spill_stride; P.stack_lds = L.stack_lds;
     P.spill_depth = std::max(0, (int)c->stack_need - L.stack_lds);
     P.pass0_az = c->pass0_az;
-    P.cull_pop = c->cull_pop; P.seg_chunk = c->seg_chunk; P.stackless = c->stackless;
+    P.lastpass_anyhit = c->lastpass_anyhit; P.cull_pop = c->cull_pop; P.seg_chunk = c->seg_chunk; P.stackless = c->stackless;
     P.grid_hint = L.d_hint.p; P.ovf_list = L.d_ovf_list.p; P.ovf_stride = L.ovf_stride;
     P.hist_host = (c->tight_grid && g.n_reflections > 1) ? L.h_hist : nullptr;
 }
diff --git a/radarays_ros_amd/csrc/rr_kernels.hip b/radarays_ros_amd/csrc/rr_kernels.hip
--- a/radarays_ros_amd/csrc/rr_kernels.hip
+++ b/radarays_ros_amd/csrc/rr_kernels.hip
@@ -69,8 +69,9 @@
 __device__ inline Hit traverse(const float4* __restrict__ base4, const uint32_t tri_base4,
                                const RaySetup& R, float range_max, float hit_pad,
                                uint32_t* lds_stack, int stack_lds, uint32_t* spill, int spill_stride, int gray,
-                               unsigned& n_nodes, unsigned& n_tris, unsigned* wstat = nullptr)
-{
+                               unsigned& n_nodes, unsigned& n_tris, unsigned* wstat = nullptr, const bool any = false)
+{
+
     const int q = threadIdx.x & 3;
     const int wave = threadIdx.x >> 6;
     const int rw = (threadIdx.x & 63) >> 2;
@@ -160,6 +161,7 @@
             const unsigned long long key = ((unsigned long long)tm << 32) | fm;
             if (key < bestkey) {
                 bestkey = key; best_first = first;
+                if (any) break;
                 tcull = __builtin_fmaf(__uint_as_float(tm), 1.0001f, 1e-3f);
             }
         }
@@ -190,7 +192,7 @@
 }
 
 __device__ inline Hit traverse_stackless(const float4* __restrict__ base4, const uint32_t tri_base4,
-                                         const RaySetup& R, float range_max, float hit_pad)
+                                         const RaySetup& R, float range_max, float hit_pad, const bool any = false)
 {
     const int q = threadIdx.x & 3;
     const V3 o = R.o, d = R.d;
@@ -256,6 +258,7 @@
             const unsigned long long key = ((unsigned long long)tm << 32) | fm;
             if (key < bestkey) {
                 bestkey = key; best_first = first;
+                if (any) break;
                 tcull = __builtin_fmaf(__uint_as_float(tm), 1.0001f, 1e-3f);
             }
             prev = (int)leafkey;
@@ -285,7 +288,7 @@
 
 template <bool FIRST, bool STATS, bool SPILL, bool CULL, bool SL = false>
 __device__ __forceinline__ void trace_group(const Params& P, const int pass, const int seg_y, const int gx, const int count,
-                                            uint32_t* lds_stack, const int gdim_x, const PoseArgs* poses = nullptr)
+                                            uint32_t* lds_stack, const int gdim_x, const PoseArgs* poses = nullptr, const bool dead = false)
 {
     const int r = threadIdx.x >> 2, q = threadIdx.x & 3;
     const int cur = pass & 1;
@@ -335,9 +338,9 @@
     if (active) {
         const int gray = ((FIRST ? 0 : seg_y) * gdim_x + (int)gx) * kRaysPerBlock + r;
         Hit h;
-        if constexpr (SL) h = traverse_stackless(reinterpret_cast<const float4*>(P.nodes), P.tri_base4, R, P.range_max, P.hit_pad);
+        if constexpr (SL) h = traverse_stackless(reinterpret_cast<const float4*>(P.nodes), P.tri_base4, R, P.range_max, P.hit_pad, dead);
         else h = traverse<STATS, SPILL, CULL>(reinterpret_cast<const float4*>(P.nodes), P.tri_base4, R, P.range_max, P.hit_pad, lds_stack, P.stack_lds,
-                                              P.spill, P.spill_stride, gray, nn, nt, STATS ? ws : nullptr);
+                                              P.spill, P.spill_stride, gray, nn, nt, STATS ? ws : nullptr, dead);
         if (q == 0) {
             const size_t hk = (size_t)seg * P.cap + j;
             P.hit[hk] = make_uint2(__float_as_uint((h.tri != 0xFFFFFFFFu) ? h.t : -1.0f), h.tri);
@@ -346,7 +349,9 @@
     if (STATS) {
         unsigned it = nt >> 16; nt &= 0xFFFFu;
         for (int off = 32; off > 0; off >>= 1) { nn += __shfl_down(nn, off); nt += __shfl_down(nt, off); it = max(it, (unsigned)__shfl_down(it, off)); }
+        const unsigned n_any = dead ? (unsigned)__builtin_popcountll(__ballot(active)) >> 2 : 0u;
         if ((threadIdx.x & 63) == 0) {
+            if (n_any) atomicAdd(&P.counters->anyhit_rays, (unsigned long long)n_any);
             atomicAdd(&P.counters->nodes, (unsigned long long)nn);
             atomicAdd(&P.counters->tris, (unsigned long long)nt);
             atomicAdd(&P.counters->wave_iters, (unsigned long long)it);
@@ -365,6 +370,16 @@
             atomicAdd(&P.counters->quad_steps, (unsigned long long)d2);
         }
     }
+}
+
+struct TraceSpan { int end; bool dead; };
+__device__ __forceinline__ TraceSpan trace_span(const Params& P, const int cur, const int seg, const int gx)
+{
+    const int count = (int)P.count[cur][seg], nlive = (int)P.live[seg];
+    TraceSpan ts;
+    ts.dead = nlive != count && gx * kRaysPerBlock >= trace_dead_begin(nlive);
+    ts.end = ts.dead ? trace_len(count, nlive) : nlive;
+    return ts;
 }
 
 template <bool FIRST, bool STATS, bool SPILL, bool CULL, bool SL = false>
@@ -389,11 +404,16 @@
         seg_y = ch * P.seg_chunk + (int)blockIdx.x;
         if (seg_y >= P.n_seg) return;
     }
-    const int count = FIRST ? 0 : (int)P.count[cur][seg_y];
-    if (!FIRST && gx * kRaysPerBlock >= count) return;
+    int count = 0;
+    bool dead = false;
+    if (!FIRST) {
+        const TraceSpan ts = trace_span(P, cur, seg_y, gx);
+        if (ts.end <= gx * kRaysPerBlock) return;
+        count = ts.end; dead = ts.dead;
+    }
     const PoseArgs* pa = nullptr;
     if constexpr (FIRST) pa = &poses;
-    trace_group<FIRST, STATS, SPILL, CULL, SL>(P, pass, seg_y, gx, count, lds_stack, gdim, pa);
+    trace_group<FIRST, STATS, SPILL, CULL, SL>(P, pass, seg_y, gx, count, lds_stack, gdim, pa, dead);
 }
 
 template <bool CULL>
@@ -406,9 +426,11 @@
     const int tight = (int)P.tight_groups[pass];
     for (uint32_t i = 0; i < n; i++) {
         const int seg = (int)P.ovf_list[(size_t)pass * P.ovf_stride + i];
-        const int count = (int)P.count[pass & 1][seg];
-        for (int g = tight + (int)blockIdx.x; g * kRaysPerBlock < count; g += (int)gridDim.x) {
-            trace_group<false, false, false, CULL>(P, pass, seg, g, count, lds_stack, 0);
+        const int tlen = trace_len((int)P.count[pass & 1][seg], (int)P.live[seg]);
+        for (int g = tight + (int)blockIdx.x; g * kRaysPerBlock < tlen; g += (int)gridDim.x) {
+            const TraceSpan ts = trace_span(P, pass & 1, seg, g);
+            if (ts.end <= g * kRaysPerBlock) continue;
+            trace_group<false, false, false, CULL>(P, pass, seg, g, ts.end, lds_stack, 0, nullptr, ts.dead);
             if (threadIdx.x == 0) atomicAdd(&P.grid_hint->repaired, 1ull);
         }
     }
@@ -607,6 +629,13 @@
     } else {
         const uint32_t slot = P.idx[cur][(size_t)seg * P.cap + j];
         const size_t w = base2 + slot;
+        const uint32_t medium = __float_as_uint(reinterpret_cast<const float*>(P.waves[cur].B + w)[2]);
+        if (dead_wave(P, pass, np_f, (int)medium == P.material_id_air)) {
+            const SigRec none = { -1, 0.0f };
+            P.cflag[s0] = __uint_as_float(P.hit[(size_t)seg * P.cap + j].x) >= 0.0f ? 4 : 0; P.cflag[s1] = 0;
+            P.sigtmp[s0] = none; P.sigtmp[s1] = none;
+            return;
+        }
         const float4 A = P.waves[cur].A[w], B = P.waves[cur].B[w];
         const double2 C = P.waves[cur].C[w];
         orig = { A.x, A.y, A.z };
@@ -665,7 +694,7 @@
             if (renergy > (double)P.thr)
             {
                 if (!last) {
-                    f0 |= 1;
+                    f0 |= ((int)mat == P.material_id_air) ? 1 : 3;
                     const V3 o2 = v_add(orig, v_scale(rdir, skip_dist));
                     const double t2 = time + (double)skip_dist / 0.3;
                     P.waves[nxt].A[s0] = make_float4(o2.x, o2.y, o2.z, rdir.x);
@@ -697,7 +726,7 @@
             }
             if (!last && tenergy > (double)P.thr)
             {
-                f1 |= 1;
+                f1 |= ((int)mat_refr == P.material_id_air) ? 1 : 3;
                 const V3 o2 = v_add(orig, v_scale(tdir, skip_dist));
                 const double t2 = time + (double)skip_dist / 0.3;
                 P.waves[nxt].A[s1] = make_float4(o2.x, o2.y, o2.z, tdir.x);
@@ -739,6 +768,9 @@
     const int sig_before = n_sig;
     int n_hit = 0, n_refl = 0, my_hits = 0;
     unsigned ovf = 0;
+    const int np_f = passes_of(P, seg / P.n_loc);
+    const bool sort_dead = P.lastpass_anyhit && pass + 1 == np_f - 1;
+    int my_live0 = 0, my_live1 = 0;
     uint8_t f_nx = 0; SigRec sr_nx = { -1, 0.0f };
     if ((int)threadIdx.x < n_slots) { f_nx = P.cflag[base2 + threadIdx.x]; sr_nx = P.sigtmp[base2 + threadIdx.x]; }
     for (int b = 0; b < n_slots; b += 256) {
@@ -753,6 +785,7 @@
         const int pre = block_excl_scan(((s & 1) ? (c << 10) : c) | (g << 20), tot, lds);
         const int pos = n_child + (pre & 1023) + ((pre >> 10) & 1023);
         if (c) { if (pos < P.cap) { P.idx[nxt][(size_t)seg * P.cap + pos] = (uint32_t)s; P.refpos[base2 + s] = (uint32_t)pos; } else { ovf = 1; P.refpos[base2 + s] = 0xFFFFFFFFu; } }
+        if (sort_dead && c && pos < P.cap && !dead_wave(P, pass + 1, np_f, !(f & 2))) { if (s & 1) my_live1++; else my_live0++; }
         n_child += (tot & 1023) + ((tot >> 10) & 1023);
         n_refl += tot & 1023;
         const int spos = n_sig + ((pre >> 20) & 1023);
@@ -766,6 +799,7 @@
         n_hit = tot;
     }
     __syncthreads();
+    int n_live = 0;
     {
         int n_refl_placed = 0;
         {
@@ -779,36 +813,53 @@
                 int tot; block_excl_scan(mine, tot, lds); n_refl_placed = tot;
             }
         }
-        int placed0 = 0, placed1 = 0;
+        const int n_placed = min(n_child, P.cap);
+        bool dead_block = false;
+        if (sort_dead) {
+            int tot0, tot1;
+            block_excl_scan(my_live0, tot0, lds); block_excl_scan(my_live1, tot1, lds);
+            dead_block = n_placed + 15 <= P.cap && tot0 + tot1 < n_placed;
+            if (dead_block) { n_refl_placed = tot0; n_live = tot0 + tot1; }
+        }
+        if (!dead_block) n_live = n_placed;
+        const int dead_at = trace_dead_begin(n_live);
+        if (dead_block && n_live + (int)threadIdx.x < dead_at)
+            P.torder[nxt][(size_t)seg * P.cap + n_live + threadIdx.x] = make_uint2(0xFFFFFFFFu, 0u);
+        const int n_parents = pass >= np_f - 1 ? 0 : count;
+        int placed0 = 0, placed1 = 0, placed_d = 0;
         auto fetch = [&](int k, int& c0, int& c1, uint32_t& rp0, uint32_t& rp1, uint32_t& jp) {
             c0 = c1 = 0; rp0 = rp1 = 0xFFFFFFFFu; jp = 0;
-            if (k < count) {
+            if (k < n_parents) {
                 const uint32_t j = FIRST ? P.beam_order2[beam_base(P, seg / P.n_loc) + k] : P.torder[cur][(size_t)seg * P.cap + k].x;
                 const size_t sl = base2 + 2 * (size_t)j;
                 const uint2 rp = *reinterpret_cast<const uint2*>(P.refpos + sl);
                 const uint8_t f0 = P.cflag[sl], f1 = P.cflag[sl + 1];
                 if (f0 & 1) { rp0 = rp.x; c0 = rp0 != 0xFFFFFFFFu; }
                 if (f1 & 1) { rp1 = rp.y; c1 = rp1 != 0xFFFFFFFFu; }
+                if (dead_block) { c0 |= (c0 && dead_wave(P, pass + 1, np_f, !(f0 & 2))) << 1; c1 |= (c1 && dead_wave(P, pass + 1, np_f, !(f1 & 2))) << 1; }
                 jp = j;
             }
         };
         int c0n, c1n; uint32_t rp0n, rp1n, jpn;
         fetch((int)threadIdx.x, c0n, c1n, rp0n, rp1n, jpn);
-        for (int b = 0; b < count; b += 256) {
+        for (int b = 0; b < n_parents; b += 256) {
             const int c0 = c0n, c1 = c1n; const uint32_t rp0 = rp0n, rp1 = rp1n, jp = jpn;
             fetch(b + 256 + (int)threadIdx.x, c0n, c1n, rp0n, rp1n, jpn);
             int tot;
-            const int pre = block_excl_scan(c0 | (c1 << 10), tot, lds);
-            if (c0) P.torder[nxt][(size_t)seg * P.cap + placed0 + (pre & 1023)] = make_uint2(rp0, 2u * jp);
-            if (c1) P.torder[nxt][(size_t)seg * P.cap + n_refl_placed + placed1 + ((pre >> 10) & 1023)] = make_uint2(rp1, 2u * jp + 1u);
-            placed0 += tot & 1023; placed1 += (tot >> 10) & 1023;
+            const int d0 = c0 >> 1, d1 = c1 >> 1;
+            const int pre = block_excl_scan((c0 == 1) | ((c1 == 1) << 10) | ((d0 + d1) << 20), tot, lds);
+            const size_t tb = (size_t)seg * P.cap, td = tb + dead_at + placed_d + ((pre >> 20) & 1023);
+            if (c0) P.torder[nxt][d0 ? td : tb + placed0 + (pre & 1023)] = make_uint2(rp0, 2u * jp);
+            if (c1) P.torder[nxt][d1 ? td + d0 : tb + n_refl_placed + placed1 + ((pre >> 10) & 1023)] = make_uint2(rp1, 2u * jp + 1u);
+            placed0 += tot & 1023; placed1 += (tot >> 10) & 1023; placed_d += (tot >> 20) & 1023;
         }
     }
     if (__syncthreads_or((int)ovf) && threadIdx.x == 0) { atomicOr(&P.counters->overflow, 1u); atomicOr(P.sticky, 1u); }
     if (threadIdx.x == 0) {
         P.count[nxt][seg] = (uint32_t)min(n_child, P.cap);
+        P.live[seg] = (uint32_t)n_live;
         if (P.grid_hint && pass + 1 < kMaxPasses) {
-            const uint32_t cn = (uint32_t)min(n_child, P.cap);
+            const uint32_t cn = (uint32_t)trace_len(min(n_child, P.cap), n_live);
             if (cn > P.grid_hint->hist[pass + 1]) atomicMax(&P.grid_hint->hist[pass + 1], cn);
             const uint32_t tg = P.tight_groups[pass + 1];
             if (tg && cn > tg * (uint32_t)kRaysPerBlock) {
@@ -1332,7 +1383,8 @@
     const int n_seg = (pass == 0 && P.set_mode) ? P.n_groups * P.n_loc : P.n_seg;
     const int A0 = P.pass0_az, Sw0 = kRaysPerWave / A0;
     const size_t waves0 = (size_t)((n_seg + A0 - 1) / A0) * (size_t)((P.n_beam + Sw0 - 1) / Sw0);
-    const long bound = std::min<long>((long)P.cap, pass < 20 ? (long)P.n_beam << pass : (long)P.cap);
+    long bound = std::min<long>((long)P.cap, pass < 20 ? (long)P.n_beam << pass : (long)P.cap);
+    if (P.lastpass_anyhit && pass > 0 && (P.set_mode || pass == P.n_passes - 1)) bound = std::min<long>((long)P.cap, bound + 15);
     const unsigned row = (pass > 0 && pass < kMaxPasses && P.tight_groups[pass]) ? (unsigned)P.tight_groups[pass]
                                                                                : (unsigned)((bound + kRaysPerBlock - 1) / kRaysPerBlock);
     const bool tightened = pass > 0 && pass < kMaxPasses && P.tight_groups[pass];
diff --git a/radarays_ros_amd/csrc/rr_probe.hip b/radarays_ros_amd/csrc/rr_probe.hip
--- a/radarays_ros_amd/csrc/rr_probe.hip
+++ b/radarays_ros_amd/csrc/rr_probe.hip
@@ -45,6 +45,19 @@
     { const int rcb = read_counters(c, h); if (rcb) return rcb; }
     out[0] = h.n_waves; out[1] = h.it_all; out[2] = h.it_node; out[3] = h.it_leaf; out[4] = h.quad_steps; out[5] = h.max_iters;
     out[6] = h.nodes; out[7] = h.quad_steps > h.nodes ? h.quad_steps - h.nodes : 0;
+    return 0;
+}
+int rr_get_anyhit_rays(rr_ctx* c, uint64_t* rays)
+{
+    if (!c || !rays) return -1;
+    RR_HIP(c, hipSetDevice(c->device));
+    RR_HIP(c, hipDeviceSynchronize());
+    *rays = 0;
+    Lane& L = c->lanes[c->last_lane];
+    if (!L.d_counters.p) return 0;
+    Counters h;
+    { const int rcb = read_counters(c, h); if (rcb) return rcb; }
+    *rays = h.anyhit_rays;
     return 0;
 }
 int rr_set_timing_mode(rr_ctx* c, int enable) { if (!c) return -1; c->timing = enable; return 0; }
diff --git a/radarays_ros_amd/native.py b/radarays_ros_amd/native.py
--- a/radarays_ros_amd/native.py
+++ b/radarays_ros_amd/native.py
@@ -20,7 +20,7 @@
     "rr_create_multi", "rr_destroy_multi", "rr_multi_last_error", "rr_multi_device_count", "rr_multi_rccl_version", "rr_multi_ctx",
     "rr_multi_set_mesh", "rr_multi_set_mesh_gpu", "rr_multi_set_materials", "rr_multi_set_config", "rr_multi_set_beam_samples",
     "rr_multi_set_noise_offsets", "rr_multi_set_motion_poses", "rr_multi_simulate", "rr_multi_simulate_batch",
-    "rr_multi_simulate_batch_async", "rr_multi_wait", "rr_peek_error_bits_async", "rr_get_traversal_shape",
+    "rr_multi_simulate_batch_async", "rr_multi_wait", "rr_peek_error_bits_async", "rr_get_traversal_shape", "rr_get_anyhit_rays",
     "rr_cone_dirs", "rr_sample_cone_local", "rr_load_mesh_file", "rr_mesh_reorder_objects", "rr_free_mesh",
     "rr_simulate_param_sets_device", "rr_simulate_param_sets", "rr_score_images_device",
     "rr_set_object_poses", "rr_update_vertices", "rr_get_tree_cost", "rr_rebuild_tree",
@@ -191,6 +191,7 @@
     L.rr_multi_wait.argtypes = [vp, vp]
     L.rr_peek_error_bits_async.argtypes = [vp, vp, vp]
     L.rr_get_traversal_shape.argtypes = [vp, vp]
+    L.rr_get_anyhit_rays.argtypes = [vp, C.POINTER(C.c_uint64)]
     L.rr_simulate_param_sets_device.argtypes = [vp, vp, C.POINTER(RRParamSet), C.c_int, C.c_size_t, vp, vp]
     L.rr_simulate_param_sets.argtypes = [vp, vp, C.POINTER(RRParamSet), C.c_int, C.c_size_t, vp, vp, vp]
     L.rr_score_images_device.argtypes = [vp, vp, C.c_int, vp, vp, vp, vp]
@@ -443,6 +444,11 @@
         return dict(zip(("waves", "iterations", "node_path_issues", "leaf_path_issues", "live_quad_steps", "max_iterations",
                          "node_steps", "leaf_steps"), (int(x) for x in a)))
 
+    def anyhit_rays(self):
+        n = C.c_uint64(0)
+        self._ck(self._L.rr_get_anyhit_rays(self._h, C.byref(n)))
+        return int(n.value)
+
     def simulate_columns_device(self, pose, az_begin, az_end, d_cols_u8_ptr, d_cols_f32_ptr=None, stream=None):
         p = np.ascontiguousarray(pose, np.float32)
         self._ck(self._L.rr_simulate_columns_device(self._h, p.ctypes.data, az_begin, az_end,
```

Result: no change. 4691 images/s, median of 6 (+1.0%).
